# wenet-e2e/wenet

Hardware: AMD Instinct MI355X
Metric: audio-seconds/sec (RTF^-1), 12L Conformer fbank80, ctc_prefix_beam_search (higher is better)
Workload: dtype f32 (feed-forward and subsampling-conv2 GEMMs: fp32 operands as three exact bf16 planes, six plane products on the bf16 matrix cores, f32 accumulate -- error <= the v_mfma_f32 kernel's, tests/test_gpu_x6.py; everything else v_mfma_f32)

## Files before the change

include/wenet_amd.h:

```cpp
#ifndef WENET_AMD_H_
#define WENET_AMD_H_

#include <stdint.h>

#ifdef __cplusplus
extern "C" {
#endif

typedef struct wn_model wn_model;

typedef struct {
  int32_t feat_dim;
  int32_t d_model;
  int32_t n_heads;
  int32_t ffn_dim;
  int32_t n_layers;
  int32_t cnn_kernel;
  int32_t causal;
  int32_t use_dynamic_chunk;
  int32_t static_chunk_size;
  int32_t vocab;
  int32_t has_cmvn;
  int32_t dec_heads;
  int32_t dec_ffn_dim;
  int32_t dec_layers;
  int32_t dec_r_layers;
  int32_t bidirectional;
  int32_t sos, eos;
  int32_t max_pos;
  float norm_eps;
  int32_t encoder_type;
  int32_t input_layer;
  int32_t activation;
  int32_t key_bias;
  int32_t cnn_norm;
  int32_t dec_activation;
  int32_t dec_key_bias;
  int32_t dec_src_key_bias;
  int32_t dec_learned_pos;
  int32_t dec_max_pos;
} wn_config;

typedef struct {
  const char* name;
  const float* data;
  int64_t numel;
} wn_tensor;

const char* wn_last_error(void);
const char* wn_version(void);

int wn_model_create(const wn_config* cfg, const wn_tensor* weights,
                    int32_t n_weights, int32_t device, wn_model** out);
void wn_model_destroy(wn_model* m);

int wn_model_clone(const wn_model* src, wn_model** out);

#define WN_PREC_F32 0
#define WN_PREC_BF16 1
#define WN_PREC_FP8 2
int wn_model_set_precision(wn_model* m, int32_t precision);
int32_t wn_model_get_precision(const wn_model* m);

int32_t wn_batch_size(const wn_model* m);

int wn_model_set_encode_gate(wn_model* m, void* event);

int wn_workspace_create(int32_t device, wn_model** out);

int64_t wn_resample_length(int64_t n_in, int32_t orig_freq, int32_t new_freq);
int wn_resample(wn_model* m, const float* pcm_dev, int64_t n_in, int32_t orig_freq,
                int32_t new_freq, float* out_dev, int64_t n_out, void* stream);

int wn_fbank(wn_model* m, const float* pcm_dev, const int64_t* sample_off_host,
             int32_t B, float* feats_dev, int32_t max_frames,
             int32_t* n_frames_host, void* stream);

int wn_log_mel(wn_model* m, const float* pcm_dev, const int64_t* sample_off_host,
               int32_t B, int32_t n_mels, float* feats_dev, int32_t max_frames,
               int32_t* n_frames_host, void* stream);

int wn_encode(wn_model* m, const float* feats_dev, const int32_t* feat_lens_host,
              int32_t B, int32_t T, int32_t decoding_chunk_size,
              int32_t num_left_chunks, float* enc_out_dev,
              int32_t* enc_lens_host, void* stream);

int wn_encode_chunk(wn_model* m, const float* feats_dev, int32_t time, int32_t offset,
                    int32_t required_cache_size, const float* att_cache_dev,
                    int32_t cache_t1, const float* cnn_cache_dev, float* out_dev,
                    float* new_att_cache_dev, float* new_cnn_cache_dev,
                    int32_t* chunk_out, int32_t* new_cache_t1_out, void* stream);

int wn_encode_chunk_batch(wn_model* m, int32_t n_sess, const float* feats_dev, int32_t time,
                          const int32_t* offsets_host, int32_t required_cache_size,
                          const float* const* att_cache_dev, const int32_t* cache_t1_host,
                          const float* const* cnn_cache_dev, float* out_dev,
                          float* const* new_att_cache_dev, float* const* new_cnn_cache_dev,
                          int32_t* chunk_out, int32_t* new_cache_t1_out, void* stream);

int wn_set_encoder_out(wn_model* m, const float* enc_out_dev,
                       const int32_t* enc_lens_host, int32_t B, int32_t Tp,
                       void* stream);

int wn_ctc_logprobs(wn_model* m, int32_t topk, int32_t blank_id,
                    float blank_penalty, float* logp_dev, int32_t Tp,
                    void* stream);

int wn_set_ctc_probs(wn_model* m, const float* logp_dev,
                     const int32_t* lens_host, int32_t B, int32_t Tp,
                     int32_t V, int32_t topk, void* stream);

int wn_ctc_greedy_search(wn_model* m, int32_t blank_id, int32_t* tokens_host,
                         int32_t* tok_lens_host, int32_t max_len, void* stream);

int wn_ctc_force_align(wn_model* m, int32_t blank_id, float blank_penalty,
                       const int32_t* labels_host, const int32_t* label_lens_host,
                       int32_t max_label, const float* logp_dev, const int32_t* lens_host,
                       int32_t B, int32_t Tp, int32_t V, int32_t* path_host, float* score_host,
                       int32_t* status_host, float* frame_logp_host, float* emit_host,
                       void* stream);

int wn_set_context_graph(wn_model* m, int32_t n_nodes, const int32_t* fail,
                         const double* node_score, const double* output_score,
                         const double* token_score, int32_t n_edges,
                         const int32_t* edge_from, const int32_t* edge_token,
                         const int32_t* edge_to, void* stream);

int wn_ctc_prefix_beam_search(wn_model* m, int32_t beam, int32_t blank_id,
                              int32_t* n_hyps_host, int32_t* hyp_lens_host,
                              int32_t* hyp_tlens_host, int32_t* hyp_tokens_host,
                              int32_t* hyp_times_host, double* hyp_scores_host,
                              int32_t max_len, void* stream);

typedef struct wn_stream_set wn_stream_set;

typedef struct wn_stream_result {
  int32_t* n_hyps;
  int32_t* hyp_lens;
  int32_t* hyp_tlens;
  int32_t* hyp_tokens;
  int32_t* hyp_times;
  double* hyp_scores;
  double* hyp_viterbi;
  int32_t* frames_decoded;
  int32_t* trailing_blank;
  int32_t max_len;
} wn_stream_result;

int wn_stream_create(wn_model* m, int32_t n_slots, int32_t beam, int32_t max_frames,
                     int32_t blank_id, wn_stream_set** out, void* stream);
int wn_stream_destroy(wn_stream_set* set);

int wn_stream_set_endpoint(wn_stream_set* set, float blank_threshold, float blank_scale);

int wn_stream_reset(wn_stream_set* set, int32_t n, const int32_t* slot_ids, void* stream);

int wn_stream_advance(wn_stream_set* set, int32_t n, const int32_t* slot_ids,
                      const float* logp_dev, const int32_t* n_t_host, int32_t Tp, int32_t V,
                      int32_t nbest, const wn_stream_result* out, void* stream);

int wn_stream_advance_encoded(wn_stream_set* set, int32_t n, const int32_t* slot_ids,
                              const float* enc_out_dev, const int32_t* n_t_host, int32_t chunk,
                              int32_t nbest, const wn_stream_result* out, void* stream);

int wn_attention_rescoring(wn_model* m, int32_t beam, const int32_t* n_hyps_host,
                           const int32_t* hyp_lens_host,
                           const int32_t* hyp_tokens_host, int32_t max_len,
                           float reverse_weight, float* l2r_logp_host,
                           float* r2l_logp_host, void* stream);

int wn_rescore_prefetch(wn_model* m, int32_t use_right_decoder, void* stream);

int wn_rescore(wn_model* m, int32_t beam, const int32_t* n_hyps_host,
               const int32_t* hyp_lens_host, const int32_t* hyp_tokens_host,
               const double* ctc_scores_host, int32_t max_len, double ctc_weight,
               double reverse_weight, int32_t* best_idx_host, float* best_score_host,
               double* confidence_host, double* tok_conf_host, float* all_scores_host,
               void* stream);

int wn_decoder_forward(wn_model* m, int32_t utt, int32_t which, int32_t n_seq,
                       const int32_t* tokens_host, const int32_t* lens_host,
                       int32_t max_len, float* logp_dev, void* stream);

int wn_filter_blank_embedding(wn_model* m, float* padded_out_dev, int32_t* n_keep_host,
                              int32_t* t_out, void* stream);

int wn_attention_beam_search(wn_model* m, int32_t beam, int32_t maxlen, float length_penalty,
                             int32_t* tokens_host, int32_t* lens_host, void* stream);

// ... 395 lines not shown
```

wenet_amd/_lib.py:

```python
import ctypes
import os
from ctypes import (POINTER, Structure, c_char_p, c_double, c_float, c_int32,
                    c_int64, c_void_p)

_HERE = os.path.dirname(os.path.abspath(__file__))
LIB_PATH = os.path.join(_HERE, 'libwenet_amd.so')


class WnConfig(Structure):
    _fields_ = [(n, c_int32) for n in (
        'feat_dim', 'd_model', 'n_heads', 'ffn_dim', 'n_layers', 'cnn_kernel',
        'causal', 'use_dynamic_chunk', 'static_chunk_size', 'vocab',
        'has_cmvn', 'dec_heads', 'dec_ffn_dim', 'dec_layers', 'dec_r_layers',
        'bidirectional', 'sos', 'eos', 'max_pos')] + [('norm_eps', c_float)] + [
            (n, c_int32) for n in ('encoder_type', 'input_layer', 'activation',
                                   'key_bias', 'cnn_norm',
                                   'dec_activation', 'dec_key_bias', 'dec_src_key_bias',
                                   'dec_learned_pos', 'dec_max_pos')]


class WnTransducerConfig(Structure):
    _fields_ = [(n, c_int32) for n in ('pred_embed', 'pred_hidden', 'pred_layers', 'pred_out',
                                       'join_dim', 'blank')]


class WnStatelessPredictorConfig(Structure):
    _fields_ = [(n, c_int32) for n in ('kind', 'context', 'heads', 'activation', 'conv_bias')] + [
        ('norm_eps', c_float)]


class WnFireRedConfig(Structure):
    _fields_ = [(n, c_int32) for n in ('sub_channels', 'conv_inner_factor', 'max_frames')] + [
        ('attn_norm_eps', c_float)]


class WnBranchformerConfig(Structure):
    _fields_ = [(n, c_int32) for n in ('kind', 'cgmlp_units', 'cgmlp_kernel', 'merge_kernel',
                                       'linear_after_conv', 'head_dim')]


class WnParaformerConfig(Structure):
    _fields_ = [(n, c_int32) for n in ('lfr_m', 'lfr_n', 'kernel_size', 'dec_blocks',
                                       'max_frames')] + [
        (n, c_float) for n in ('threshold', 'tail_threshold', 'smooth_factor',
                               'noise_threshold')]


class WnTensor(Structure):
    _fields_ = [('name', c_char_p), ('data', POINTER(c_float)),
                ('numel', c_int64)]


class WnStreamResult(Structure):
    _fields_ = [('n_hyps', POINTER(c_int32)), ('hyp_lens', POINTER(c_int32)),
                ('hyp_tlens', POINTER(c_int32)), ('hyp_tokens', POINTER(c_int32)),
                ('hyp_times', POINTER(c_int32)), ('hyp_scores', POINTER(c_double)),
                ('hyp_viterbi', POINTER(c_double)), ('frames_decoded', POINTER(c_int32)),
                ('trailing_blank', POINTER(c_int32)), ('max_len', c_int32)]


class WnRnntStreamResult(Structure):
    _fields_ = [('tok_lens', POINTER(c_int32)), ('tokens', POINTER(c_int32)),
                ('times', POINTER(c_int32)), ('frames_decoded', POINTER(c_int32)),
                ('trailing_blank', POINTER(c_int32)), ('max_len', c_int32),
                ('steps', POINTER(c_int32))]


class WnRnntBeamStreamResult(Structure):
    _fields_ = [('n_hyps', POINTER(c_int32)), ('hyp_lens', POINTER(c_int32)),
                ('hyp_tokens', POINTER(c_int32)), ('hyp_scores', POINTER(c_double)),
                ('frames_decoded', POINTER(c_int32)), ('trailing_blank', POINTER(c_int32)),
                ('max_len', c_int32)]


class WnAttentionOp(Structure):
    _fields_ = [('Q', c_void_p), ('K', c_void_p), ('V', c_void_p),
                ('ldq', c_int32), ('ldk', c_int32), ('ldv', c_int32),
                ('q_rows', c_int32), ('kv_rows', c_int32),
                ('P', c_void_p), ('ldp', c_int32), ('p_rows', c_int32),
                ('p_off', POINTER(c_int32)), ('bias_u', c_void_p), ('bias_v', c_void_p),
                ('O', c_void_p), ('ldo', c_int32),
                ('q_off', POINTER(c_int32)), ('q_len', POINTER(c_int32)),
                ('kv_off', POINTER(c_int32)), ('kv_len', POINTER(c_int32)),
                ('n_seq', c_int32), ('n_heads', c_int32), ('mask_mode', c_int32),
                ('chunk_size', c_int32), ('left_chunks', c_int32), ('scale', c_float),
                ('flags', c_int32), ('precision', c_int32), ('x6_galign', c_int32)]


EXPORTS = [
    'wn_last_error', 'wn_version', 'wn_model_create', 'wn_model_destroy', 'wn_model_clone',
    'wn_model_set_precision', 'wn_model_get_precision', 'wn_batch_size', 'wn_model_set_encode_gate', 'wn_op_gemm_bf16',
    'wn_op_gemm_bf16_stored',
    'wn_attention_beam_search', 'wn_attention_beam_search_prompt', 'wn_attention_truncated',
    'wn_op_gemm_skinny', 'wn_encode_chunk_batch', 'wn_op_gemm_lowp', 'wn_op_mx_quantize', 'wn_op_ffn_fused', 'wn_op_gemm_x6', 'wn_op_ffn_x6', 'wn_op_gemm_x6r', 'wn_op_gemm_x6r512', 'wn_profile_kernel_name', 'wn_profile_ffn_split', 'wn_profile_ffn_clocks', 'wn_profile_gemm_clocks', 'wn_filter_blank_embedding',
    'wn_workspace_create', 'wn_resample_length', 'wn_resample', 'wn_fbank', 'wn_log_mel', 'wn_encode', 'wn_encode_chunk', 'wn_set_encoder_out',
    'wn_ctc_logprobs', 'wn_set_ctc_probs', 'wn_ctc_greedy_search', 'wn_ctc_force_align',
    'wn_set_context_graph', 'wn_ctc_prefix_beam_search', 'wn_attention_rescoring', 'wn_rescore', 'wn_rescore_prefetch', 'wn_decoder_forward', 'wn_decoder_next_topk', 'wn_op_gemm',
    'wn_op_layernorm', 'wn_op_log_add', 'wn_op_attention', 'wn_op_dwconv', 'wn_op_conv1',
    'wn_op_conv2d4',
    'wn_op_ctc_rows', 'wn_debug_set', 'wn_profile_enable',
    'wn_profile_collect', 'wn_tune_set', 'wn_model_tune_set', 'wn_tune_get',
    'wn_stream_create', 'wn_stream_destroy', 'wn_stream_set_endpoint', 'wn_stream_reset',
    'wn_stream_advance', 'wn_stream_advance_encoded',
    'wn_model_create_transducer', 'wn_transducer_greedy_search', 'wn_op_lstm_step',
    'wn_op_joint_argmax', 'wn_transducer_beam_search', 'wn_op_joint_fuse_topk',
    'wn_op_rnnt_beam_step', 'wn_transducer_beam_stats',
    'wn_rnnt_stream_create', 'wn_rnnt_stream_destroy', 'wn_rnnt_stream_reset',
    'wn_rnnt_stream_advance_encoded', 'wn_rnnt_stream_state',
    'wn_rnnt_beam_stream_create', 'wn_rnnt_beam_stream_destroy', 'wn_rnnt_beam_stream_reset',
    'wn_rnnt_beam_stream_advance_encoded', 'wn_rnnt_beam_stream_state',
    'wn_op_rnnt_beam_step_carry',
    'wn_transducer_score', 'wn_transducer_score_stats', 'wn_transducer_score_times',
    'wn_op_rnnt_trie',
    'wn_op_joint_logp_gather', 'wn_op_rnnt_lattice',
    'wn_op_attn_self_step', 'wn_op_attn_step_embed', 'wn_op_attn_prompt_cache', 'wn_op_beam_init',
    'wn_op_beam_update', 'wn_op_beam_finish',
    'wn_op_layernorm_ex', 'wn_op_layernorm2', 'wn_op_layernorm_mx', 'wn_op_ffn_reduce_ln',
    'wn_op_gemm_rowln',
    'wn_model_create_transducer_stateless', 'wn_op_stateless_step',
    'wn_op_attention_relshift', 'wn_op_firered_frontend', 'wn_model_create_firered',
    'wn_model_create_branchformer', 'wn_op_csgu_gate', 'wn_op_merge_dwconv', 'wn_csgu_time_tile',
    'wn_op_attention_d128', 'wn_op_lfr_front', 'wn_op_layernorm_wide', 'wn_op_cif_alpha',
    'wn_op_cif_fire', 'wn_model_create_paraformer', 'wn_paraformer_decode',
]

_lib = None


def lib():
    global _lib
    if _lib is not None:
        return _lib
    if not os.path.exists(LIB_PATH):
        raise RuntimeError(
            f'{LIB_PATH} is missing: build it with `python -m wenet_amd.build` '
            '(hipcc --offload-arch=gfx950). wenet_amd has no CPU fallback.')
    import torch
    L = ctypes.CDLL(LIB_PATH, mode=ctypes.RTLD_GLOBAL)
    i32, i64, f32, vp = c_int32, c_int64, c_float, c_void_p
    pi32, pf64 = POINTER(c_int32), POINTER(c_double)
    L.wn_last_error.restype = c_char_p
    L.wn_profile_kernel_name.restype = c_char_p
    L.wn_profile_kernel_name.argtypes = [vp]
    L.wn_profile_ffn_split.restype = c_int32
    L.wn_profile_ffn_split.argtypes = [vp]
    L.wn_profile_ffn_clocks.argtypes = [POINTER(ctypes.c_uint64)]
    L.wn_profile_gemm_clocks.argtypes = [POINTER(ctypes.c_uint64)]
    L.wn_version.restype = c_char_p
    L.wn_model_create.argtypes = [POINTER(WnConfig), POINTER(WnTensor), i32,
                                  i32, POINTER(vp)]
    L.wn_model_destroy.argtypes = [vp]
    L.wn_model_clone.argtypes = [vp, POINTER(vp)]
    L.wn_model_destroy.restype = None
    L.wn_workspace_create.argtypes = [i32, POINTER(vp)]
    L.wn_fbank.argtypes = [vp, vp, POINTER(i64), i32, vp, i32, pi32, vp]
    L.wn_log_mel.argtypes = [vp, vp, POINTER(i64), i32, i32, vp, i32, pi32, vp]
    L.wn_encode.argtypes = [vp, vp, pi32, i32, i32, i32, i32, vp, pi32, vp]
    L.wn_set_encoder_out.argtypes = [vp, vp, pi32, i32, i32, vp]
    L.wn_ctc_logprobs.argtypes = [vp, i32, i32, f32, vp, i32, vp]
    L.wn_encode_chunk.argtypes = [vp, vp, i32, i32, i32, vp, i32, vp, vp, vp, vp, pi32,
                                  pi32, vp]
    L.wn_encode_chunk_batch.argtypes = [vp, i32, vp, i32, pi32, i32, POINTER(vp), pi32,
                                        POINTER(vp), vp, POINTER(vp), POINTER(vp), pi32, pi32,
                                        vp]
    L.wn_resample_length.argtypes = [ctypes.c_int64, i32, i32]
    L.wn_resample_length.restype = ctypes.c_int64
    L.wn_resample.argtypes = [vp, vp, ctypes.c_int64, i32, i32, vp, ctypes.c_int64, vp]
    L.wn_set_ctc_probs.argtypes = [vp, vp, pi32, i32, i32, i32, i32, vp]
    L.wn_ctc_greedy_search.argtypes = [vp, i32, pi32, pi32, i32, vp]
    L.wn_ctc_force_align.argtypes = [vp, i32, f32, pi32, pi32, i32, vp, pi32, i32, i32, i32,
                                     pi32, POINTER(f32), pi32, POINTER(f32), POINTER(f32), vp]
    L.wn_set_context_graph.argtypes = [vp, i32, pi32, pf64, pf64, pf64, i32, pi32, pi32,
                                       pi32, vp]
    L.wn_ctc_prefix_beam_search.argtypes = [vp, i32, i32, pi32, pi32, pi32,
                                            pi32, pi32, pf64, i32, vp]
    L.wn_stream_create.argtypes = [vp, i32, i32, i32, i32, POINTER(vp), vp]
    L.wn_stream_destroy.argtypes = [vp]
    L.wn_stream_set_endpoint.argtypes = [vp, f32, f32]
    L.wn_stream_reset.argtypes = [vp, i32, pi32, vp]
    L.wn_stream_advance.argtypes = [vp, i32, pi32, vp, pi32, i32, i32, i32,
                                    POINTER(WnStreamResult), vp]
    L.wn_stream_advance_encoded.argtypes = [vp, i32, pi32, vp, pi32, i32, i32,
                                            POINTER(WnStreamResult), vp]
    L.wn_attention_rescoring.argtypes = [vp, i32, pi32, pi32, pi32, i32, f32,
                                         POINTER(f32), POINTER(f32), vp]
    L.wn_rescore.argtypes = [vp, i32, pi32, pi32, pi32, pf64, i32, c_double, c_double, pi32,
                             POINTER(f32), pf64, pf64, POINTER(f32), vp]
    L.wn_rescore_prefetch.argtypes = [vp, i32, vp]
    L.wn_decoder_forward.argtypes = [vp, i32, i32, i32, pi32, pi32, i32, vp, vp]
    L.wn_decoder_next_topk.argtypes = [vp, i32, pi32, pi32, pi32, i32, i32,
                                       POINTER(f32), pi32, vp]
    L.wn_attention_beam_search.argtypes = [vp, i32, i32, f32, pi32, pi32, vp]
    L.wn_attention_beam_search_prompt.argtypes = [vp, i32, i32, f32, pi32, i32, pi32, pi32, vp]
    L.wn_attention_truncated.argtypes = [vp]
    L.wn_op_gemm.argtypes = [vp, vp, vp, vp, vp, i32, i32, i32, f32, i32, vp]
    L.wn_op_gemm_skinny.argtypes = [vp, vp, vp, vp, vp, i32, i32, i32, i32, i32, i32, vp]
    L.wn_op_gemm_bf16.argtypes = L.wn_op_gemm.argtypes
    L.wn_op_gemm_bf16_stored.argtypes = [vp, vp, vp, vp, vp, i32, i32, i32, f32, i32, i32, vp]
    L.wn_op_gemm_lowp.argtypes = [vp, vp, vp, vp, vp, vp, vp, vp, i32, i32, i32, f32, i32, i32,
                                  i32, vp]
    L.wn_op_mx_quantize.argtypes = [vp, i32, i32, vp, vp, vp]
    L.wn_op_ffn_fused.argtypes = [vp, vp, vp, vp, vp, vp, vp, vp, vp, i32, i32, i32, i32, f32,
                                  f32, vp]
    L.wn_op_gemm_x6.argtypes = [vp, vp, vp, vp, vp, i32, i32, i32, f32, i32, i32, i32, vp]
    L.wn_op_ffn_x6.argtypes = [vp, vp, vp, vp, vp, vp, vp, vp, vp, i32, i32, i32, i32, f32,
                               f32, i32, vp]
    L.wn_filter_blank_embedding.argtypes = [vp, vp, pi32, pi32, vp]
    L.wn_op_gemm_x6r.argtypes = [vp, vp, vp, vp, vp, vp, vp, vp, i32, i32, i32, f32, f32, i32, vp]
    L.wn_op_gemm_x6r512.argtypes = [vp, vp, vp, vp, vp, vp, vp, vp, vp, vp, i32, i32, i32, f32, f32,
                                    i32, vp]
    L.wn_model_set_precision.argtypes = [vp, i32]
    L.wn_model_get_precision.argtypes = [vp]
    L.wn_batch_size.argtypes = [vp]
    L.wn_batch_size.restype = i32
    L.wn_model_set_encode_gate.argtypes = [vp, vp]
    L.wn_op_layernorm.argtypes = [vp, vp, vp, vp, i32, i32, f32, vp]
    L.wn_op_log_add.argtypes = [vp, vp, vp, i32, vp]
    L.wn_op_attention.argtypes = [POINTER(WnAttentionOp), pi32, vp]
    L.wn_op_dwconv.argtypes = [vp, i32, vp, vp, vp, vp, vp, i32, vp, i32, pi32, pi32, i32, i32,
                               i32, i32, i32, i32, f32, vp]
    L.wn_op_conv1.argtypes = [vp, vp, vp, vp, vp, vp, pi32, pi32, i32, i32, i32, i32, i32, i32,
                              vp]
    L.wn_op_conv2d4.argtypes = [vp, vp, pi32, i32, i32, vp, vp, vp, pi32, pi32, vp]
    L.wn_op_ctc_rows.argtypes = [vp, i32, i32, i32, i32, i32, f32, vp, vp, vp, i32, vp]
    L.wn_debug_set.argtypes = [vp, c_char_p, i32]
    L.wn_tune_set.argtypes = [c_char_p, i32]
    L.wn_model_tune_set.argtypes = [vp, c_char_p, i32]
    L.wn_tune_get.argtypes = [vp, c_char_p, pi32]
    L.wn_profile_enable.argtypes = [vp, i32]
    L.wn_profile_collect.argtypes = [vp, pi32, pf64, pf64]
    L.wn_model_create_transducer.argtypes = [POINTER(WnConfig), POINTER(WnTransducerConfig),
                                             POINTER(WnTensor), i32, i32, POINTER(vp)]
    L.wn_model_create_transducer_stateless.argtypes = [
        POINTER(WnConfig), POINTER(WnTransducerConfig), POINTER(WnStatelessPredictorConfig),
        POINTER(WnTensor), i32, i32, POINTER(vp)]
    L.wn_op_stateless_step.argtypes = [POINTER(WnStatelessPredictorConfig), pi32, POINTER(vp),
                                       pi32, vp, i32, i32, i32, i32, vp]
    L.wn_transducer_greedy_search.argtypes = [vp, i32, pi32, pi32, i32, pi32, vp]
    L.wn_rnnt_stream_create.argtypes = [vp, i32, i32, i32, i32, POINTER(vp), vp]
    L.wn_rnnt_stream_destroy.argtypes = [vp]
    L.wn_rnnt_stream_reset.argtypes = [vp, i32, pi32, vp]
    L.wn_rnnt_stream_advance_encoded.argtypes = [vp, i32, pi32, vp, pi32, i32,
# ... 107 lines not shown
```

wenet_amd/csrc/cabi_align.hip:

```cpp
#include "model_state.h"

namespace wn {
namespace {

int align_check(int blank_id, const int32_t* labels, const int32_t* label_lens, int max_label,
                const int32_t* lens, int B, int Tp, int V, const int32_t* status_host) {
  WN_CHECK(labels && label_lens && status_host, "wn_ctc_force_align: null argument");
  WN_CHECK(B >= 1 && Tp >= 1 && V >= 1 && max_label >= 0, "wn_ctc_force_align: bad argument");
  WN_CHECK(blank_id >= 0 && blank_id < V, "wn_ctc_force_align: blank_id outside the vocabulary");
  for (int b = 0; b < B; ++b) {
    WN_CHECK(label_lens[b] >= 0 && label_lens[b] <= max_label,
             "wn_ctc_force_align: label_len must be in [0, max_label]");
    if (lens) WN_CHECK(lens[b] >= 0 && lens[b] <= Tp, "wn_ctc_force_align: length > Tp");
    for (int i = 0; i < label_lens[b]; ++i) {
      const int id = labels[(size_t)b * max_label + i];
      if (id < 0 || id >= V) {
        set_error("wn_ctc_force_align: label id " + std::to_string(id) + " of utterance " +
                  std::to_string(b) + " is outside the vocabulary [0, " + std::to_string(V) + ")");
        return -1;
      }
      WN_CHECK(id != blank_id, "wn_ctc_force_align: blank_id among the labels");
    }
  }
  return 0;
// ... 2 lines not shown
}
}

extern "C" {

int wn_ctc_force_align(wn_model* m, int32_t blank_id, float blank_penalty,
                       const int32_t* labels_host, const int32_t* label_lens_host,
                       int32_t max_label, const float* logp_dev, const int32_t* lens_host,
                       int32_t B, int32_t Tp, int32_t V, int32_t* path_host, float* score_host,
                       int32_t* status_host, float* frame_logp_host, float* emit_host,
                       void* stream) {
  const bool given = logp_dev != nullptr;
  if (given) {
    WN_CHECK(lens_host, "wn_ctc_force_align: null lengths with caller-provided log-probs");
    WN_TRY(align_check(blank_id, labels_host, label_lens_host, max_label, lens_host, B, Tp, V,
                       status_host));
    WN_CHECK(m, "wn_ctc_force_align: null handle");
  } else {
    WN_CHECK(m && m->B > 0 && m->enc.p,
             "wn_ctc_force_align: no current batch (call wn_encode / wn_set_encoder_out)");
    WN_CHECK(!lens_host, "wn_ctc_force_align: lens_host without logp_dev");
    WN_CHECK(B == m->B && Tp == m->Tp, "wn_ctc_force_align: B / Tp are not the current batch's");
    V = m->cfg.vocab;
    WN_TRY(align_check(blank_id, labels_host, label_lens_host, max_label, nullptr, B, Tp, V,
                       status_host));
  }
  WN_ENTER(m);
  PrecisionScope prec_scope(m);
  hipStream_t s = (hipStream_t)stream;
  WN_HIP(hipSetDevice(m->device));

  const int M = given ? B * Tp : m->rows;
  std::vector<int> off(B), len(B);
  for (int b = 0; b < B; ++b) {
    off[b] = given ? b * Tp : m->off[b];
    len[b] = given ? lens_host[b] : m->len[b];
  }
  const int LP = max_label + 1;
  int max_fast = -1, max_slow = -1;
  std::vector<int> d((size_t)3 * B + (size_t)B * LP);
  std::vector<int64_t> bp_off(B);
  int64_t bp_bytes = 0;
  for (int b = 0; b < B; ++b) {
    const int L = label_lens_host[b];
    d[b] = off[b]; d[B + b] = len[b]; d[2 * B + b] = L;
    int* lab = d.data() + 3 * (size_t)B + (size_t)b * LP;
    lab[0] = blank_id;
    for (int i = 0; i < LP - 1; ++i) lab[1 + i] = i < L ? labels_host[(size_t)b * max_label + i] : blank_id;
    if (2 * L + 1 <= ALIGN_FAST_S) max_fast = std::max(max_fast, L);
    else max_slow = std::max(max_slow, L);
    bp_off[b] = bp_bytes;
    bp_bytes += ctc_align_bp_bytes(len[b], L, ALIGN_FAST_S);
  }
  const size_t d_bytes = (d.size() * sizeof(int) + 7) / 8 * 8;
  WN_TRY(m->stage.begin(d_bytes + bp_off.size() * sizeof(int64_t) + 256));
  WN_TRY(m->al_desc.ensure(d_bytes + bp_off.size() * sizeof(int64_t)));
  WN_TRY(m->stage.put_at(m->al_desc.p, d.data(), d.size() * sizeof(int), s));
  WN_TRY(m->stage.put_at(m->al_desc.as<char>() + d_bytes, bp_off.data(),
                         bp_off.size() * sizeof(int64_t), s));
  WN_TRY(m->stage.end(s));
  const int* dd = m->al_desc.as<int>();

  const size_t o_sc = 0, o_st = o_sc + (size_t)B * sizeof(float),
               o_path = o_st + (size_t)B * sizeof(int),
               o_fl = o_path + (size_t)B * Tp * sizeof(int),
               o_e = (o_fl + (size_t)B * Tp * 2 * sizeof(float) + 255) / 256 * 256,
               o_end = o_e + (size_t)std::max(M, 1) * LP * sizeof(float);
  WN_TRY(m->al_out.ensure(o_end));
  WN_TRY(m->al_bp.ensure((size_t)bp_bytes + 64));
  char* ob = m->al_out.as<char>();
  float* E = reinterpret_cast<float*>(ob + o_e);

  if (M > 0) {
    AlignGatherArgs g;
    g.M = M; g.V = V; g.blank = blank_id;
    g.off = dd; g.len = dd + B; g.lab_len = dd + 2 * B; g.lab = dd + 3 * B; g.lab_pitch = LP;
    g.E = E; g.ldE = LP;
    if (given) {
      g.x = logp_dev; g.ld = V; g.normalize = 0; g.blank_penalty = 0.f;
      g.row_utt = nullptr; g.Tp = Tp;
    } else {
      const ModelData& W = *m->data;
      WN_CHECK(W.ctc.w, "wn_ctc_force_align: this handle has no weights");
      const int V4 = (V + 31) / 32 * 32;
      WN_TRY(m->logits.ensure((size_t)M * V4 * sizeof(float)));
      WN_TRY(vocab_linear(m, W.ctc, m->enc.as<float>(), m->cfg.d_model, m->logits.as<float>(), V4,
                          M, s));
      g.x = m->logits.as<float>(); g.ld = V4; g.normalize = 1;
      g.blank_penalty = blank_penalty > 0.f ? blank_penalty : 0.f;
      g.row_utt = m->d_row_utt.as<int>(); g.Tp = Tp;
    }
    WN_TRY(ctc_align_gather(g, s));
  }
  AlignArgs a;
  a.E = E; a.ldE = LP; a.off = dd; a.len = dd + B; a.B = B; a.Tp = Tp;
  a.lab = dd + 3 * B; a.lab_pitch = LP; a.lab_len = dd + 2 * B;
  a.bp = m->al_bp.as<unsigned char>();
  a.bp_off = reinterpret_cast<const int64_t*>(m->al_desc.as<char>() + d_bytes);
  a.fast_S = ALIGN_FAST_S;
  a.path = reinterpret_cast<int*>(ob + o_path);
  a.frame_logp = frame_logp_host ? reinterpret_cast<float*>(ob + o_fl) : nullptr;
  a.score = reinterpret_cast<float*>(ob + o_sc);
  a.status = reinterpret_cast<int*>(ob + o_st);
  WN_TRY(ctc_align_viterbi(a, max_fast, max_slow, s));
  const size_t n_copy = emit_host ? o_end : (frame_logp_host ? o_e : o_fl);
  WN_TRY(m->al_host.ensure(n_copy));
  WN_HIP(hipMemcpyAsync(m->al_host.p, ob, n_copy, hipMemcpyDeviceToHost, s));
  WN_HIP(stream_wait(s));
  const char* hb = m->al_host.p;
  const int* st = reinterpret_cast<const int*>(hb + o_st);
  const float* sc = reinterpret_cast<const float*>(hb + o_sc);
  for (int b = 0; b < B; ++b) {
    status_host[b] = st[b];
    if (st[b] != 0) continue;
    if (score_host) score_host[b] = sc[b];
    const size_t n = (size_t)len[b];
    if (path_host)
      memcpy(path_host + (size_t)b * Tp, hb + o_path + (size_t)b * Tp * sizeof(int),
             n * sizeof(int));
    if (frame_logp_host)
      memcpy(frame_logp_host + (size_t)b * Tp * 2, hb + o_fl + (size_t)b * Tp * 2 * sizeof(float),
             n * 2 * sizeof(float));
    if (emit_host)
      memcpy(emit_host + (size_t)b * Tp * LP, hb + o_e + (size_t)off[b] * LP * sizeof(float),
             n * LP * sizeof(float));
  }
  return 0;
}

}
```

wenet_amd/csrc/cabi_ctc.hip:

```cpp
#include "model_state.h"

struct wn_stream_set {
  wn_model* m = nullptr;
  int n_slots = 0, beam = 0, max_frames = 0, blank = 0;
  float blank_thr = 0.8f;
  int64_t pool_ints = 0;
  DevBuf state, pool;
  DevBuf emit;
  std::vector<int> abs_t;
  DevBuf desc;
  Stager stage;
  DevBuf topk_val, topk_idx, logits;
  DevBuf out;
  PinnedBuf host;
};

namespace wn {
namespace {

__global__ void scatter_padded_any_kernel(const float* src, int lds,
                                          const int* off, const int* len,
                                          int Tp, int D, float* dst) {
  const int b = blockIdx.y, t = blockIdx.x;
  float* d = dst + ((int64_t)b * Tp + t) * D;
// ... 117 lines not shown
  WN_TRY(S->stage.begin(d.size() * sizeof(int) + 64));
  WN_TRY(S->stage.put(S->desc, d.data(), d.size() * sizeof(int), s));
  WN_TRY(S->stage.end(s));
  const StreamOutLayout o(n, rows, max_len);
  WN_TRY(S->out.ensure(o.end));
  WN_TRY(S->host.ensure(o.end));
  char* ob = S->out.as<char>();
  StreamPrefixBeamArgs a;
  a.topk_val = S->topk_val.as<float>(); a.topk_idx = S->topk_idx.as<int>(); a.k = beam;
  a.off = S->desc.as<int>() + n; a.len = S->desc.as<int>() + 2 * n; a.B = n;
  a.beam = beam; a.blank = S->blank; a.max_len = S->max_frames;
  a.pool = S->pool.as<int>(); a.pool_stride = S->pool_ints;
  a.n_hyps = reinterpret_cast<int*>(ob + o.nh); a.hyp_lens = reinterpret_cast<int*>(ob + o.len);
  a.hyp_tlens = reinterpret_cast<int*>(ob + o.tlen);
  a.hyp_tokens = reinterpret_cast<int*>(ob + o.tok);
  a.hyp_times = reinterpret_cast<int*>(ob + o.tim);
  a.hyp_scores = reinterpret_cast<double*>(ob + o.sc);
  a.st.state = S->state.p; a.st.slot = S->desc.as<int>();
  a.st.nbest = nbest ? 1 : 0; a.st.out_stride = max_len;
  a.st.logp = logp; a.st.ld = ld; a.st.blank_thr = S->blank_thr;
  a.st.hyp_vit = reinterpret_cast<double*>(ob + o.vit);
  a.st.emit = S->emit.as<int>();
  a.st.frames = reinterpret_cast<int*>(ob + o.fd); a.st.trail = reinterpret_cast<int*>(ob + o.tb);
  PbCycles dbg;
  WN_TRY(dbg.arm(S->m, &a.dbg_cycles));
  WN_TRY(ctc_prefix_beam_stream(a, s));
  WN_TRY(dbg.print("stream search", "state store + emit", false, s));
  WN_HIP(hipMemcpyAsync(S->host.p, ob, o.end, hipMemcpyDeviceToHost, s));
  for (int i = 0; i < n; ++i) S->abs_t[slot_ids[i]] += n_t[i];
  WN_HIP(stream_wait(s));
  const char* hb = S->host.p;
  const int* nh = reinterpret_cast<const int*>(hb + o.nh);
  const int* hl = reinterpret_cast<const int*>(hb + o.len);
  const int* htl = reinterpret_cast<const int*>(hb + o.tlen);
  const double* sc = reinterpret_cast<const double*>(hb + o.sc);
  const double* vit = reinterpret_cast<const double*>(hb + o.vit);
  memcpy(out->n_hyps, nh, (size_t)n * sizeof(int));
  memcpy(out->frames_decoded, hb + o.fd, (size_t)n * sizeof(int));
  memcpy(out->trailing_blank, hb + o.tb, (size_t)n * sizeof(int));
  for (int i = 0; i < n; ++i) {
    for (int j = 0; j < beam; ++j) {
      const size_t dst = (size_t)i * beam + j, src = (size_t)i * rows + j;
      const bool have = j < rows;
      const int nl = have ? std::min(std::max(hl[src], 0), max_len) : 0;
      const int ntl = have ? std::min(std::max(htl[src], 0), max_len) : 0;
      out->hyp_lens[dst] = nl; out->hyp_tlens[dst] = ntl;
      out->hyp_scores[dst] = have ? sc[src] : -HUGE_VAL;
      if (out->hyp_viterbi) out->hyp_viterbi[dst] = have ? vit[src] : -HUGE_VAL;
      if (have) {
        memcpy(out->hyp_tokens + dst * max_len, hb + o.tok + src * max_len * sizeof(int),
               (size_t)nl * sizeof(int));
        memcpy(out->hyp_times + dst * max_len, hb + o.tim + src * max_len * sizeof(int),
               (size_t)ntl * sizeof(int));
      }
    }
  }
  return 0;
}

}
}

extern "C" {

int wn_ctc_logprobs(wn_model* m, int32_t topk, int32_t blank_id,
                    float blank_penalty, float* logp_dev, int32_t Tp,
                    void* stream) {
  WN_CHECK(m && m->B > 0, "wn_ctc_logprobs: no current batch (call wn_encode)");
  WN_ENTER(m);
  m->pb_valid = false;
  PrecisionScope prec_scope(m);
  const ModelData& W = *m->data;
  WN_CHECK(W.ctc.w, "wn_ctc_logprobs: this handle has no weights");
  hipStream_t s = (hipStream_t)stream;
  WN_HIP(hipSetDevice(m->device));
  const wn_config& c = m->cfg;
  const int M = m->rows, V = c.vocab;
  const int k = std::max(1, topk);
  WN_CHECK(k <= V, "top-k larger than the vocabulary");
  WN_CHECK(!logp_dev || Tp == m->Tp, "wn_ctc_logprobs: Tp mismatch");
  m->ctc_rows = M; m->ctc_k = k;
  int ldv = V;
  if (M > 0) {
    const int V4 = (V + 31) / 32 * 32;
    ldv = V4;
    WN_TRY(m->logits.ensure((size_t)M * V4 * sizeof(float)));
    WN_TRY(m->topk_val.ensure((size_t)M * k * sizeof(float)));
    WN_TRY(m->topk_idx.ensure((size_t)M * k * sizeof(int)));
    WN_TRY(vocab_linear(m, W.ctc, m->enc.as<float>(), c.d_model, m->logits.as<float>(), V4, M,
                        s));
    CtcRowArgs r;
    r.logits = m->logits.as<float>(); r.ld = V4; r.M = M; r.V = V; r.k = k;
    r.blank = blank_id; r.blank_penalty = blank_penalty > 0.f ? blank_penalty : 0.f;
    r.topk_val = m->topk_val.as<float>(); r.topk_idx = m->topk_idx.as<int>();
    r.logp = logp_dev ? m->logits.as<float>() : nullptr; r.ld_out = V4;
    WN_TRY(ctc_logsoftmax_topk(r, s));
  }
  if (logp_dev) {
    if (M > 0) {
      hipLaunchKernelGGL(scatter_padded_any_kernel, dim3(m->Tp, m->B), dim3(256),
                         0, s, m->logits.as<float>(), ldv, m->d_off.as<int>(),
                         m->d_len.as<int>(), m->Tp, V, logp_dev);
      WN_HIP(hipGetLastError());
    } else {
      WN_HIP(hipMemsetAsync(logp_dev, 0, (size_t)m->B * m->Tp * V * sizeof(float), s));
    }
  }
  m->ctc_valid = true;
  return 0;
}

int wn_set_ctc_probs(wn_model* m, const float* logp_dev, const int32_t* lens_host,
                     int32_t B, int32_t Tp, int32_t V, int32_t topk,
                     void* stream) {
  WN_CHECK(m && logp_dev && lens_host && B > 0 && Tp > 0 && V > 0,
           "wn_set_ctc_probs: bad argument");
  WN_ENTER(m);
  m->pb_valid = false;
  hipStream_t s = (hipStream_t)stream;
  WN_HIP(hipSetDevice(m->device));
  const int k = std::max(1, topk);
  WN_CHECK(k <= V, "top-k larger than the vocabulary");
  std::vector<int> off(B), len(B);
  for (int b = 0; b < B; ++b) {
    WN_CHECK(lens_host[b] >= 0 && lens_host[b] <= Tp, "length > Tp");
    off[b] = b * Tp; len[b] = lens_host[b];
  }
  WN_TRY(set_layout(m, B, Tp, off, len, B * Tp, s));
  WN_TRY(m->stage.end(s));
  const int M = B * Tp;
  WN_TRY(m->topk_val.ensure((size_t)M * k * sizeof(float)));
  WN_TRY(m->topk_idx.ensure((size_t)M * k * sizeof(int)));
  hipLaunchKernelGGL(topk_raw_kernel, dim3(M), dim3(256), 0, s, logp_dev, V, V,
                     k, m->topk_val.as<float>(), m->topk_idx.as<int>());
  WN_HIP(hipGetLastError());
  m->ctc_rows = M; m->ctc_k = k; m->ctc_valid = true;
  return 0;
}

int wn_ctc_greedy_search(wn_model* m, int32_t blank_id, int32_t* tokens_host,
                         int32_t* tok_lens_host, int32_t max_len, void* stream) {
  WN_CHECK(m && m->ctc_valid, "greedy: no CTC posteriors (call wn_ctc_logprobs)");
  WN_ENTER(m);
  WN_CHECK(tokens_host && tok_lens_host, "greedy: null output");
  hipStream_t s = (hipStream_t)stream;
  WN_HIP(hipSetDevice(m->device));
  const int B = m->B;
  int longest = 0;
  for (int b = 0; b < B; ++b) longest = std::max(longest, m->len[b]);
  WN_CHECK(max_len >= longest, "greedy: max_len smaller than the longest utterance");
  const int ml = std::max(max_len, 1);
  WN_TRY(m->g_tok.ensure((size_t)B * ml * sizeof(int)));
  WN_TRY(m->g_len.ensure((size_t)B * sizeof(int)));
  WN_TRY(ctc_greedy_collapse(m->topk_idx.as<int>(), m->ctc_k, m->d_off.as<int>(),
                             m->d_len.as<int>(), B, blank_id, m->g_tok.as<int>(),
                             ml, m->g_len.as<int>(), s));
  WN_HIP(hipMemcpyAsync(tokens_host, m->g_tok.p, (size_t)B * ml * sizeof(int),
                        hipMemcpyDeviceToHost, s));
  WN_HIP(hipMemcpyAsync(tok_lens_host, m->g_len.p, (size_t)B * sizeof(int),
                        hipMemcpyDeviceToHost, s));
  WN_HIP(stream_wait(s));
  return 0;
}

int wn_filter_blank_embedding(wn_model* m, float* padded_out_dev, int32_t* n_keep_host,
                              int32_t* t_out, void* stream) {
  WN_CHECK(m && m->B > 0 && m->enc.p && m->ctc_valid && n_keep_host && t_out,
           "filter_blank_embedding: needs the encoder output and the CTC posteriors of the "
           "current batch (wn_encode / wn_set_encoder_out, then wn_ctc_logprobs)");
  WN_ENTER(m);
  hipStream_t s = (hipStream_t)stream;
  WN_HIP(hipSetDevice(m->device));
  const int B = m->B, d = m->cfg.d_model, M = m->rows;
  WN_CHECK(m->ctc_rows == M, "filter_blank_embedding: CTC posteriors of another layout");
  WN_TRY(m->nb_map.ensure((size_t)std::max(M, 1) * sizeof(int)));
  WN_TRY(m->nb_keep.ensure((size_t)B * sizeof(int)));
  WN_TRY(nonblank_map(m->topk_idx.as<int>(), m->ctc_k, m->d_off.as<int>(), m->d_len.as<int>(), B,
                      m->nb_map.as<int>(), m->nb_keep.as<int>(), s));
  std::vector<int> keep(B);
  WN_HIP(hipMemcpyAsync(keep.data(), m->nb_keep.p, (size_t)B * sizeof(int),
                        hipMemcpyDeviceToHost, s));
  WN_HIP(stream_wait(s));
  int T = 0;
  for (int b = 0; b < B; ++b) { n_keep_host[b] = keep[b]; T = std::max(T, keep[b]); }
  *t_out = T;
  if (T == 0) {
    static bool warned = false;
    if (!warned) {
      fprintf(stderr, "[wenet_amd] filter_blank_embedding: no non-blank frame in the whole "
                      "batch; the encoder output is left unfiltered\n");
      warned = true;
// ... 184 lines not shown
  WN_TRY(S->desc.ensure(3 * (size_t)n_slots * sizeof(int)));
  const StreamOutLayout o(n_slots, 1, max_frames);
  WN_TRY(S->out.ensure(o.end));
  WN_TRY(S->host.ensure(o.end));
  std::vector<int> all(n_slots);
  for (int i = 0; i < n_slots; ++i) all[i] = i;
  WN_TRY(S->stage.begin(all.size() * sizeof(int) + 64));
  WN_TRY(S->stage.put(S->desc, all.data(), all.size() * sizeof(int), s));
  WN_TRY(S->stage.end(s));
  WN_TRY(ctc_stream_reset(S->state.p, S->pool.as<int>(), S->pool_ints, max_frames, beam,
                          S->desc.as<int>(), n_slots, s));
  WN_HIP(hipStreamSynchronize(s));
  *out = S.release();
  return 0;
}

int wn_stream_destroy(wn_stream_set* set) {
  delete set;
  return 0;
}

int wn_stream_set_endpoint(wn_stream_set* set, float blank_threshold, float blank_scale) {
  WN_CHECK(set, "wn_stream_set_endpoint: null argument");
  WN_CHECK(blank_threshold > 0.f && blank_scale > 0.f, "wn_stream_set_endpoint: bad argument");
  set->blank_thr = blank_threshold * blank_scale;
  return 0;
}

int wn_stream_reset(wn_stream_set* set, int32_t n, const int32_t* slot_ids, void* stream) {
  WN_CHECK(set && slot_ids, "wn_stream_reset: null argument");
  WN_CHECK(n >= 1 && n <= set->n_slots, "wn_stream_reset: n must be in [1, n_slots]");
  for (int i = 0; i < n; ++i)
    WN_CHECK(slot_ids[i] >= 0 && slot_ids[i] < set->n_slots, "wn_stream_reset: slot id out of range");
  WN_ENTER(set->m);
  hipStream_t s = (hipStream_t)stream;
  WN_HIP(hipSetDevice(set->m->device));
  WN_TRY(set->stage.begin((size_t)n * sizeof(int) + 64));
  WN_TRY(set->stage.put(set->desc, slot_ids, (size_t)n * sizeof(int), s));
  WN_TRY(set->stage.end(s));
  WN_TRY(ctc_stream_reset(set->state.p, set->pool.as<int>(), set->pool_ints, set->max_frames,
                          set->beam, set->desc.as<int>(), n, s));
  for (int i = 0; i < n; ++i) set->abs_t[slot_ids[i]] = 0;
  return 0;
}

int wn_stream_advance(wn_stream_set* set, int32_t n, const int32_t* slot_ids,
                      const float* logp_dev, const int32_t* n_t_host, int32_t Tp, int32_t V,
                      int32_t nbest, const wn_stream_result* out, void* stream) {
  WN_CHECK(set && slot_ids && logp_dev && n_t_host && out, "wn_stream_advance: null argument");
  WN_CHECK(Tp >= 1 && V >= 1, "wn_stream_advance: bad argument");
  WN_CHECK(set->beam <= V, "wn_stream_advance: top-k larger than the vocabulary");
  WN_CHECK(set->blank < V, "wn_stream_advance: blank_id outside the vocabulary");
  WN_TRY(stream_check(set, n, slot_ids, n_t_host, Tp, out));
  WN_ENTER(set->m);
  hipStream_t s = (hipStream_t)stream;
  WN_HIP(hipSetDevice(set->m->device));
  const int M = n * Tp, k = set->beam;
  WN_TRY(set->topk_val.ensure((size_t)M * k * sizeof(float)));
  WN_TRY(set->topk_idx.ensure((size_t)M * k * sizeof(int)));
  hipLaunchKernelGGL(topk_raw_kernel, dim3(M), dim3(256), 0, s, logp_dev, V, V, k,
                     set->topk_val.as<float>(), set->topk_idx.as<int>());
  WN_HIP(hipGetLastError());
  return stream_search(set, n, slot_ids, n_t_host, Tp, logp_dev, V, nbest, out, s);
}

int wn_stream_advance_encoded(wn_stream_set* set, int32_t n, const int32_t* slot_ids,
                              const float* enc_out_dev, const int32_t* n_t_host, int32_t chunk,
                              int32_t nbest, const wn_stream_result* out, void* stream) {
  WN_CHECK(set && slot_ids && enc_out_dev && n_t_host && out,
           "wn_stream_advance_encoded: null argument");
  WN_CHECK(chunk >= 1, "wn_stream_advance_encoded: bad argument");
  wn_model* m = set->m;
  const ModelData& W = *m->data;
  WN_CHECK(W.ctc.w, "wn_stream_advance_encoded: this handle has no weights");
  WN_CHECK(set->beam <= m->cfg.vocab && set->blank < m->cfg.vocab,
           "wn_stream_advance_encoded: beam / blank_id outside the vocabulary");
  WN_TRY(stream_check(set, n, slot_ids, n_t_host, chunk, out));
  WN_ENTER(m);
  PrecisionScope prec_scope(m);
  hipStream_t s = (hipStream_t)stream;
  WN_HIP(hipSetDevice(m->device));
  const wn_config& c = m->cfg;
  const int M = n * chunk, V = c.vocab, k = set->beam;
  const int V4 = (V + 31) / 32 * 32;
  WN_TRY(set->logits.ensure((size_t)M * V4 * sizeof(float)));
  WN_TRY(set->topk_val.ensure((size_t)M * k * sizeof(float)));
  WN_TRY(set->topk_idx.ensure((size_t)M * k * sizeof(int)));
  WN_TRY(vocab_linear(m, W.ctc, enc_out_dev, c.d_model, set->logits.as<float>(), V4, M, s));
  CtcRowArgs r;
  r.logits = set->logits.as<float>(); r.ld = V4; r.M = M; r.V = V; r.k = k;
  r.blank = set->blank; r.blank_penalty = 0.f;
  r.topk_val = set->topk_val.as<float>(); r.topk_idx = set->topk_idx.as<int>();
  r.logp = set->logits.as<float>(); r.ld_out = V4;
  WN_TRY(ctc_logsoftmax_topk(r, s));
  return stream_search(set, n, slot_ids, n_t_host, chunk, set->logits.as<float>(), V4, nbest, out,
                       s);
}

}
```

wenet_amd/csrc/cabi_firered.hip:

```cpp
#include "model_state.h"

static int encoder_layers_firered(wn_model* m, hipStream_t s) {
  const ModelData& W = *m->data;
  const wn_config& c = m->cfg;
  const int d = c.d_model, d2 = 2 * d, H = c.n_heads, M = m->rows;
  float* x = m->x.as<float>();
  float* t1 = m->t1.as<float>();
  float* t2 = m->t2.as<float>();
  float* hb = m->hbuf.as<float>();
  float* qkv = m->qkv.as<float>();
  const float eps = c.norm_eps;
  int max_len = 0;
  for (int b = 0; b < m->B; ++b) max_len = std::max(max_len, m->len[b]);
  const int n_run = m->dbg_layers >= 0 ? std::min(m->dbg_layers, c.n_layers) : c.n_layers;
  for (int li = 0; li < n_run; ++li) {
    const EncLayer& L = W.layers[li];
    WN_TRY(ln(L.norm_ff_mac, x, t1, M, d, eps, s));
    WN_TRY(linear(L.ffm1, t1, d, hb, c.ffn_dim, M, s, ACT_SILU));
    WN_TRY(linear(L.ffm2, hb, c.ffn_dim, x, d, M, s, ACT_NONE, x, d, 0.5f));
    WN_TRY(ln(L.norm_mha, x, t1, M, d, m->fr.c.attn_norm_eps, s));
    WN_TRY(linear(L.qkv, t1, d, qkv, 3 * d, M, s));
    RelShiftAttnArgs a;
    a.Q = qkv; a.K = qkv + d; a.V = qkv + 2 * d;
    a.ldq = a.ldk = a.ldv = 3 * d;
    a.P = L.pos_tab; a.ldp = d;
    a.p_center = m->fr.c.max_frames - 1; a.p_rows = 2 * m->fr.c.max_frames - 1;
    a.bias_u = L.bias_u; a.bias_v = L.bias_v;
    a.O = t2; a.ldo = d;
    a.off = m->d_off.as<int>(); a.len = m->d_len.as<int>();
    a.n_seq = m->B; a.n_heads = H; a.max_len = max_len;
    a.scale = 1.0f / sqrtf(64.0f);
    WN_TRY(attention_relshift(a, s));
    WN_TRY(linear(L.out, t2, d, x, d, M, s, ACT_NONE, x, d));
    WN_TRY(ln(L.norm_conv, x, t1, M, d, eps, s));
    float* glu = hb;
    float* cv = hb + (size_t)M * d2;
    WN_TRY(linear(L.pw1, t1, d, glu, d2, M, s, ACT_NONE, nullptr, 0, 1.0f, true));
    DwConvArgs dw;
    dw.x = glu; dw.ldx = d2; dw.wt = L.dw_wt; dw.bias = L.dw_b; dw.cpad = L.cpad;
    dw.ln_w = L.conv_norm.w; dw.ln_b = L.conv_norm.b; dw.norm_mode = 0;
    dw.y = cv; dw.ldy = d2;
    dw.row_utt = m->d_row_utt.as<int>(); dw.off = m->d_off.as<int>(); dw.len = m->d_len.as<int>();
    dw.M = M; dw.D = d2; dw.K = c.cnn_kernel; dw.causal = 0;
    dw.t_max = m->Tp; dw.eps = 1e-5f;
    WN_TRY(dwconv_ln_silu(dw, s));
    WN_TRY(linear(L.pw2, cv, d2, x, d, M, s, ACT_NONE, x, d));
    WN_TRY(ln(L.norm_ff, x, t1, M, d, eps, s));
    WN_TRY(linear(L.ff1, t1, d, hb, c.ffn_dim, M, s, ACT_SILU));
    WN_TRY(linear(L.ff2, hb, c.ffn_dim, x, d, M, s, ACT_NONE, x, d, 0.5f));
    WN_TRY(ln(L.norm_final, x, x, M, d, eps, s));
  }
  WN_TRY(m->enc.ensure((size_t)std::max(M, 1) * d * sizeof(float)));
  WN_HIP(hipMemcpyAsync(m->enc.p, m->x.p, (size_t)M * d * sizeof(float), hipMemcpyDeviceToDevice,
                        s));
  return 0;
}

int encode_firered(wn_model* m, const float* feats_dev, const int32_t* feat_lens_host, int B, int T,
                   float* enc_out_dev, int32_t* enc_lens_host, hipStream_t s) {
  const ModelData& W = *m->data;
  const wn_config& c = m->cfg;
  const int d = c.d_model, F1 = m->F1(), F2 = m->F2(), C = m->fr.c.sub_channels;
  auto out_len = [](int n) { return n > 0 ? ((n + 6 - 3) / 2 + 1 - 3) / 2 + 1 : 0; };
  const int Tp = out_len(T);
  WN_CHECK(B < 65536, "wn_encode: more than 65535 utterances");
  WN_CHECK(Tp <= m->fr.c.max_frames,
           "wn_encode: an utterance of " + std::to_string(T) + " frames gives " +
               std::to_string(Tp) + " encoder frames, more than the " +
               std::to_string(m->fr.c.max_frames) + " the position rows of this handle cover");
  m->ln0_done = false;
  m->front_route = 0;
  std::vector<int> off2(B), len2(B), off1(B), len1(B), flen(B);
  int M = 0, M1 = 0, max_t2 = 0;
  for (int b = 0; b < B; ++b) {
    const int L = feat_lens_host[b];
    WN_CHECK(L >= 0 && L <= T, "wn_encode: feature length out of range");
    const int l2 = out_len(L), l1 = l2 > 0 ? 2 * l2 + 1 : 0;
    flen[b] = L;
    off2[b] = M; len2[b] = l2; M += l2;
    off1[b] = M1; len1[b] = l1; M1 += l1;
    max_t2 = std::max(max_t2, l2);
    if (enc_lens_host) enc_lens_host[b] = l2;
  }
  WN_TRY(set_layout(m, B, Tp, off2, len2, M, s));
  if (M > 0) {
    WN_TRY(upload_desc(m, m->d_off1, off1, s));
    WN_TRY(upload_desc(m, m->d_len1, len1, s));
    WN_TRY(upload_desc(m, m->ck_desc, flen, s));
  }
  WN_TRY(m->stage.end(s));
  if (M > 0) {
    const int hid = std::max(c.ffn_dim, 4 * d);
    WN_TRY(m->c1.ensure((size_t)M1 * F1 * C * sizeof(float)));
    WN_TRY(m->c2.ensure((size_t)M * F2 * C * sizeof(float)));
    WN_TRY(m->x.ensure((size_t)M * d * sizeof(float)));
    WN_TRY(m->t1.ensure((size_t)M * d * sizeof(float)));
    WN_TRY(m->t2.ensure((size_t)M * d * sizeof(float)));
    WN_TRY(m->hbuf.ensure((size_t)M * hid * sizeof(float)));
    WN_TRY(m->qkv.ensure((size_t)M * 3 * d * sizeof(float)));
    FireRedFrontArgs a;
    a.feats = feats_dev; a.mean = W.cmvn_mean; a.istd = W.cmvn_istd;
    a.w1 = W.conv1_w; a.b1 = W.conv1_b; a.w2 = W.conv2.w; a.b2 = W.conv2.b;
    a.h1 = m->c1.as<float>(); a.out = m->c2.as<float>(); a.ldo = C * F2;
    a.len = m->ck_desc.as<int>();
    a.t1_off = m->d_off1.as<int>(); a.t1_len = m->d_len1.as<int>();
    a.t2_off = m->d_off.as<int>(); a.t2_len = m->d_len.as<int>();
    a.B = B; a.T = T; a.F = c.feat_dim; a.F1 = F1; a.F2 = F2; a.C = C; a.max_t2 = max_t2;
    WN_TRY(firered_frontend(a, s));
    WN_TRY(linear(W.sub_out, m->c2.as<float>(), C * F2, m->x.as<float>(), d, M, s));
    WN_TRY(encoder_layers_firered(m, s));
  }
  if (enc_out_dev) {
    if (M > 0) {
      WN_TRY(scatter_padded(m->enc.as<float>(), d, m->d_off.as<int>(), m->d_len.as<int>(), B, Tp,
                            d, enc_out_dev, s));
    } else if (Tp > 0) {
      WN_HIP(hipMemsetAsync(enc_out_dev, 0, (size_t)B * Tp * d * sizeof(float), s));
    }
  }
  return 0;
}

extern "C" {

int wn_model_create_firered(const wn_config* cfg, const wn_firered_config* fcfg,
                            const wn_tensor* weights, int32_t n_weights, int32_t device,
                            wn_model** out) {
  WN_CHECK(fcfg, "wn_model_create_firered: null argument");
  return create_model_impl(cfg, nullptr, nullptr, fcfg, nullptr, weights, n_weights, device, out);
}

}
```

wenet_amd/csrc/cabi_model.hip:

```cpp
#include "model_state.h"
#include "weight_stage.h"

namespace wn {
namespace {

int stage_fused(const Src& src, HostStage& hs, const std::string& name,
                const std::vector<std::string>& parts, int out_each, int in,
                int no_bias_part = -1) {
  std::vector<float> w((size_t)parts.size() * out_each * in),
      b((size_t)parts.size() * out_each, 0.f);
  for (size_t i = 0; i < parts.size(); ++i) {
    WN_GET(pw, parts[i] + ".weight", (int64_t)out_each * in);
    memcpy(w.data() + i * out_each * in, pw, sizeof(float) * out_each * in);
    if ((int)i == no_bias_part) continue;
    WN_GET(pb, parts[i] + ".bias", out_each);
    memcpy(b.data() + i * out_each, pb, sizeof(float) * out_each);
  }
  hs.add(name + ".weight", w.data(), w.size());
  hs.add(name + ".bias", b.data(), b.size());
  return 0;
}

int stage_decoder(const Src& src, HostStage& hs, const std::string& pfx,
                  int nlayers, const wn_config& c) {
// ... 818 lines not shown
        if (!l->w || l->in % 128 != 0) continue;
        char* q = p;
        p += ((size_t)l->out * l->in + 255) / 256 * 256;
        unsigned* sc = reinterpret_cast<unsigned*>(p);
        p += (size_t)(l->in / 128) * l->out * 4;
        WN_TRY(mx_quantize(l->w, l->in, l->out, l->in, q, sc, l->out, nullptr));
        at[l->w] = ModelData::MxW{q, sc};
      }
      WN_HIP(hipStreamSynchronize(nullptr));
    }
    W.weights_mx.swap(buf);
    W.mx_at.swap(at);
    W.mx_built = true;
  }
  m->prec = precision == PREC_F32 ? PREC_F32 : PREC_BF16;
  m->fp8_ffn = precision == PREC_FP8;
  return 0;
}

int32_t wn_model_get_precision(const wn_model* m) {
  return m ? (m->fp8_ffn ? (int32_t)PREC_FP8 : m->prec) : -1;
}

int32_t wn_batch_size(const wn_model* m) { return m ? m->B : -1; }

int wn_model_set_encode_gate(wn_model* m, void* event) {
  WN_CHECK(m, "wn_model_set_encode_gate: null handle");
  m->enc_gate = (hipEvent_t)event;
  return 0;
}

int wn_profile_enable(wn_model* m, int32_t on) {
  WN_CHECK(m, "wn_profile_enable: null model");
  m->prof_on = on != 0;
  m->prof_stride = on > 1 ? (unsigned)on : 6u;
  m->prof_used = 0;
  m->prof_flops = 0.0;
  return 0;
}

const char* wn_profile_kernel_name(const wn_model* m) {
  return m ? m->prof_kernel : "";
}

int32_t wn_profile_ffn_split(const wn_model* m) { return m ? m->prof_split : 0; }

int wn_profile_gemm_clocks(uint64_t* out64) {
  WN_CHECK(out64, "wn_profile_gemm_clocks: null output");
  if (wn::tune().x6_probe == 8)
    return wn::gemm_x6r_clocks(reinterpret_cast<unsigned long long*>(out64));
  if (wn::tune().lp_probe & 4)
    return wn::gemm_lp_clocks(reinterpret_cast<unsigned long long*>(out64));
  return wn::gemm_x6_clocks(reinterpret_cast<unsigned long long*>(out64));
}

int wn_profile_ffn_clocks(uint64_t* out64) {
  WN_CHECK(out64, "wn_profile_ffn_clocks: null output");
  return wn::ffn_x6f_clocks(reinterpret_cast<unsigned long long*>(out64));
}

int wn_profile_collect(wn_model* m, int32_t* n_launches, double* total_ms,
                       double* total_flops) {
  WN_CHECK(m && n_launches && total_ms && total_flops, "wn_profile_collect: null");
  double ms = 0.0;
  for (size_t i = 0; i + 1 < m->prof_used; i += 2) {
    WN_HIP(hipEventSynchronize(m->prof_ev[i + 1]));
    float t = 0.f;
    WN_HIP(hipEventElapsedTime(&t, m->prof_ev[i], m->prof_ev[i + 1]));
    ms += t;
  }
  *n_launches = (int32_t)(m->prof_used / 2);
  *total_ms = ms;
  *total_flops = m->prof_flops;
  m->prof_used = 0;
  m->prof_flops = 0.0;
  return 0;
}

int wn_debug_set(wn_model* m, const char* key, int32_t value) {
  WN_CHECK(m && key, "wn_debug_set: null argument");
  const std::string k(key);
  if (k == "n_layers") m->dbg_layers = value;
  else if (k == "skip_after_norm") m->dbg_skip_after_norm = value;
  else { set_error("wn_debug_set: unknown key " + k); return -1; }
  return 0;
}

int wn_tune_set(const char* key, int32_t value) {
  WN_CHECK(key, "wn_tune_set: null key");
  const std::string k(key);
  int* f = tune_field(g_tune_default, k);
  if (!f) { set_error("wn_tune_set: unknown key " + k); return -1; }
  WN_CHECK(value != TUNE_INHERIT, "wn_tune_set: INT32_MIN is the per-handle 'inherit' marker");
  if (tune_check(k, value, "wn_tune_set") != 0) return -1;
  *f = value;
  return 0;
}

int wn_model_tune_set(wn_model* m, const char* key, int32_t value) {
  WN_CHECK(m && key, "wn_model_tune_set: null argument");
  WN_ENTER(m);
  const std::string k(key);
  int* f = tune_field(m->tune_ovr, k);
  if (!f) { set_error("wn_model_tune_set: unknown key " + k); return -1; }
  if (tune_check(k, value, "wn_model_tune_set") != 0) return -1;
  *f = value;
  return 0;
}

int wn_tune_get(const wn_model* m, const char* key, int32_t* value) {
  WN_CHECK(key && value, "wn_tune_get: null argument");
  const std::string k(key);
  Tune eff = g_tune_default;
  if (m) tune_resolve(m->tune_ovr, &eff);
  const int* f = tune_field(eff, k);
  if (!f) { set_error("wn_tune_get: unknown key " + k); return -1; }
  *value = *f;
  return 0;
}

int wn_workspace_create(int32_t device, wn_model** out) {
  WN_CHECK(out, "wn_workspace_create: null argument");
  WN_HIP(hipSetDevice(device));
  wn_model* m = new wn_model();
  memset(&m->cfg, 0, sizeof(m->cfg));
  m->device = device;
  *out = m;
  return 0;
}

}
```

wenet_amd/csrc/conformer.hip:

```cpp
#include <algorithm>
#include "model_state.h"

namespace {
struct ProfBracket {
  wn_model* m;
  hipStream_t s;
  bool on = false;
  int record(int which) { WN_HIP(hipEventRecord(m->prof_ev[m->prof_used + which], s)); return 0; }
  int begin() {
    on = m->prof_on && (m->prof_seq++ % m->prof_stride) == 0;
    if (!on) return 0;
    if (m->prof_used + 2 > m->prof_ev.size())
      for (int i = 0; i < 64; ++i) {
        hipEvent_t e;
        WN_HIP(hipEventCreate(&e));
        m->prof_ev.push_back(e);
      }
    return record(0);
  }
  int end(double flops, const char* kernel) {
    if (!on) return 0;
    WN_TRY(record(1));
    m->prof_used += 2;
    m->prof_flops += flops;
// ... 10 lines not shown
  WN_TRY(linear(l, A, l.in, C, l.out, M, s, act, nullptr, 0, 1.0f, false, h16, h16));
  return pb.end(2.0 * M * (double)l.out * l.in,
                t_linear_took_x6
                    ? "x6_split + gemm_x6_kernel (FFN w_1 + act through linear(), six bf16 plane products)"
                    : "gemm (FFN w_1)");
}

int ffn_module(wn_model* m, const Norm& nrm, const Linear& w1, const Linear& w2, int act,
               float alpha, bool ln_done, bool h16, hipStream_t s) {
  const wn_config& c = m->cfg;
  const int d = c.d_model, M = m->rows;
  float* x = m->x.as<float>();
  float* t1 = m->t1.as<float>();
  float* hb = m->hbuf.as<float>();
  bool mx = false;
  const ModelData::MxW *q1 = nullptr, *q2 = nullptr;
  if (t_mx && h16 && !ln_done) {
    auto i1 = t_mx->find(w1.w), i2 = t_mx->find(w2.w);
    const int64_t t256 = (int64_t)cdiv(M, 256) * cdiv(std::min(w1.out, w2.out), 256);
    GemmArgs p1, p2;
    p1.M = p2.M = M; p1.N = w1.out; p1.K = d; p1.lda = d; p1.ldc = w1.out;
    p1.fp8 = p2.fp8 = true; p1.c_mx = true;
    p2.N = d; p2.K = w1.out; p2.lda = w1.out; p2.ldc = d; p2.resid = x; p2.ldr = d;
    if (i1 != t_mx->end() && i2 != t_mx->end() && d % 256 == 0 && w1.out % 128 == 0 &&
        t256 >= tune().fp8_min_tiles && gemm_bf16p_supported(p1) && gemm_bf16p_supported(p2)) {
      mx = true; q1 = &i1->second; q2 = &i2->second;
    }
  }
  if (!mx) {
    if (!ln_done) WN_TRY(ln(nrm, x, t1, M, d, c.norm_eps, s, h16));
    WN_TRY(ffn_w1(m, w1, t1, hb, M, s, act, h16));
    return linear(w2, hb, w1.out, x, d, M, s, ACT_NONE, x, d, alpha, false, h16);
  }
  const int pitch = cdiv(M, 256) * 256;
  WN_TRY(m->mx_sa.ensure((size_t)(d / 128) * pitch * 4));
  WN_TRY(m->mx_sh.ensure((size_t)(w1.out / 128) * pitch * 4));
  WN_TRY(layernorm_mx(x, d, nrm.w, nrm.b, t1, m->mx_sa.as<unsigned>(), pitch, M, d,
                      c.norm_eps, s));
  GemmArgs g;
  g.A = t1; g.bias = w1.b; g.C = hb; g.M = M; g.N = w1.out; g.K = d;
  g.lda = d; g.ldc = w1.out; g.act = act; g.fp8 = true; g.c_mx = true;
  g.a_scale = m->mx_sa.as<unsigned>(); g.a_scale_pitch = pitch;
  g.w_scale = q1->scale; g.w_scale_pitch = w1.out;
  g.c_scale = m->mx_sh.as<unsigned>(); g.c_scale_pitch = pitch;
  ProfBracket pb{m, s};
  WN_TRY(pb.begin());
  WN_TRY(gemm_mxfp8(g, q1->q, s));
  WN_TRY(pb.end(2.0 * M * (double)w1.out * d, nullptr));
  GemmArgs h;
  h.A = hb; h.bias = w2.b; h.C = x; h.resid = x; h.M = M; h.N = d; h.K = w1.out;
  h.lda = w1.out; h.ldc = d; h.ldr = d; h.alpha = alpha; h.fp8 = true;
  h.a_scale = m->mx_sh.as<unsigned>(); h.a_scale_pitch = pitch;
  h.w_scale = q2->scale; h.w_scale_pitch = d;
  return gemm_mxfp8(h, q2->q, s);
}

int ffn_x6_split(int M, int F) {
  int S = 1;
  while (S < 16 && cdiv(M, 128) * (S * 2) <= 256 && (F / 16) % (S * 2) == 0) S *= 2;
  return S;
}

static int ffn_x6_route(wn_model* m, const Linear& w1, const Linear& w2, int act) {
  const ModelData& W = *m->data;
  const int d = m->cfg.d_model, M = m->rows, F = w1.out;
  if (t_gemm_prec != PREC_F32 || tune().gemm_x6 == 0 || w1.out != w2.in ||
      !(d == 256 || d == 512) || F % 16 != 0)
    return 0;
  const bool small = M < 512 && tune().gemm_x6 != 2;
  const bool fused_ok = tune().ffn_x6f != 0 && tune().x6_af32 == 0 &&
                        ffn_x6f_supported(M, d, F, act) && !(small && tune().ffn_x6f == 3);
  if (W.x6_at.count(w1.w) == 0 || W.x6_at.count(w2.w) == 0) return 0;
  const bool fused = fused_ok && W.x6p_at.count(w2.w) != 0;
  if (small) return fused ? 1 : 0;
  return fused ? 1 : 2;
}

static void* t1_image_for(wn_model* m, const Linear& w1, const Linear& w2, int act) {
  if (tune().ffn_ximg == 0) return nullptr;
  const int r = ffn_x6_route(m, w1, w2, act);
  if (r == 0 || (r == 2 && tune().x6_af32 != 0)) return nullptr;
  if (m->t1_img.ensure(x6_bytes(m->rows, m->cfg.d_model)) != 0) return nullptr;
  return m->t1_img.p;
}

static int ffn_x6_try(wn_model* m, const Linear& w1, const Linear& w2, int act, hipStream_t s) {
  const ModelData& W = *m->data;
  const int d = m->cfg.d_model, M = m->rows, F = w1.out;
  const bool ximg = m->t1_img_ok;
  m->t1_img_ok = false;
  const int route = ffn_x6_route(m, w1, w2, act);
  WN_CHECK(route != 0 || !ximg,
           "ffn_x6_try: LN(x) was left as a plane image but no six-product form takes it");
  if (route == 0) return 0;
  auto i1 = W.x6_at.find(w1.w), i2 = W.x6_at.find(w2.w);
  ProfBracket pb{m, s};
  if (route == 1) {
    FfnX6Args a;
    a.S = ffn_x6f_split(M, F);
    if (m->ffn_part.ensure((size_t)a.S * M * d * sizeof(float)) != 0) return -1;
    a.X = m->t1.as<float>(); a.ldx = d; a.W13 = i1->second; a.W2p = W.x6p_at.find(w2.w)->second;
    a.b1 = w1.b;
    if (ximg) { a.X3 = m->t1_img.p; a.X = nullptr; }
    a.P = m->ffn_part.as<float>(); a.M = M; a.D = d; a.F = F; a.act = act;
    WN_TRY(pb.begin());
    if (ffn_x6f(a, s) != 0) return -1;
    WN_TRY(pb.end(4.0 * M * (double)F * d,
                  "ffn_x6f_kernel (FFN w_1 + act + w_2, six bf16 plane products)"));
    m->prof_split = a.S;
    return a.S;
  }
  const int S = ffn_x6_split(M, F);
  if (m->ffn_part.ensure((size_t)S * M * d * sizeof(float)) != 0) return -1;
  const bool af32 = tune().x6_af32 != 0 && (int64_t)M * F * 4 < ((int64_t)1 << 31);
  X6Args g1;
  g1.B3 = i1->second; g1.M = M; g1.N = F; g1.K = d; g1.bias = w1.b; g1.act = act;
  if (af32) {
    WN_CHECK(!ximg, "ffn_x6_try: LN(x) was left as a plane image, x6_af32 wants fp32 rows");
    if (m->hbuf.ensure((size_t)M * F * sizeof(float)) != 0) return -1;
    g1.A = m->t1.as<float>(); g1.lda = d; g1.a_bytes = (int64_t)M * d * 4;
    g1.epi = 0; g1.C = m->hbuf.as<float>(); g1.ldc = F;
  } else {
    if (m->x6_h.ensure(x6_bytes(M, F)) != 0 || (!ximg && m->x6_a.ensure(x6_bytes(M, d)) != 0)) return -1;
    if (!ximg && x6_split(m->t1.as<float>(), M, d, d, m->x6_a.as<char>(), s) != 0) return -1;
    g1.A3 = ximg ? m->t1_img.as<char>() : m->x6_a.as<char>(); g1.epi = 2; g1.C3 = m->x6_h.as<char>();
  }
  WN_TRY(pb.begin());
  if (gemm_x6(g1, s) != 0) return -1;
  WN_TRY(pb.end(2.0 * M * (double)F * d, "gemm_x6_kernel (FFN w_1 + act, six bf16 plane products)"));
  X6Args g2;
  g2.B3 = i2->second; g2.M = M; g2.N = d; g2.K = F;
  g2.epi = 1; g2.ksplit = S; g2.C = m->ffn_part.as<float>();
  if (af32) { g2.A = m->hbuf.as<float>(); g2.lda = F; g2.a_bytes = (int64_t)M * F * 4; }
  else g2.A3 = m->x6_h.as<char>();
  if (gemm_x6(g2, s) != 0) return -1;
  m->prof_split = S;
  return S;
}

int ffn_x6_pair(wn_model* m, const Linear& w1, const Linear& w2, int act, const float* A, int M,
                hipStream_t s) {
  const ModelData& W = *m->data;
  const int d = w1.in, F = w1.out;
  if (t_gemm_prec != PREC_F32 || tune().gemm_x6 == 0 || tune().x6_linear == 0 ||
      w1.out != w2.in || w2.out != d || !(d == 256 || d == 512) || F % 16 != 0 || M < 512 ||
      2.0 * M * (double)F * d < 1e8 * g_x6_linear_min)
    return 0;
  auto i1 = W.x6_at.find(w1.w), i2 = W.x6_at.find(w2.w);
  if (i1 == W.x6_at.end() || i2 == W.x6_at.end()) return 0;
  const int S = ffn_x6_split(M, F);
  if (m->ffn_part.ensure((size_t)S * M * d * sizeof(float)) != 0 ||
      m->x6_a.ensure(x6_bytes(M, d)) != 0 || m->x6_h.ensure(x6_bytes(M, F)) != 0)
    return -1;
  if (x6_split(A, M, d, d, m->x6_a.as<char>(), s) != 0) return -1;
  X6Args g1;
  g1.A3 = m->x6_a.as<char>(); g1.B3 = i1->second; g1.M = M; g1.N = F; g1.K = d; g1.bias = w1.b;
  g1.act = act; g1.epi = 2; g1.C3 = m->x6_h.as<char>();
  if (gemm_x6(g1, s) != 0) return -1;
  X6Args g2;
  g2.A3 = m->x6_h.as<char>(); g2.B3 = i2->second; g2.M = M; g2.N = d; g2.K = F;
  g2.epi = 1; g2.ksplit = S; g2.C = m->ffn_part.as<float>();
  if (gemm_x6(g2, s) != 0) return -1;
  return S;
}

static int ffn_fused_try(wn_model* m, const Linear& w1, const Linear& w2, int act, hipStream_t s) {
// ... 146 lines not shown
  a.mask_mode = c.mask_mode; a.chunk_size = c.cs; a.left_chunks = c.lc;
  a.scale = 1.0f / sqrtf(64.0f);
  if (ax6_img) {
    a.x6_img = m->attn_img.p; a.x6_img_bytes = m->attn_img.cap; a.x6_rows = M;
    if (tune().attn_x6_galign != 0) {
      a.x6_galign = 1;
      a.row_utt = m->d_row_utt.as<int>();
    }
  } else if (a.fold && tune().attn_x6 != 0 && c.f32 && M >= 512) {
    if (m->attn_img.ensure(attention_x6_image_bytes(M, m->B, H)) == 0) {
      a.x6_img = m->attn_img.p; a.x6_img_bytes = m->attn_img.cap; a.x6_rows = M;
    }
  }
  if (c.f32 && tune().attn_x6_order != 0 && m->attn_n_blk > 0) {
    a.blk_tab = m->d_row_utt.as<int>() + m->attn_blk_off;
    a.n_blk = m->attn_n_blk;
  }
  if (!qkv_q) return attention(a, s);
  a.x6_img_ready = true;
  WN_CHECK(a.fold && attention_x6_supported(a),
           "encoder: QKV wrote the key-tile images but the six-product attention declines");
  return attention_x6(a, s);
}

int conv_module(const LayerCtx& c, const EncLayer& L, bool* ln_ff_done) {
  wn_model* m = c.m;
  const wn_config& cfg = m->cfg;
  const int d = c.d, M = c.M;
  hipStream_t s = c.s;
  float *x = c.x, *t1 = c.t1, *t2 = c.t2;
  auto image = [&](const Linear& l, int N, int epi) {
    return c.rowx ? x6r_image(c, l, N, epi) : nullptr;
  };
  const void* out_ch = tune().x6r_chain != 0 ? image(L.out, d, 3) : nullptr;
  const void* pw1_ch = !out_ch ? nullptr : d == 512 ? x6_image(L.pw1) : image(L.pw1, 2 * d, 2);
  if (out_ch && pw1_ch) {
    X6RArgs g = x6r_rowln_args(c, L.out, out_ch, t2, L.norm_conv, 3);
    g.y = nullptr;
    g.W3b = pw1_ch; g.bias2 = L.pw1.b; g.C = t2; g.ldc = d;
    if (gemm_x6r(g, s) != 0) return -2;
  } else {
    if (const void* w6 = image(L.out, d, 1)) {
      if (gemm_x6r(x6r_rowln_args(c, L.out, w6, t2, L.norm_conv, 1), s) != 0) return -2;
    } else if (c.rowln) {
      WN_TRY(rowln_gemm(c, L.out, t2, L.norm_conv));
    } else {
      WN_TRY(linear(L.out, t2, d, x, d, M, s, ACT_NONE, x, d, 1.0f, false, c.h16));
      WN_TRY(ln(L.norm_conv, x, t1, M, d, c.eps, s, c.h16));
    }
    if (const void* w6 = image(L.pw1, 2 * d, 2)) {
      X6RArgs g;
      g.A = t1; g.lda = d; g.K = d; g.W3 = w6; g.bias = L.pw1.b; g.M = M; g.N = 2 * d;
      g.epi = 2; g.C = t2; g.ldc = d;
      WN_TRY(gemm_x6r(g, s));
    } else {
      WN_TRY(linear(L.pw1, t1, d, t2, d, M, s, ACT_NONE, nullptr, 0, 1.0f, true, c.h16));
    }
  }
  DwConvArgs dw;
  dw.x = t2; dw.ldx = d; dw.wt = L.dw_wt; dw.bias = L.dw_b; dw.cpad = L.cpad;
  dw.ln_w = L.conv_norm.w; dw.ln_b = L.conv_norm.b; dw.norm_mode = cfg.cnn_norm;
  dw.y = t1; dw.ldy = d;
  dw.row_utt = m->d_row_utt.as<int>(); dw.off = m->d_off.as<int>();
  dw.len = m->d_len.as<int>();
  dw.M = M; dw.D = d; dw.K = cfg.cnn_kernel; dw.causal = cfg.causal;
  dw.t_max = m->Tp; dw.eps = 1e-5f;
  const void* pw2_w6 = image(L.pw2, d, 1);
  const bool dwc = pw2_w6 && tune().x6r_dwc != 0 && d == 256;
  if (!dwc) WN_TRY(dwconv_ln_silu(dw, s));
  *ln_ff_done = pw2_w6 || c.rowln;
  if (pw2_w6) {
    void* ff_img = t1_image_for(m, L.ff1, L.ff2, ACT_SILU);
    X6RArgs g = x6r_rowln_args(c, L.pw2, pw2_w6, t1, L.norm_ff, 1);
    if (dwc) { g.dw = dw; g.dw_on = 1; }
    if (ff_img) { g.y3 = ff_img; g.y = nullptr; }
    if (gemm_x6r(g, s) != 0) return -2;
    m->t1_img_ok = ff_img != nullptr;
    return 0;
  }
  if (c.rowln) return rowln_gemm(c, L.pw2, t1, L.norm_ff);
  return linear(L.pw2, t1, d, x, d, M, s, ACT_NONE, x, d);
}

int final_ffn(const LayerCtx& c, const EncLayer& L, const EncLayer* Ln, bool ln_ff_done) {
  wn_model* m = c.m;
  const int d = c.d, M = c.M;
  hipStream_t s = c.s;
  int fS = 0;
  if (c.f32) {
    if (!ln_ff_done) WN_TRY(ln(L.norm_ff, c.x, c.t1, M, d, c.eps, s));
    fS = ffn_fused_try(m, L.ff1, L.ff2, ACT_SILU, s);
    if (fS < 0) return -2;
  }
  if (fS > 0) {
    const float* P = m->ffn_part.as<float>();
    if (!Ln)
      return ffn_reduce_ln(c.x, P, fS, L.ff2.b, 0.5f, L.norm_final.w, L.norm_final.b, nullptr,
                           nullptr, nullptr, M, d, c.eps, 2, s);
    void* mac_img = t1_image_for(m, Ln->ffm1, Ln->ffm2, ACT_SILU);
    if (!mac_img)
      return ffn_reduce_ln(c.x, P, fS, L.ff2.b, 0.5f, L.norm_final.w, L.norm_final.b,
                           Ln->norm_ff_mac.w, Ln->norm_ff_mac.b, c.t1, M, d, c.eps, 1, s);
    WN_TRY(ffn_reduce_ln_img(c.x, P, fS, L.ff2.b, 0.5f, L.norm_final.w, L.norm_final.b,
                             Ln->norm_ff_mac.w, Ln->norm_ff_mac.b, mac_img, M, d, c.eps, s));
    m->t1_img_ok = true;
    return 0;
  }
  WN_TRY(ffn_module(m, L.norm_ff, L.ff1, L.ff2, ACT_SILU, 0.5f, c.f32, c.h16, s));
  if (Ln && !(t_mx && c.h16))
    return layernorm2(c.x, L.norm_final.w, L.norm_final.b, Ln->norm_ff_mac.w, Ln->norm_ff_mac.b,
                      c.x, c.t1, M, d, c.eps, s, c.h16);
  return ln(L.norm_final, c.x, c.x, M, d, c.eps, s);
}

}

int encoder_layers(wn_model* m, int chunk, int left, hipStream_t s) {
  const ModelData& W = *m->data;
  const wn_config& cfg = m->cfg;
  const LayerCtx c(m, chunk, left, s);
  const int n_run = m->dbg_layers >= 0 ? std::min(m->dbg_layers, cfg.n_layers) : cfg.n_layers;
  m->t1_img_ok = false;
  for (int li = 0; li < n_run; ++li) {
    const EncLayer& L = W.layers[li];
    const void* qkv_w6 = x6r_image(c, L.qkv, 3 * c.d, 0);
    int pro_S = 0;
    bool ln_ff_done = false;
    WN_TRY(macaron_ffn(c, L, li, qkv_w6 != nullptr, &pro_S));
    WN_TRY(self_attention(c, L, qkv_w6, pro_S));
    WN_TRY(conv_module(c, L, &ln_ff_done));
    WN_TRY(final_ffn(c, L, li + 1 < n_run ? &W.layers[li + 1] : nullptr, ln_ff_done));
  }
  return after_norm_out(m, s);
}

int encoder_layers_chunk(wn_model* m, int n_sess, int R, const int* offsets,
                         std::vector<ChunkSess>& sess, float* out, hipStream_t s) {
  const ModelData& W = *m->data;
  const wn_config& c = m->cfg;
  const int d = c.d_model, H = c.n_heads, M = n_sess * R;
  const int lorder = c.causal ? c.cnn_kernel - 1 : 0;
  const int LR = lorder + R;
  float* x = m->x.as<float>();
  float* t1 = m->t1.as<float>();
  float* t2 = m->t2.as<float>();
  float* hb = m->hbuf.as<float>();
  float* qkv = m->qkv.as<float>();
  const float eps = c.norm_eps;
  std::vector<int> qoff(n_sess), qlen(n_sess, R), kvoff(n_sess), kvlen(n_sess), poff(n_sess),
      coff(n_sess), clen(n_sess, LR), rowutt((size_t)n_sess * LR);
  std::vector<int64_t> pw2_rows((size_t)M);
  int total_kv = 0, max_tk = 0;
  for (int b = 0; b < n_sess; ++b) {
    const int tk = sess[b].t1 + R;
    qoff[b] = b * R;
    kvoff[b] = total_kv; kvlen[b] = tk;
    sess[b].kv_off = total_kv;
    total_kv += tk; max_tk = std::max(max_tk, tk);
    poff[b] = offsets[b] - sess[b].t1;
    coff[b] = b * LR;
    for (int r = 0; r < LR; ++r) rowutt[(size_t)b * LR + r] = b;
    for (int r = 0; r < R; ++r) pw2_rows[(size_t)b * R + r] = ((int64_t)b * LR + lorder + r) * d;
  }
  WN_TRY(m->ck_kv.ensure((size_t)total_kv * 2 * d * sizeof(float)));
  WN_TRY(m->ck_xext.ensure((size_t)n_sess * LR * d * sizeof(float)));
  WN_TRY(m->ck_glu.ensure((size_t)n_sess * LR * d * sizeof(float)));
  WN_TRY(m->stage.begin((size_t)(n_sess * (LR + 8) + 64) * sizeof(int) +
                        (size_t)M * sizeof(int64_t) + n_sess * sizeof(ChunkSess) + 4096));
  WN_TRY(upload_desc(m, m->ck_desc, qoff, s));
  WN_TRY(upload_desc(m, m->r_qlen, qlen, s));
  WN_TRY(upload_desc(m, m->r_kvoff, kvoff, s));
  WN_TRY(upload_desc(m, m->r_kvlen, kvlen, s));
  WN_TRY(upload_desc(m, m->r_pos, poff, s));
  WN_TRY(upload_desc(m, m->r_qoff, coff, s));
  WN_TRY(upload_desc(m, m->r_tgt, clen, s));
  WN_TRY(upload_desc(m, m->ck_rowutt, rowutt, s));
  WN_TRY(m->stage.put(m->d_a_row_off, pw2_rows.data(), pw2_rows.size() * sizeof(int64_t), s));
  WN_TRY(m->stage.put(m->ck_sess, sess.data(), sess.size() * sizeof(ChunkSess), s));
  WN_TRY(m->stage.end(s));
  const ChunkSess* dsess = m->ck_sess.as<ChunkSess>();
  float* kv = m->ck_kv.as<float>();
  float* xext = m->ck_xext.as<float>();
  float* glu = m->ck_glu.as<float>();
  for (int li = 0; li < c.n_layers; ++li) {
    const EncLayer& L = W.layers[li];
    WN_TRY(ln(L.norm_ff_mac, x, t1, M, d, eps, s));
    WN_TRY(linear(L.ffm1, t1, d, hb, c.ffn_dim, M, s, ACT_SILU));
    WN_TRY(linear(L.ffm2, hb, c.ffn_dim, x, d, M, s, ACT_NONE, x, d, 0.5f));
    WN_TRY(ln(L.norm_mha, x, t1, M, d, eps, s));
    WN_TRY(linear(L.qkv, t1, d, qkv, 3 * d, M, s));
    WN_TRY(chunk_kv_assemble(dsess, n_sess, li, max_tk, qkv, R, H, kv, s));
    AttnArgs a;
    a.Q = qkv; a.ldq = 3 * d;
    a.K = kv; a.V = kv + d; a.ldk = a.ldv = 2 * d;
    a.P = L.pos_tab; a.ldp = d; a.p_off = m->r_pos.as<int>();
    a.bias_u = L.bias_u; a.bias_v = L.bias_v;
    a.O = t2; a.ldo = d;
    a.q_off = m->ck_desc.as<int>(); a.q_len = m->r_qlen.as<int>();
    a.kv_off = m->r_kvoff.as<int>(); a.kv_len = m->r_kvlen.as<int>();
    a.n_seq = n_sess; a.n_heads = H; a.max_q_len = R;
    a.mask_mode = 0;
    a.scale = 1.0f / sqrtf(64.0f);
    WN_TRY(attention(a, s));
    WN_TRY(linear(L.out, t2, d, x, d, M, s, ACT_NONE, x, d));
    WN_TRY(ln(L.norm_conv, x, t1, M, d, eps, s));
    if (lorder > 0) {
      WN_TRY(chunk_conv_input(dsess, n_sess, li, t1, R, d, lorder, xext, s));
      WN_TRY(linear(L.pw1, xext, d, glu, d, n_sess * LR, s, ACT_NONE, nullptr, 0, 1.0f, true));
    } else {
      WN_TRY(linear(L.pw1, t1, d, glu, d, M, s, ACT_NONE, nullptr, 0, 1.0f, true));
    }
    DwConvArgs dw;
    dw.x = glu; dw.ldx = d; dw.wt = L.dw_wt; dw.bias = L.dw_b; dw.cpad = L.cpad;
    dw.ln_w = L.conv_norm.w; dw.ln_b = L.conv_norm.b; dw.norm_mode = c.cnn_norm;
// ... 22 lines not shown
```

wenet_amd/csrc/ffn_fused.hip:

```cpp
#include "common.h"
#include "gemm_epilogue.h"
#include "kernels.h"
#include "x6.h"

namespace wn {

namespace {

typedef int i32x4 __attribute__((ext_vector_type(4)));

constexpr int FBM = 128;
constexpr int FHC = 64;
constexpr int STG = 32768;
constexpr int HC_BYTES = FBM * FHC * 4;

template <int ND, int ACT, int RING>
__global__ __launch_bounds__(512) void ffn_fused_kernel(FfnArgs p) {
  extern __shared__ __attribute__((aligned(16))) char smem_f[];
  typedef __attribute__((address_space(3))) void* lds_ptr;
  constexpr int D = 256 * ND;
  constexpr int NA = D / 32;
  constexpr int NB = (FHC / 32) * ND;
  constexpr int SPC = NA + NB;
  char* hc = smem_f + RING * STG;
// ... 147 lines not shown
        if (ACT == ACT_RELU) x = fmaxf(x, 0.f);
        if (ACT == ACT_GELU) x = 0.5f * x * (1.0f + erff(x * 0.70710678118654752f));
        const int row = wmA * 32 + (r & 3) + 8 * (r >> 2) + 4 * hi;
        *reinterpret_cast<float*>(hc + row * 256 + ((((col >> 2) ^ (row & 15))) << 4) +
                                  (col & 3) * 4) = x;
      }
    }
    asm volatile("s_waitcnt lgkmcnt(0)" ::: "memory");
    __builtin_amdgcn_s_barrier();
    FragB xb0 = loadB(g, 0, 0), xb1 = loadB(g, 0, 1);
#pragma unroll
    for (int j = 0; j < NB; ++j, ++g) {
      const int kt = j / ND, nd = j % ND;
      auto mmaB = [&](const FragB& f) {
#pragma unroll
        for (int s = 0; s < 4; ++s)
#pragma unroll
          for (int mt = 0; mt < 2; ++mt)
#pragma unroll
            for (int nt = 0; nt < 2; ++nt)
              yacc[nd][mt][nt] = __builtin_amdgcn_mfma_f32_32x32x2f32(
                  f.a[mt][s], f.b[nt][s], yacc[nd][mt][nt], 0, 0, 0);
      };
      const FragB yb0 = loadB(g, kt, 2), yb1 = loadB(g, kt, 3);
      mmaB(xb0); mmaB(xb1);
      mid_barrier(g);
      if (j + 1 < NB) {
        xb0 = loadB(g + 1, (j + 1) / ND, 0);
        xb1 = loadB(g + 1, (j + 1) / ND, 1);
      } else if (c + 1 < nchunk) {
        xa0 = loadA(g + 1, 0);
        xa1 = loadA(g + 1, 1);
      }
      mmaB(yb0); mmaB(yb1);
    }
  }
  asm volatile("s_waitcnt vmcnt(0)" ::: "memory");

  float* P = p.P + (int64_t)slice * p.M * D;
#pragma unroll
  for (int nd = 0; nd < ND; ++nd)
#pragma unroll
    for (int mt = 0; mt < 2; ++mt)
#pragma unroll
      for (int nt = 0; nt < 2; ++nt) {
        const int col = nd * 256 + wnB * 64 + nt * 32 + li;
        const int row0 = m0 + wmB * 64 + mt * 32 + 4 * hi;
#pragma unroll
        for (int r = 0; r < 16; ++r) {
          const int row = row0 + (r & 3) + 8 * (r >> 2);
          if (row < p.M) P[(int64_t)row * D + col] = yacc[nd][mt][nt][r];
        }
      }
}


template <int E, int MODE>
__global__ __launch_bounds__(256) void ffn_reduce_ln_kernel(
    float* __restrict__ x, const float* __restrict__ P, int S, const float* __restrict__ b2,
    float alpha, const float* __restrict__ w, const float* __restrict__ b,
    const float* __restrict__ w2, const float* __restrict__ bb2, float* __restrict__ y,
    int M, float eps) {
  static_assert(E % 4 == 0, "4 columns per lane and chunk");
  constexpr int D = E * 64;
  const int lane = threadIdx.x & 63;
  const int row = blockIdx.x * 4 + (threadIdx.x >> 6);
  if (row >= M) return;
  float v[E];
#pragma unroll
  for (int j = 0; j < E / 4; ++j) {
    const int c = j * 256 + lane * 4;
    f32x4 acc = *reinterpret_cast<const f32x4*>(b2 + c);
    int s = 0;
    for (; s + 8 <= S; s += 8) {
      f32x4 t[8];
#pragma unroll
      for (int u = 0; u < 8; ++u)
        t[u] = *reinterpret_cast<const f32x4*>(P + ((int64_t)(s + u) * M + row) * D + c);
#pragma unroll
      for (int u = 0; u < 8; ++u) acc += t[u];
    }
    for (; s < S; ++s)
      acc += *reinterpret_cast<const f32x4*>(P + ((int64_t)s * M + row) * D + c);
    const f32x4 xo = *reinterpret_cast<const f32x4*>(x + (int64_t)row * D + c);
#pragma unroll
    for (int e = 0; e < 4; ++e) v[4 * j + e] = xo[e] + alpha * acc[e];
  }
  auto store = [&](float* dst) {
#pragma unroll
    for (int j = 0; j < E / 4; ++j)
      *reinterpret_cast<f32x4*>(dst + (int64_t)row * D + j * 256 + lane * 4) =
          f32x4{v[4 * j], v[4 * j + 1], v[4 * j + 2], v[4 * j + 3]};
  };
  auto norm = [&](const float* gw, const float* gb) {
    float s = 0.f;
#pragma unroll
    for (int e = 0; e < E; ++e) s += v[e];
    const float mean = wave_sum(s) * (1.0f / D);
    float q = 0.f;
#pragma unroll
    for (int e = 0; e < E; ++e) {
      const float d = v[e] - mean;
      q = __builtin_fmaf(d, d, q);
    }
    const float rstd = 1.0f / sqrtf(wave_sum(q) * (1.0f / D) + eps);
#pragma unroll
    for (int j = 0; j < E / 4; ++j) {
      const f32x4 ww = *reinterpret_cast<const f32x4*>(gw + j * 256 + lane * 4);
      const f32x4 bv = *reinterpret_cast<const f32x4*>(gb + j * 256 + lane * 4);
#pragma unroll
      for (int e = 0; e < 4; ++e) v[4 * j + e] = (v[4 * j + e] - mean) * rstd * ww[e] + bv[e];
    }
  };
  if (MODE == 0) {
    store(x);
    norm(w, b);
    store(y);
  } else if (MODE == 1) {
    norm(w, b);
    store(x);
    norm(w2, bb2);
    store(y);
  } else {
    norm(w, b);
    store(x);
  }
}

template <int E>
__global__ __launch_bounds__(256) void ffn_reduce_ln_img_kernel(
    float* __restrict__ x, const float* __restrict__ P, int S, const float* __restrict__ b2,
    float alpha, const float* __restrict__ w, const float* __restrict__ b,
    const float* __restrict__ w2, const float* __restrict__ bb2, char* __restrict__ y3,
    int M, float eps) {
  static_assert(E % 4 == 0, "4 columns per lane and chunk");
  constexpr int D = E * 64;
  constexpr int NP = D / 8;
  constexpr int SEG = 144;
  __shared__ __attribute__((aligned(16))) char planes[3 * NP * SEG];
  const int lane = threadIdx.x & 63, wave = threadIdx.x >> 6;
  const int m0 = blockIdx.x * 8;
  for (int rr = 0; rr < 2; ++rr) {
    const int rl = wave * 2 + rr;
    const int row = m0 + rl;
    if (row >= M) continue;
    float v[E];
#pragma unroll
    for (int j = 0; j < E / 4; ++j) {
      const int c = j * 256 + lane * 4;
      f32x4 acc = *reinterpret_cast<const f32x4*>(b2 + c);
      int s = 0;
      for (; s + 8 <= S; s += 8) {
        f32x4 t[8];
#pragma unroll
        for (int u = 0; u < 8; ++u)
          t[u] = *reinterpret_cast<const f32x4*>(P + ((int64_t)(s + u) * M + row) * D + c);
#pragma unroll
        for (int u = 0; u < 8; ++u) acc += t[u];
      }
      for (; s < S; ++s)
        acc += *reinterpret_cast<const f32x4*>(P + ((int64_t)s * M + row) * D + c);
      const f32x4 xo = *reinterpret_cast<const f32x4*>(x + (int64_t)row * D + c);
#pragma unroll
      for (int e = 0; e < 4; ++e) v[4 * j + e] = xo[e] + alpha * acc[e];
    }
    auto norm = [&](const float* gw, const float* gb) {
      float sm = 0.f;
#pragma unroll
      for (int e = 0; e < E; ++e) sm += v[e];
      const float mean = wave_sum(sm) * (1.0f / D);
      float q = 0.f;
#pragma unroll
      for (int e = 0; e < E; ++e) {
        const float d = v[e] - mean;
        q = __builtin_fmaf(d, d, q);
      }
      const float rstd = 1.0f / sqrtf(wave_sum(q) * (1.0f / D) + eps);
#pragma unroll
      for (int j = 0; j < E / 4; ++j) {
        const f32x4 ww = *reinterpret_cast<const f32x4*>(gw + j * 256 + lane * 4);
        const f32x4 bv = *reinterpret_cast<const f32x4*>(gb + j * 256 + lane * 4);
#pragma unroll
        for (int e = 0; e < 4; ++e) v[4 * j + e] = (v[4 * j + e] - mean) * rstd * ww[e] + bv[e];
      }
    };
    norm(w, b);
#pragma unroll
    for (int j = 0; j < E / 4; ++j)
      *reinterpret_cast<f32x4*>(x + (int64_t)row * D + j * 256 + lane * 4) =
          f32x4{v[4 * j], v[4 * j + 1], v[4 * j + 2], v[4 * j + 3]};
    norm(w2, bb2);
#pragma unroll
    for (int j = 0; j < E / 4; ++j) {
      bf16x4 h0, h1, h2;
#pragma unroll
      for (int e = 0; e < 4; ++e) {
        const Split3 sp = split3(v[4 * j + e]);
        h0[e] = sp.h0; h1[e] = sp.h1; h2[e] = sp.h2;
      }
      const int piece = (j * 16 + (lane >> 2)) * 2 + ((lane >> 1) & 1);
      char* o = planes + piece * SEG + rl * 16 + (lane & 1) * 8;
      *reinterpret_cast<bf16x4*>(o) = h0;
      *reinterpret_cast<bf16x4*>(o + NP * SEG) = h1;
      *reinterpret_cast<bf16x4*>(o + 2 * NP * SEG) = h2;
    }
  }
  __syncthreads();
  const int tiles = (M + 31) >> 5, tile = m0 >> 5, r32 = m0 & 31;
#pragma unroll
  for (int it = 0; it < 3 * NP * 8 / 256; ++it) {
    const int q = it * 256 + threadIdx.x;
    const int rl = q & 7, ph = q >> 3;
    const int pl = ph / NP, kh = ph - pl * NP;
    if (m0 + rl < M) {
      const f32x4 val = *reinterpret_cast<const f32x4*>(planes + ph * SEG + rl * 16);
      *reinterpret_cast<f32x4*>(y3 + ((int64_t)(kh >> 1) * tiles + tile) * X3_TILE + pl * X3_REC +
                                (kh & 1) * 512 + (r32 + rl) * 16) = val;
    }
  }
}

}


int ffn_fused_split(int M, int D, int F) {
  const int tiles_m = cdiv(M, FBM), cap = 256;
  int S = 1;
  while (S < 16 && tiles_m * (S * 2) <= cap && F % (S * 2 * FHC) == 0) S *= 2;
  while (F / S / FHC > 16) {
    if (F % (S * 2 * FHC) != 0) return 0;
    S *= 2;
  }
  return S;
}

bool ffn_fused_supported(int M, int D, int F, int act) {
  if (!(D == 256 || D == 512) || F % FHC != 0 || M <= 0) return false;
  if (act != ACT_SILU && act != ACT_RELU && act != ACT_GELU) return false;
  if ((int64_t)M * D * 4 >= (int64_t(1) << 31) || (int64_t)F * D * 4 >= (int64_t(1) << 31))
    return false;
  const int S = ffn_fused_split(M, D, F);
  if (S <= 0) return false;
  return tune().ffn_fused == 2 || cdiv(M, FBM) * S >= 128;
}

template <int ND, int ACT>
int launch_ffn(const FfnArgs& a, hipStream_t s) {
  const size_t lds = (size_t)4 * STG + HC_BYTES;
  const dim3 grid(cdiv(a.M, FBM) * a.S), blk(512);
  auto kern = ffn_fused_kernel<ND, ACT, 4>;
  WN_MAX_DYN_LDS(kern, lds);
  hipLaunchKernelGGL(kern, grid, blk, lds, s, a);
  WN_HIP(hipGetLastError());
  return 0;
}

int ffn_fused(const FfnArgs& a, hipStream_t s) {
  WN_CHECK(a.X && a.W1 && a.b1 && a.W2 && a.P && a.S > 0 && a.F % (a.S * FHC) == 0 &&
               a.F / a.S / FHC <= 16, "ffn_fused: bad arguments");
  WN_CHECK(a.D == 256 || a.D == 512, "ffn_fused: d_model 256 or 512");
#define WN_FFN(ND)                                                         \
  switch (a.act) {                                                         \
    case ACT_SILU: return launch_ffn<ND, ACT_SILU>(a, s);                  \
    case ACT_RELU: return launch_ffn<ND, ACT_RELU>(a, s);                  \
    case ACT_GELU: return launch_ffn<ND, ACT_GELU>(a, s);                  \
    default: break;                                                        \
  }
  if (a.D == 256) { WN_FFN(1) } else { WN_FFN(2) }
#undef WN_FFN
  set_error("ffn_fused: unsupported activation");
  return -1;
}

int ffn_reduce_ln(float* x, const float* P, int S, const float* b2, float alpha,
                  const float* w, const float* b, const float* w2, const float* bb2, float* y,
                  int M, int D, float eps, int mode, hipStream_t s) {
  WN_CHECK(M > 0 && (D == 256 || D == 512) && mode >= 0 && mode <= 2, "ffn_reduce_ln: shape");
  dim3 g(cdiv(M, 4)), t(256);
#define WN_RL(E, MODE)                                                                 \
  hipLaunchKernelGGL((ffn_reduce_ln_kernel<E, MODE>), g, t, 0, s, x, P, S, b2, alpha, w, b, \
                     w2, bb2, y, M, eps)
  if (D == 256) {
    if (mode == 0) WN_RL(4, 0); else if (mode == 1) WN_RL(4, 1); else WN_RL(4, 2);
  } else {
    if (mode == 0) WN_RL(8, 0); else if (mode == 1) WN_RL(8, 1); else WN_RL(8, 2);
  }
#undef WN_RL
  WN_HIP(hipGetLastError());
  return 0;
}

int ffn_reduce_ln_img(float* x, const float* P, int S, const float* b2, float alpha,
                      const float* w, const float* b, const float* w2, const float* bb2,
                      void* y3, int M, int D, float eps, hipStream_t s) {
  WN_CHECK(M > 0 && (D == 256 || D == 512) && y3 && w2 && bb2, "ffn_reduce_ln_img: shape");
  if (D == 256)
    hipLaunchKernelGGL(ffn_reduce_ln_img_kernel<4>, dim3(cdiv(M, 8)), dim3(256), 0, s, x, P, S,
                       b2, alpha, w, b, w2, bb2, reinterpret_cast<char*>(y3), M, eps);
  else
    hipLaunchKernelGGL(ffn_reduce_ln_img_kernel<8>, dim3(cdiv(M, 8)), dim3(256), 0, s, x, P, S,
                       b2, alpha, w, b, w2, bb2, reinterpret_cast<char*>(y3), M, eps);
  WN_HIP(hipGetLastError());
  return 0;
}

}
```

wenet_amd/csrc/kernels.h:

```cpp
#pragma once
#include "common.h"

namespace wn {

int layernorm(const float* x, int ldx, const float* w, const float* b, float* y,
              int ldy, int M, int D, float eps, hipStream_t s, bool y_bf16 = false);

int layernorm_mx(const float* x, int ldx, const float* w, const float* b, void* q,
                 unsigned* scale, int pitch, int M, int D, float eps, hipStream_t s);

int layernorm2(const float* x, const float* w1, const float* b1, const float* w2,
               const float* b2, float* y1, float* y2, int M, int D, float eps,
               hipStream_t s, bool y2_bf16 = false);

struct Conv1Args {
  const float* feats;
  const float* mean;
  const float* istd;
  const float* w;
  const float* bias;
  float* out;
  char* out3 = nullptr;
  int tiles = 0;
  const int* t1_off;
// ... 58 lines not shown
  int nw = 2;
  bool relpos = false;
  bool in16 = false;
  bool kbias = false;
  int code() const {
    return kind | ks << 4 | nw << 8 | (int)relpos << 12 | (int)in16 << 13 | (int)kbias << 14;
  }
};
AttnForm attention_form(const AttnArgs& a);
AttnForm attention_bf16_form(const AttnArgs& a);
size_t attention_x6_image_bytes(int rows, int n_seq, int n_heads);
bool attention_x6_supported(const AttnArgs& a);
int attention_x6(const AttnArgs& a, hipStream_t s);
int relpos_fold(float* K, int ldk, const float* P, int ldp, const float* bias_u,
                const float* bias_v, const int* row_utt, const int* off, const int* p_off,
                float* kbias, int n_heads, int M, int D, hipStream_t s);
int attention_bf16(const AttnArgs& a, hipStream_t s);

struct RelShiftAttnArgs {
  const float* Q; const float* K; const float* V;
  int ldq, ldk, ldv;
  const float* P; int ldp;
  int p_center, p_rows;
  const float* bias_u; const float* bias_v;
  float* O; int ldo;
  const int* off; const int* len;
  int n_seq, n_heads, max_len;
  float scale = 0.125f;
};
int attention_relshift(const RelShiftAttnArgs& a, hipStream_t s);

struct FireRedFrontArgs {
  const float* feats;
  const float* mean;
  const float* istd;
  const float* w1;
  const float* b1;
  const float* w2;
  const float* b2;
  float* h1;
  float* out; int ldo;
  const int* len;
  const int* t1_off; const int* t1_len;
  const int* t2_off; const int* t2_len;
  int B, T, F, F1, F2, C, max_t2;
};
int firered_frontend(const FireRedFrontArgs& a, hipStream_t s);

constexpr int CSGU_TILE = 32;
constexpr int CSGU_MAX_K = 63;
constexpr int CSGU_MAX_C = 1024;
struct DwTileArgs {
  const float* x; int ldx;
  const float* wt;
  const float* bias;
  float* y; int ldy;
  const int* off; const int* len;
  int B, C, K, causal, max_len;
  const float* ln_w = nullptr; const float* ln_b = nullptr;
  float2* stats = nullptr; int M = 0; float eps = 1e-5f;
  const float* r = nullptr; int ldr = 0;
};
int csgu_gate(const DwTileArgs& a, hipStream_t s);
int merge_dwconv(const DwTileArgs& a, hipStream_t s);
int csgu_mul(const float* r, int ldr, const float* g, int ldg, float* y, int ldy, int M, int C,
             hipStream_t s);

struct FfnArgs {
  const float* X;
  const float* W1;
  const float* b1;
  const float* W2;
  float* P;
  int M, D, F, S, act;
};
int ffn_fused_split(int M, int D, int F);
bool ffn_fused_supported(int M, int D, int F, int act);
int ffn_fused(const FfnArgs& a, hipStream_t s);
int ffn_reduce_ln(float* x, const float* P, int S, const float* b2, float alpha,
                  const float* w, const float* b, const float* w2, const float* bb2, float* y,
                  int M, int D, float eps, int mode, hipStream_t s);
int ffn_reduce_ln_img(float* x, const float* P, int S, const float* b2, float alpha,
                      const float* w, const float* b, const float* w2, const float* bb2,
                      void* y3, int M, int D, float eps, hipStream_t s);

struct X6Args {
  const void* A3 = nullptr;
  const float* A = nullptr; int lda = 0; int64_t a_bytes = 0;
  const void* B3 = nullptr;
  int M = 0, N = 0, K = 0;
  int row0 = 0;
  int ksplit = 1;
  int bm = 0;
  int nw = 0;
  int epi = 0;
  const float* bias = nullptr;
  const float* resid = nullptr; int ldr = 0;
  float alpha = 1.0f; int act = 0;
  float* C = nullptr; int ldc = 0;
  void* C3 = nullptr;
  const int* a_pix = nullptr;
  int a_tiles = 0, conv_kbc = 0;
  int conv_taps = 0;
  int tap_delta[9] = {0, 0, 0, 0, 0, 0, 0, 0, 0};
  int probe = 0;
  float* part = nullptr; size_t part_bytes = 0;
};
int gemm_x6_clocks(unsigned long long* out);
size_t x6_bytes(int R, int K);
int x6_split(const float* src, int R, int K, int ld, void* dst, hipStream_t s);
int gemm_x6_bm(int M, int N, int ksplit);
int gemm_x6(const X6Args& a, hipStream_t s);
enum X6ConvTile {
  X6CONV_128 = 0,
  X6CONV_256 = 1,
  X6CONV_256_REM128 = 2,
  X6CONV_256_KTAIL = 3
};
struct X6ConvForm {
  int tile = X6CONV_128;
  int full = 0;
  int slices = 0;
};
X6ConvForm gemm_x6_conv_form(const X6Args& a);
struct FfnX6Args {
  const float* X = nullptr;
  int ldx = 0;
  const void* X3 = nullptr;
  const void* W13 = nullptr;
  const void* W2p = nullptr;
  const float* b1 = nullptr;
  float* P = nullptr;
  int M = 0, D = 0, F = 0, S = 0, act = 0;
};
int ffn_x6f_clocks(unsigned long long* out);
int x6_split_perm(const float* src, int R, int K, int ld, void* dst, hipStream_t s);
int ffn_x6f_split(int M, int F);
bool ffn_x6f_supported(int M, int D, int F, int act);
int ffn_x6f(const FfnX6Args& a, hipStream_t s);


struct RowLnArgs {
  const float* A; int lda;
  const float* W;
  const float* bias;
  const float* resid; int ldr;
  float alpha;
  float* x_out; int ldx;
  const float* ln_w; const float* ln_b; float eps;
  float* y; int ldy;
  int M, N, K;
};
struct X6RArgs {
  const float* A = nullptr; int lda = 0;
  int K = 256;
  const void* W3 = nullptr;
  const float* bias = nullptr;
  int M = 0, N = 0;
  int epi = 0;
  float* C = nullptr; int ldc = 0;
  const float* resid = nullptr; int ldr = 0; float alpha = 1.0f;
  float* x_out = nullptr; int ldx = 0;
  const float* ln_w = nullptr; const float* ln_b = nullptr; float eps = 1e-5f;
  float* y = nullptr; int ldy = 0;
  void* y3 = nullptr;
  const void* W3b = nullptr; const float* bias2 = nullptr;
  const float* pro_P = nullptr; int pro_S = 0; const float* pro_b2 = nullptr;
// ... 398 lines not shown
```

wenet_amd/csrc/model.hip:

```cpp
#include <algorithm>
#include "model_state.h"

namespace wn {

static thread_local std::string g_error;
void set_error(const std::string& msg) { g_error = msg; }
const char* last_error_cstr() { return g_error.c_str(); }

}

thread_local const std::map<const float*, ModelData::MxW>* t_mx = nullptr;
thread_local const std::map<const float*, const void*>* t_x6 = nullptr;
thread_local DevBuf* t_x6_a = nullptr;

namespace wn {
Tune g_tune_default;
thread_local const Tune* t_tune = nullptr;

int* tune_field(Tune& t, const std::string& key) {
#define X(name, dflt) if (key == #name) return &t.name;
  WN_TUNE_KEYS(X)
#undef X
  return nullptr;
}
// ... 9 lines not shown
    set_error(std::string(who) + ": x6_probe 1 / 2 (no MFMAs / no DMA) need a WN_ABLATION build");
    return -1;
  }
  if (key == "ffn_x6f_var" && value != 0 && value != 25088) {
    set_error(std::string(who) + ": ffn_x6f_var variants other than the clock-stamp form "
              "(25088) need a WN_ABLATION build");
    return -1;
  }
  if (key == "attn_x6_var" && value != 0) {
    set_error(std::string(who) + ": attn_x6_var needs a WN_ABLATION build");
    return -1;
  }
  if (key == "ffn_x6f_ring" && value != 3) {
    set_error(std::string(who) + ": ffn_x6f_ring needs a WN_ABLATION build");
    return -1;
  }
#endif
  return 0;
}

void tune_resolve(const Tune& ovr, Tune* eff) {
#define X(name, dflt) eff->name = ovr.name != TUNE_INHERIT ? ovr.name : g_tune_default.name;
  WN_TUNE_KEYS(X)
#undef X
}

Tune tune_all_inherit() {
  Tune t;
#define X(name, dflt) t.name = TUNE_INHERIT;
  WN_TUNE_KEYS(X)
#undef X
  return t;
}
}


bool bf16_store_active() {
  return t_gemm_prec == PREC_BF16 && tune().bf16_store != 0 && tune().attn_bf16 != 0 &&
         t_wslab_bf16 != nullptr;
}

int upload_desc(wn_model* m, DevBuf& buf, const std::vector<int>& v,
                hipStream_t s) {
  return m->stage.put(buf, v.data(), v.size() * sizeof(int), s);
}

thread_local bool t_linear_took_x6 = false;

int linear(const Linear& l, const float* A, int lda, float* C, int ldc, int M,
           hipStream_t s, int act, const float* resid, int ldr, float alpha, bool glu, bool a_bf16,
           bool c_bf16) {
  if (t_gemm_prec == PREC_F32 && tune().gemm_x6 != 0 && tune().x6_linear != 0 && t_x6 && t_x6_a && !glu &&
      !a_bf16 && !c_bf16 && l.in % 16 == 0 && l.out % 4 == 0 && lda % 4 == 0 && ldc % 4 == 0 &&
      (resid == nullptr || ldr % 4 == 0) && M >= 512 &&
      2.0 * M * (double)l.out * l.in >= 1e8 * g_x6_linear_min) {
    auto it = t_x6->find(l.w);
    if (it != t_x6->end()) {
      t_linear_took_x6 = true;
      WN_TRY(t_x6_a->ensure(x6_bytes(M, l.in)));
      WN_TRY(x6_split(A, M, l.in, lda, t_x6_a->as<char>(), s));
      X6Args x;
      x.A3 = t_x6_a->as<char>(); x.B3 = it->second; x.M = M; x.N = l.out; x.K = l.in;
      x.epi = 0; x.bias = l.b; x.resid = resid; x.ldr = ldr; x.alpha = alpha; x.act = act;
      x.C = C; x.ldc = ldc;
      return gemm_x6(x, s);
    }
  }
  t_linear_took_x6 = false;
  GemmArgs g;
  g.A = A; g.W = l.w; g.bias = l.b; g.C = C; g.resid = resid;
  g.M = M; g.N = l.out; g.K = l.in; g.lda = lda; g.ldc = ldc; g.ldr = ldr;
  g.alpha = alpha; g.act = act; g.glu = glu;
  g.a_bf16 = a_bf16; g.c_bf16 = c_bf16;
  return gemm_f32(g, s);
}

int ln(const Norm& n, const float* x, float* y, int M, int D, float eps,
       hipStream_t s, bool y_bf16) {
  return layernorm(x, D, n.w, n.b, y, D, M, D, eps, s, y_bf16);
}

int after_norm_out(wn_model* m, hipStream_t s) {
  const int d = m->cfg.d_model, M = m->rows;
  WN_TRY(m->enc.ensure((size_t)std::max(M, 1) * d * sizeof(float)));
  if (m->dbg_skip_after_norm) {
    WN_HIP(hipMemcpyAsync(m->enc.p, m->x.p, (size_t)M * d * sizeof(float),
                          hipMemcpyDeviceToDevice, s));
    return 0;
  }
  return ln(m->data->after_norm, m->x.as<float>(), m->enc.as<float>(), M, d, m->cfg.norm_eps, s);
}

int build_x6_images(const wn_config& cfg, ModelData& W, bool skip_encoder) {
  std::vector<const Linear*> ws;
  static const std::vector<EncLayer> no_layers;
  const std::vector<EncLayer>& enc_layers = skip_encoder ? no_layers : W.layers;
  for (const auto& L : enc_layers) { ws.push_back(&L.ffm1); ws.push_back(&L.ffm2);
                                    ws.push_back(&L.ff1); ws.push_back(&L.ff2);
                                    ws.push_back(&L.qkv); ws.push_back(&L.out);
                                    ws.push_back(&L.pw2); ws.push_back(&L.pw1); }
  for (const Decoder* D : {&W.left, &W.right})
    for (const auto& L : D->layers) {
      ws.push_back(&L.self_qkv); ws.push_back(&L.self_out); ws.push_back(&L.src_q);
      ws.push_back(&L.src_kv); ws.push_back(&L.src_out); ws.push_back(&L.ff1);
      ws.push_back(&L.ff2);
    }
  for (const auto& L : W.tf_layers) { ws.push_back(&L.qkv); ws.push_back(&L.out);
                                       ws.push_back(&L.ff1); ws.push_back(&L.ff2); }
  if (W.conv2.w && !skip_encoder) ws.push_back(&W.conv2);
  if (W.sub_out.w && !skip_encoder) ws.push_back(&W.sub_out);
  std::vector<const Linear*> vocab;
  if (W.ctc.w) vocab.push_back(&W.ctc);
  for (const Decoder* D : {&W.left, &W.right})
    if (D->out.w) vocab.push_back(&D->out);
  for (const Linear* l : vocab) ws.push_back(l);
  size_t bytes = 0;
  for (const Linear* l : ws)
    if (l->w && l->in % 16 == 0) bytes += x6_bytes(l->out, l->in);
  if (bytes > 0) {
    WN_TRY(W.weights_x6.ensure(bytes));
    char* p = W.weights_x6.as<char>();
    for (const Linear* l : ws) {
      if (!l->w || l->in % 16 != 0 || W.x6_at.count(l->w)) continue;
      WN_TRY(x6_split(l->w, l->out, l->in, l->in, p, nullptr));
      W.x6_at[l->w] = p;
      p += x6_bytes(l->out, l->in);
    }
  }
  if (cfg.d_model == 256) {
    std::vector<const Linear*> w2s;
    for (const auto& L : enc_layers) { w2s.push_back(&L.ffm2); w2s.push_back(&L.ff2); }
    size_t pbytes = 0;
    for (const Linear* l : w2s)
      if (l->w && l->in % 64 == 0 && l->out == 256) pbytes += x6_bytes(l->out, l->in);
    if (pbytes > 0) {
      WN_TRY(W.weights_x6p.ensure(pbytes));
      char* q = W.weights_x6p.as<char>();
      for (const Linear* l : w2s) {
        if (!l->w || l->in % 64 != 0 || l->out != 256 || W.x6p_at.count(l->w)) continue;
        WN_TRY(x6_split_perm(l->w, l->out, l->in, l->in, q, nullptr));
        W.x6p_at[l->w] = q;
        q += x6_bytes(l->out, l->in);
      }
    }
  }
  if (cfg.d_model == 256 && cfg.n_heads == 4) {
    size_t n_q = 0;
    for (const auto& L : enc_layers)
      if (L.qkv.w && L.qkv.b && L.qkv.out == 768 && L.qkv.in == 256 && L.pos_tab) ++n_q;
    if (n_q > 0) {
      const size_t img = x6_bytes(768, 256), per = img + 768 * sizeof(float);
      DevBuf stage;
      WN_TRY(stage.ensure((size_t)768 * 256 * sizeof(float)));
      WN_TRY(W.weights_x6q.ensure(n_q * per));
      char* q = W.weights_x6q.as<char>();
      for (const auto& L : enc_layers) {
        if (!(L.qkv.w && L.qkv.b && L.qkv.out == 768 && L.qkv.in == 256 && L.pos_tab) ||
            W.x6q_at.count(L.qkv.w))
          continue;
        float* qb = reinterpret_cast<float*>(q + img);
        for (int h = 0; h < 4; ++h)
          for (int part = 0; part < 3; ++part) {
            const size_t nr = (size_t)h * 192 + part * 64, orow = (size_t)part * 256 + h * 64;
            WN_HIP(hipMemcpyAsync(stage.as<float>() + nr * 256, L.qkv.w + orow * 256,
                                  64 * 256 * sizeof(float), hipMemcpyDeviceToDevice, nullptr));
            WN_HIP(hipMemcpyAsync(qb + nr, L.qkv.b + orow, 64 * sizeof(float),
                                  hipMemcpyDeviceToDevice, nullptr));
          }
        WN_TRY(x6_split(stage.as<float>(), 768, 256, 256, q, nullptr));
        W.x6q_at[L.qkv.w] = {q, qb};
        q += per;
      }
      WN_HIP(hipStreamSynchronize(nullptr));
    }
  }
  size_t b4_floats = 0;
  for (const Linear* l : vocab)
    if (l->b && l->out % 4 != 0) b4_floats += (size_t)(l->out + 3) / 4 * 4;
  if (b4_floats > 0) {
    WN_TRY(W.bias4_buf.ensure(b4_floats * sizeof(float)));
    WN_HIP(hipMemsetAsync(W.bias4_buf.p, 0, b4_floats * sizeof(float), nullptr));
    float* q = W.bias4_buf.as<float>();
    for (const Linear* l : vocab) {
      if (!l->b || l->out % 4 == 0 || W.bias4.count(l->w)) continue;
      WN_HIP(hipMemcpyAsync(q, l->b, (size_t)l->out * sizeof(float), hipMemcpyDeviceToDevice,
                            nullptr));
      W.bias4[l->w] = q;
      q += (l->out + 3) / 4 * 4;
    }
  }
  return 0;
}

int vocab_linear(wn_model* m, const Linear& l, const float* A, int lda, float* C, int ldc,
                 int M, hipStream_t s) {
  const ModelData& W = *m->data;
  const int V = l.out, V4 = (V + 3) / 4 * 4;
  WN_CHECK(ldc >= V4 && ldc % 4 == 0, "vocab_linear: pitch");
  const void* w6 = nullptr;
  const float* bias = l.b;
  if (t_gemm_prec == PREC_F32 && tune().gemm_x6 != 0 && tune().x6_linear != 0 &&
      l.in % 16 == 0 && lda % 4 == 0 && M >= 512) {
    auto it = W.x6_at.find(l.w);
    if (it != W.x6_at.end()) w6 = it->second;
    if (w6 && V != V4 && l.b) {
      bias = nullptr;
      auto ib = W.bias4.find(l.w);
      if (ib != W.bias4.end()) bias = ib->second;
      if (!bias) w6 = nullptr;
    }
  }
  if (!w6) return linear(l, A, lda, C, ldc, M, s);
  WN_TRY(m->x6_lin.ensure(x6_bytes(M, l.in)));
  WN_TRY(x6_split(A, M, l.in, lda, m->x6_lin.as<char>(), s));
  X6Args x;
  x.A3 = m->x6_lin.as<char>(); x.B3 = w6; x.M = M; x.N = V4; x.K = l.in;
  x.epi = 0; x.bias = bias; x.C = C; x.ldc = ldc;
  return gemm_x6(x, s);
}

namespace wn {
namespace {

__global__ void build_conv2_pix_kernel(const int* row_utt2, const int* off2, const int* off1,
                                       int M, int F1, int F2, int fstep, int* a_pix) {
  const int i = blockIdx.x * blockDim.x + threadIdx.x;
  if (i >= M * F2) return;
  const int g = i / F2, f2 = i % F2;
  const int u = row_utt2[g];
  a_pix[i] = (off1[u] + 2 * (g - off2[u])) * F1 + fstep * f2;
}

__global__ void build_conv2_rows_kernel(const int* row_utt2, const int* off2,
                                        const int* off1, int M, int F1, int F2,
                                        int C, int64_t* a_row_off) {
  const int i = blockIdx.x * blockDim.x + threadIdx.x;
  if (i >= M * F2) return;
  const int g = i / F2, f2 = i % F2;
  const int u = row_utt2[g];
  const int t2 = g - off2[u];
  const int64_t t1 = off1[u] + 2 * t2;
  a_row_off[i] = (t1 * F1 + 2 * f2) * (int64_t)C;
}

__global__ void scatter_padded_kernel(const float* src, int lds, const int* off,
                                      const int* len, int Tp, int D4,
                                      float* dst) {
  const int b = blockIdx.y, t = blockIdx.x;
  f32x4* d = reinterpret_cast<f32x4*>(dst + ((int64_t)b * Tp + t) * D4 * 4);
  if (t < len[b]) {
    const f32x4* s =
        reinterpret_cast<const f32x4*>(src + (int64_t)(off[b] + t) * lds);
    for (int i = threadIdx.x; i < D4; i += blockDim.x) d[i] = s[i];
  } else {
    const f32x4 z = {0.f, 0.f, 0.f, 0.f};
    for (int i = threadIdx.x; i < D4; i += blockDim.x) d[i] = z;
  }
}

__global__ void pad_feats_kernel(const float* feats, int T, int F, const int* seg_off,
                                 const int* len, const float* mean,
                                 const float* istd, float* xpad) {
  const int b = blockIdx.y, j = blockIdx.x;
  const int L = len[b];
  if (j >= L + 3) return;
  float* dst = xpad + (int64_t)(seg_off[b] + j) * F;
  const int t = j - 1;
  if (t >= 0 && t < L) {
    const float* src = feats + ((int64_t)b * T + t) * F;
    for (int i = threadIdx.x; i < F; i += blockDim.x) {
      float v = src[i];
      if (mean) v = (v - mean[i]) * istd[i];
      dst[i] = v;
    }
  } else {
    for (int i = threadIdx.x; i < F; i += blockDim.x) dst[i] = 0.f;
  }
}

__global__ void zero_rows_kernel(float* base, int D4, const int* rows, int n) {
  const int r = blockIdx.x;
  if (r >= n) return;
  f32x4* d = reinterpret_cast<f32x4*>(base + (int64_t)rows[r] * D4 * 4);
  const f32x4 z = {0.f, 0.f, 0.f, 0.f};
  for (int i = threadIdx.x; i < D4; i += blockDim.x) d[i] = z;
}

}
}

int scatter_padded(const float* src, int lds, const int* off, const int* len, int B, int Tp, int D,
                   float* dst, hipStream_t s) {
  hipLaunchKernelGGL(scatter_padded_kernel, dim3(Tp, B), dim3(64), 0, s, src, lds, off, len, Tp,
                     D / 4, dst);
  WN_HIP(hipGetLastError());
  return 0;
}

int set_layout(wn_model* m, int B, int Tp, const std::vector<int>& off,
               const std::vector<int>& len, int rows, hipStream_t s) {
  m->B = B; m->Tp = Tp; m->off = off; m->len = len; m->rows = rows;
  m->mem_cache_valid = false;
  if (m->kv_ready) {
    (void)hipStreamWaitEvent(s, m->side.e1, 0);
    m->kv_ready = false;
  }
  std::vector<int> row_utt(std::max(rows, 1), -1);
  for (int b = 0; b < B; ++b)
    for (int t = 0; t < len[b]; ++t) row_utt[off[b] + t] = b;
  m->attn_blk_off = (int)((row_utt.size() + 15) / 16 * 16);
  m->attn_n_blk = 0;
  {
    const int H = m->cfg.n_heads;
    std::vector<int> order(B);
    for (int b = 0; b < B; ++b) order[b] = b;
    std::stable_sort(order.begin(), order.end(), [&](int x, int y) { return len[x] > len[y]; });
    std::vector<int> tab;
    if (B < 65536 && H < 256)
      for (int light = 0; light < 2; ++light)
        for (int b : order) {
          const int nqb = (len[b] + 63) / 64;
          for (int qb = 0; qb < nqb && qb < 256; ++qb) {
            const bool is_light = len[b] - qb * 64 <= 32;
            if ((int)is_light != light) continue;
            for (int h = 0; h < H; ++h) tab.push_back((b << 16) | (h << 8) | qb);
          }
        }
    row_utt.resize(m->attn_blk_off + tab.size(), -1);
    std::copy(tab.begin(), tab.end(), row_utt.begin() + m->attn_blk_off);
    m->attn_n_blk = (int)tab.size();
  }
  WN_TRY(m->stage.begin((size_t)(row_utt.size() + 4 * B + 64) * sizeof(int) + 1024));
  WN_TRY(upload_desc(m, m->d_off, off, s));
  WN_TRY(upload_desc(m, m->d_len, len, s));
  WN_TRY(upload_desc(m, m->d_row_utt, row_utt, s));
  m->ctc_valid = false;
  return 0;
}

int sub_out_linear(wn_model* m, int M, int F2, hipStream_t s) {
  const ModelData& W = *m->data;
  const wn_config& c = m->cfg;
  const int d = c.d_model, K = F2 * d;
  if (t_gemm_prec != PREC_F32 || tune().gemm_x6 == 0 || W.layers.empty() ||
      (d != 256 && d != 512) || K % 16 != 0 || M < 512 || (int64_t)M * K * 4 >= ((int64_t)1 << 31) ||
      bf16_store_active())
    return 0;
  auto it = W.x6_at.find(W.sub_out.w);
  if (it == W.x6_at.end()) return 0;
  const int bm = 256;
  const int tiles = cdiv(M, bm) * cdiv(d, 256), nkb = K / 16;
  int S = 0;
  for (int t = std::min(16, 256 / std::max(tiles, 1)); t >= 2; --t)
    if (nkb % t == 0) { S = t; break; }
  if (S < 2) return 0;
  WN_TRY(m->ffn_part.ensure((size_t)S * M * d * sizeof(float)));
  X6Args g;
  g.A = m->c2.as<float>(); g.lda = K; g.a_bytes = (int64_t)M * K * 4;
  g.B3 = it->second; g.M = M; g.N = d; g.K = K; g.epi = 1; g.ksplit = S; g.bm = bm;
  g.C = m->ffn_part.as<float>();
  WN_TRY(gemm_x6(g, s));
  WN_HIP(hipMemsetAsync(m->x.p, 0, (size_t)M * d * sizeof(float), s));
  const EncLayer& L0 = W.layers[0];
  WN_TRY(ffn_reduce_ln(m->x.as<float>(), m->ffn_part.as<float>(), S, W.sub_out.b, sqrtf((float)d),
                       L0.norm_ff_mac.w, L0.norm_ff_mac.b, nullptr, nullptr, m->t1.as<float>(), M,
                       d, c.norm_eps, 0, s));
  m->ln0_done = true;
  return 1;
}

int encode_gate_wait(wn_model* m, hipStream_t s) {
  if (m->enc_gate) {
    hipEvent_t e = m->enc_gate;
    m->enc_gate = nullptr;
    WN_HIP(hipStreamWaitEvent(s, e, 0));
  }
  return 0;
}

int conv2_kind(const wn_model* m, int M, int M1, const void** w6) {
  const ModelData& W = *m->data;
  const int d = m->cfg.d_model, F1 = m->F1(), F2 = m->F2();
  *w6 = nullptr;
  if (t_gemm_prec == PREC_F32 && tune().gemm_x6 != 0 && d % 32 == 0 &&
      F1 <= 64 &&
      (M * F2 >= 4096 || tune().gemm_x6 == 2)) {
    auto it = W.x6_at.find(W.conv2.w);
    if (it != W.x6_at.end()) *w6 = it->second;
  }
  if (*w6 && (tune().x6_af32 != 0 || tune().x6_conv_af32 != 0) &&
      (int64_t)M1 * F1 * d * 4 < ((int64_t)1 << 31))
    return CONV2_X6_AF32;
  return *w6 ? CONV2_X6_PLANES : CONV2_GEMM_F32;
}

int subsample_conv2d4(wn_model* m, const float* feats_dev,
                      const int32_t* feat_lens_host, int B, int T,
                      int32_t* enc_lens_host, int pos0, hipStream_t s) {
  const ModelData& W = *m->data;
  const wn_config& c = m->cfg;
  const int d = c.d_model, F1 = m->F1(), F2 = m->F2();
  const int Tp = ((T - 1) / 2 - 1) / 2;
  m->ln0_done = false;
  m->front_route = 0;
  WN_CHECK(pos0 + Tp <= c.max_pos, "utterance longer than the positional table");
  std::vector<int> off2(B), len2(B), off1(B), len1(B);
  int M = 0, M1 = 0, max_t1 = 0;
  for (int b = 0; b < B; ++b) {
    const int L = feat_lens_host[b];
    WN_CHECK(L >= 0 && L <= T, "wn_encode: feature length out of range");
    const int l2 = L > 6 ? (L - 7) / 4 + 1 : 0;
    off2[b] = M; len2[b] = l2; M += l2;
    const int l1 = l2 > 0 ? 2 * l2 + 1 : 0;
    off1[b] = M1; len1[b] = l1; M1 += l1;
    max_t1 = std::max(max_t1, l1);
    if (enc_lens_host) enc_lens_host[b] = l2;
  }
  WN_TRY(set_layout(m, B, Tp, off2, len2, M, s));
  if (M == 0) WN_TRY(m->stage.end(s));
  if (M > 0) {
    WN_TRY(upload_desc(m, m->d_off1, off1, s));
    WN_TRY(upload_desc(m, m->d_len1, len1, s));
    WN_TRY(m->stage.end(s));
    if (tune().enc_gate_pos == 0) WN_TRY(encode_gate_wait(m, s));
    WN_TRY(m->c1.ensure((size_t)M1 * F1 * d * sizeof(float)));
    WN_TRY(m->c2.ensure((size_t)M * F2 * d * sizeof(float)));
    WN_TRY(m->x.ensure((size_t)M * d * sizeof(float)));
    WN_TRY(m->t1.ensure((size_t)M * d * sizeof(float)));
    WN_TRY(m->t2.ensure((size_t)M * d * sizeof(float)));
    WN_TRY(m->hbuf.ensure((size_t)M * c.ffn_dim * sizeof(float)));
    WN_TRY(m->qkv.ensure((size_t)M * 3 * d * sizeof(float)));
    WN_TRY(m->d_a_row_off.ensure((size_t)M * F2 * sizeof(int64_t)));
    const void* w6 = nullptr;
    const int kind = conv2_kind(m, M, M1, &w6);
    if (kind == CONV2_X6_AF32) {
      WN_TRY(m->c1.ensure((size_t)M1 * F1 * d * sizeof(float)));
      Conv1Args c1;
      c1.feats = feats_dev; c1.mean = W.cmvn_mean; c1.istd = W.cmvn_istd;
      c1.w = W.conv1_w; c1.bias = W.conv1_b; c1.out = m->c1.as<float>();
      c1.t1_off = m->d_off1.as<int>(); c1.t1_len = m->d_len1.as<int>();
      c1.B = B; c1.T = T; c1.F = c.feat_dim; c1.F1 = F1; c1.C = d; c1.max_t1 = max_t1;
      WN_TRY(cmvn_conv1_relu(c1, s));
      int* pix = reinterpret_cast<int*>(m->d_a_row_off.as<int64_t>());
      hipLaunchKernelGGL(build_conv2_pix_kernel, dim3(cdiv(M * F2, 256)), dim3(256), 0, s,
                         m->d_row_utt.as<int>(), m->d_off.as<int>(), m->d_off1.as<int>(), M,
                         F1, F2, 2, pix);
      WN_HIP(hipGetLastError());
      X6Args g;
      g.A = m->c1.as<float>(); g.a_bytes = (int64_t)M1 * F1 * d * 4;
      g.B3 = w6; g.M = M * F2; g.N = d; g.K = 9 * d;
      g.epi = 0; g.bias = W.conv2.b; g.act = ACT_RELU; g.C = m->c2.as<float>(); g.ldc = d;
      g.a_pix = pix; g.conv_kbc = d / 16;
      for (int ky = 0; ky < 3; ++ky)
        for (int kx = 0; kx < 3; ++kx) g.tap_delta[ky * 3 + kx] = ky * F1 + kx;
      const X6ConvForm form = gemm_x6_conv_form(g);
      WN_TRY(gemm_x6(g, s));
      WN_TRY(linear(W.sub_out, m->c2.as<float>(), F2 * d, m->x.as<float>(), d, M,
                    s, ACT_NONE, nullptr, 0, sqrtf((float)d)));
      m->front_route = front_route_code(kind, form, false, t_linear_took_x6);
      return 0;
    }
    if (kind == CONV2_X6_PLANES) {
      const int tiles = cdiv(M1 * F1, 32);
      WN_TRY(m->c1.ensure(x6_bytes(M1 * F1, d)));
      Conv1Args c1;
      c1.feats = feats_dev; c1.mean = W.cmvn_mean; c1.istd = W.cmvn_istd;
      c1.w = W.conv1_w; c1.bias = W.conv1_b; c1.out = nullptr;
      c1.out3 = m->c1.as<char>(); c1.tiles = tiles;
      c1.t1_off = m->d_off1.as<int>(); c1.t1_len = m->d_len1.as<int>();
      c1.B = B; c1.T = T; c1.F = c.feat_dim; c1.F1 = F1; c1.C = d; c1.max_t1 = max_t1;
      WN_TRY(cmvn_conv1_relu(c1, s));
      int* pix = reinterpret_cast<int*>(m->d_a_row_off.as<int64_t>());
      hipLaunchKernelGGL(build_conv2_pix_kernel, dim3(cdiv(M * F2, 256)), dim3(256), 0, s,
                         m->d_row_utt.as<int>(), m->d_off.as<int>(), m->d_off1.as<int>(), M,
                         F1, F2, 1, pix);
      WN_HIP(hipGetLastError());
      WN_TRY(encode_gate_wait(m, s));
      X6Args g;
      g.A3 = m->c1.as<char>(); g.B3 = w6; g.M = M * F2; g.N = d; g.K = 9 * d;
      g.epi = 0; g.bias = W.conv2.b; g.act = ACT_RELU; g.C = m->c2.as<float>(); g.ldc = d;
      g.a_pix = pix; g.a_tiles = tiles; g.conv_kbc = d / 16;
      g.conv_taps = 9;
      {
        const int ncu = 256;
        const int t256 = cdiv(M * F2, 256), rem = t256 - t256 / ncu * ncu;
        if (d <= 256 && t256 >= ncu && rem > 0 && rem <= ncu / 2) {
// ... 36 lines not shown
    g.act = ACT_RELU; g.a_row_off = m->d_a_row_off.as<int64_t>();
    g.conv_C = d; g.conv_sy = (int64_t)F1 * d; g.conv_sx = d;
    WN_TRY(gemm_f32(g, s));
    WN_TRY(linear(W.sub_out, m->c2.as<float>(), F2 * d, m->x.as<float>(), d, M,
                  s, ACT_NONE, nullptr, 0, sqrtf((float)d)));
    m->front_route = front_route_code(kind, X6ConvForm(), false, t_linear_took_x6);
  }
  return 0;
}

int transformer_layers(wn_model* m, hipStream_t s) {
  const ModelData& W = *m->data;
  const wn_config& c = m->cfg;
  const int d = c.d_model, M = m->rows;
  float* x = m->x.as<float>();
  float* t1 = m->t1.as<float>();
  float* t2 = m->t2.as<float>();
  float* hb = m->hbuf.as<float>();
  float* qkv = m->qkv.as<float>();
  const float eps = c.norm_eps;
  int max_len = 0;
  for (int b = 0; b < m->B; ++b) max_len = std::max(max_len, m->len[b]);
  const int act = c.activation == 1 ? ACT_GELU : ACT_SILU;
  const bool h16 = bf16_store_active();
  const int n_run = m->dbg_layers >= 0 ? std::min(m->dbg_layers, c.n_layers)
                                      : c.n_layers;
  for (int li = 0; li < n_run; ++li) {
    const TfLayer& L = W.tf_layers[li];
    WN_TRY(ln(L.n1, x, t1, M, d, eps, s, h16));
    const bool q16 = h16 && tune().qkv_bf16 != 0;
    WN_TRY(linear(L.qkv, t1, d, qkv, 3 * d, M, s, ACT_NONE, nullptr, 0, 1.0f, false,
                  h16, q16));
    AttnArgs a;
    if (q16) {
      const __bf16* qh = reinterpret_cast<const __bf16*>(qkv);
      a.Q = reinterpret_cast<const float*>(qh);
      a.K = reinterpret_cast<const float*>(qh + d);
      a.V = reinterpret_cast<const float*>(qh + 2 * d);
      a.qkv_bf16 = true;
    } else {
      a.Q = qkv; a.K = qkv + d; a.V = qkv + 2 * d;
    }
    a.ldq = a.ldk = a.ldv = 3 * d;
    a.O = t2; a.ldo = d; a.o_bf16 = h16;
    a.q_off = a.kv_off = m->d_off.as<int>();
    a.q_len = a.kv_len = m->d_len.as<int>();
    a.n_seq = m->B; a.n_heads = c.n_heads; a.max_q_len = max_len;
    a.mask_mode = 0;
    a.scale = 1.0f / sqrtf(64.0f);
    WN_TRY(attention(a, s));
    WN_TRY(linear(L.out, t2, d, x, d, M, s, ACT_NONE, x, d, 1.0f, false, h16));
    WN_TRY(ffn_module(m, L.n2, L.ff1, L.ff2, act, 1.0f, false, h16, s));
  }
  return after_norm_out(m, s);
}

int encode_transformer(wn_model* m, const float* feats_dev,
                       const int32_t* feat_lens_host, int B, int T,
                       float* enc_out_dev, int32_t* enc_lens_host, hipStream_t s) {
  const ModelData& W = *m->data;
  const wn_config& c = m->cfg;
  const int d = c.d_model, F = c.feat_dim;
  const int Tp = (T - 1) / 2 + 1;
  const int par = (T + 1) % 2;
  WN_CHECK(Tp <= c.max_pos, "utterance longer than the positional table");
  std::vector<int> seg(B), off2(B), len2(B), lens(B);
  int rows_pad = 0, M = 0;
  std::vector<int> zero_rows;
  for (int b = 0; b < B; ++b) {
    const int L = feat_lens_host[b];
    WN_CHECK(L >= 0 && L <= T, "wn_encode: feature length out of range");
    lens[b] = L;
    seg[b] = rows_pad;
    rows_pad += L + 3;
    const int l2 = L > par ? (L - par + 1) / 2 : 0;
    off2[b] = M; len2[b] = l2; M += l2;
    if (enc_lens_host) enc_lens_host[b] = l2;
    zero_rows.push_back(seg[b]);
    if (L == T) zero_rows.push_back(seg[b] + 1 + L);
  }
  m->B = B; m->Tp = Tp; m->off = off2; m->len = len2; m->rows = M;
  m->ctc_valid = false;
  m->mem_cache_valid = false;
  if (m->kv_ready) {
    (void)hipStreamWaitEvent(s, m->side.e1, 0);
    m->kv_ready = false;
  }
  if (M == 0) {
    WN_TRY(m->stage.begin((size_t)B * 16 + 1024));
    WN_TRY(upload_desc(m, m->d_off, off2, s));
    WN_TRY(upload_desc(m, m->d_len, len2, s));
    WN_TRY(m->stage.end(s));
  } else {
    std::vector<int64_t> a_off((size_t)M);
    std::vector<int> row_t((size_t)M);
    for (int b = 0; b < B; ++b)
      for (int t = 0; t < len2[b]; ++t) {
        a_off[off2[b] + t] = (int64_t)(seg[b] + 2 * t) * d;
        row_t[off2[b] + t] = t;
      }
    WN_TRY(m->stage.begin((size_t)M * 16 + (size_t)B * 64 * 5 + zero_rows.size() * 4 +
                          64 * 12 + 4096));
    WN_TRY(upload_desc(m, m->d_off, off2, s));
    WN_TRY(upload_desc(m, m->d_len, len2, s));
    {
      std::vector<int> row_utt(M, -1);
      for (int b = 0; b < B; ++b)
        for (int t = 0; t < len2[b]; ++t) row_utt[off2[b] + t] = b;
      WN_TRY(upload_desc(m, m->d_row_utt, row_utt, s));
      m->attn_n_blk = 0;
    }
    WN_TRY(upload_desc(m, m->d_off1, seg, s));
    WN_TRY(upload_desc(m, m->d_len1, lens, s));
    WN_TRY(upload_desc(m, m->d_row_t, row_t, s));
    WN_TRY(upload_desc(m, m->d_zero_rows, zero_rows, s));
    WN_TRY(m->stage.put(m->d_a_row_off, a_off.data(), a_off.size() * sizeof(int64_t), s));
    WN_TRY(m->stage.end(s));
    const int K1 = W.tconv1.in;
    WN_TRY(m->xpad.ensure(((size_t)rows_pad * F + K1 + 64) * sizeof(float)));
    WN_TRY(m->c1.ensure(((size_t)rows_pad + 2) * d * sizeof(float)));
    WN_TRY(m->x.ensure((size_t)M * d * sizeof(float)));
    WN_TRY(m->t1.ensure((size_t)M * d * sizeof(float)));
    WN_TRY(m->t2.ensure((size_t)M * d * sizeof(float)));
    WN_TRY(m->pos_rows.ensure((size_t)M * d * sizeof(float)));
    WN_TRY(m->hbuf.ensure((size_t)M * c.ffn_dim * sizeof(float)));
    WN_TRY(m->qkv.ensure((size_t)M * 3 * d * sizeof(float)));
    int max_len = 0;
    for (int b = 0; b < B; ++b) max_len = std::max(max_len, lens[b]);
    WN_HIP(hipMemsetAsync(m->xpad.as<float>() + (size_t)rows_pad * F, 0,
                          (size_t)(K1 + 64) * sizeof(float), s));
    hipLaunchKernelGGL(pad_feats_kernel, dim3(max_len + 3, B), dim3(64), 0, s,
                       feats_dev, T, F, m->d_off1.as<int>(), m->d_len1.as<int>(),
                       W.cmvn_mean, W.cmvn_istd, m->xpad.as<float>());
    WN_HIP(hipGetLastError());
    GemmArgs g1;
    g1.A = m->xpad.as<float>(); g1.W = W.tconv1.w; g1.bias = W.tconv1.b;
    g1.C = m->c1.as<float>() + d; g1.M = rows_pad - 2; g1.N = d; g1.K = K1;
    g1.lda = F; g1.ldc = d; g1.act = ACT_GELU;
    WN_CHECK(F % 4 == 0, "conv1d2 front end: feature dim must be a multiple of 4");
    WN_TRY(gemm_f32(g1, s));
    hipLaunchKernelGGL(zero_rows_kernel, dim3((unsigned)zero_rows.size()), dim3(64), 0,
                       s, m->c1.as<float>(), d / 4, m->d_zero_rows.as<int>(),
                       (int)zero_rows.size());
    WN_HIP(hipGetLastError());
    WN_TRY(copy_rows(W.pe, d, m->d_row_t.as<int>(), m->pos_rows.as<float>(), d,
                     nullptr, M, d, s));
    GemmArgs g2;
    g2.A = m->c1.as<float>(); g2.W = W.tconv2.w; g2.bias = W.tconv2.b;
    g2.C = m->x.as<float>(); g2.M = M; g2.N = d; g2.K = 3 * d; g2.ldc = d;
    g2.act = ACT_GELU; g2.resid = m->pos_rows.as<float>(); g2.ldr = d;
    g2.a_row_off = m->d_a_row_off.as<int64_t>();
    g2.conv_C = 3 * d; g2.conv_sy = 0; g2.conv_sx = 0;
    WN_TRY(gemm_f32(g2, s));
    WN_TRY(transformer_layers(m, s));
  }
  if (enc_out_dev) {
    if (M > 0) {
      WN_TRY(scatter_padded(m->enc.as<float>(), d, m->d_off.as<int>(), m->d_len.as<int>(), B, Tp,
                            d, enc_out_dev, s));
    } else if (Tp > 0) {
      WN_HIP(hipMemsetAsync(enc_out_dev, 0, (size_t)B * Tp * d * sizeof(float), s));
    }
  }
  return 0;
}

// ... 1 lines not shown
```

wenet_amd/csrc/model_state.h:

```cpp
#pragma once
#include <math.h>
#include <stdio.h>
#include <stdlib.h>
#include <string.h>

#include <atomic>
#include <chrono>
#include <map>
#include <memory>
#include <mutex>
#include <string>
#include <vector>

#include "../../include/wenet_amd.h"
#include "kernels.h"

namespace wn {

const char* last_error_cstr();


struct DevBuf {
  void* p = nullptr;
  size_t cap = 0;
// ... 179 lines not shown
  DevBuf weights_x6q;
  std::map<const float*, std::pair<const void*, const float*>> x6q_at;
  DevBuf bias4_buf;
  std::map<const float*, const float*> bias4;
  std::map<std::string, const float*> w;
  const float* conv1_w = nullptr; const float* conv1_b = nullptr;
  Linear conv2, sub_out;
  const float* cmvn_mean = nullptr; const float* cmvn_istd = nullptr;
  const float* pe = nullptr;
  Norm after_norm;
  Linear ctc;
  std::vector<EncLayer> layers;
  std::vector<TfLayer> tf_layers;
  Linear tconv1, tconv2;
  bool fbank_ok = true;
  Decoder left, right;
  DevBuf pos_tabs;
  struct LstmLayer { const float* w_ih; const float* w_hh; const float* b_ih; const float* b_hh; };
  const float* pred_embed = nullptr;
  std::vector<LstmLayer> pred_rnn;
  Linear pred_proj, j_enc, j_pred, j_out;
  const float* pred_pos = nullptr;
  const float* pred_conv_w = nullptr; const float* pred_conv_b = nullptr;
  Linear pred_ffn;
  Norm pred_norm;
  PfData pf;
  const float* fb_window = nullptr; const float* fb_twiddle = nullptr;
  const float* fb_mel_w = nullptr;
  DevBuf fb_tab_i;

  mutable std::mutex lazy;
  mutable DevBuf weights_bf16;
  struct MxW { const void* q; const unsigned* scale; };
  mutable DevBuf weights_mx;
  mutable std::map<const float*, MxW> mx_at;
  mutable bool mx_built = false;
  mutable DevBuf lm_dft;
  mutable std::map<int, DevBuf> lm_mel;
  mutable std::map<std::pair<int, int>, DevBuf> rs_taps;
};

struct wn_model {
  wn_config cfg;
  struct {
    bool on = false;
    wn_transducer_config c = {};
    wn_stateless_predictor_config sp = {};
  } tr;
  struct {
    bool on = false;
    wn_firered_config c = {};
  } fr;
  struct {
    bool on = false;
    wn_branchformer_config c = {};
  } bf;
  struct {
    bool on = false;
    wn_paraformer_config c = {};
  } pf;
  DevBuf pf_alpha, pf_img, pf_emb, pf_int, pf_x, pf_y, pf_t, pf_o, pf_q, pf_kv, pf_h, pf_out;
  PinnedBuf pf_host;
  int device = 0;
  std::shared_ptr<const ModelData> data = std::make_shared<ModelData>();
  bool fp8_ffn = false;
  DevBuf nb_map, nb_keep, nb_enc, nb_off_old;
  DevBuf x6_a, x6_h;
  DevBuf x6_lin;
  DevBuf mx_sa, mx_sh;

  int B = 0, Tp = 0, rows = 0;
  std::vector<int> off, len;
  DevBuf d_off, d_len, d_row_utt, d_off1, d_len1, d_a_row_off;
  DevBuf c1, c2, x, t1, t2, hbuf, qkv, enc;
  DevBuf bf_cat, bf_mrg, bf_gate, bf_stats;
  DevBuf ffn_part;
  DevBuf attn_kbias;
  DevBuf xpad, pos_rows, d_row_t, d_zero_rows;
  DevBuf ck_kv, ck_xext, ck_glu, ck_desc, ck_rowutt, ck_sess;
  DevBuf lm_off, lm_foff, lm_nfr, lm_rowutt, lm_frames, lm_spec, lm_pw, lm_melout, lm_umax;
  int ctc_rows = 0, ctc_k = 0;
  bool ctc_valid = false;
  bool ln0_done = false;
  int front_route = 0;
  DevBuf logits, topk_val, topk_idx;
  DevBuf pb_dbg;
  DevBuf g_tok, g_len, pb_pool;
  DevBuf pb_out;
  PinnedBuf pb_host;
  bool pb_valid = false;
  int pb_B = 0, pb_beam = 0, pb_max_len = 0;
  size_t pb_o_sc = 0, pb_o_nh = 0, pb_o_len = 0, pb_o_tok = 0;
  DevBuf al_desc, al_bp, al_out;
  PinnedBuf al_host;
  DevBuf r_tok, r_rtok, r_pos, r_tgt, r_rtgt, r_qoff, r_qlen, r_kvoff, r_kvlen;
  DevBuf r_x, r_t1, r_t2, r_qkv, r_h, r_mem, r_logits, r_out;
  DevBuf r_mem_all;
  DevBuf r_seqsrc, r_seqfirst;
  DevBuf r_gqoff, r_gqlen, r_gkvoff, r_gkvlen;
  DevBuf r_hyp;
  DevBuf r_res;
  PinnedBuf r_host;
  DevBuf ab_cache, ab_state;
  DevBuf ab_prompt;
  DevBuf sk_part;
  DevBuf tr_enc, tr_f32, tr_i32, tr_tok;
  DevBuf tr_ctc;
  int tr_beam_steps = 0;
  int64_t tr_beam_advance = 0;
  int64_t tr_score_rows = 0, tr_score_unshared = 0;
  int tr_score_nodes = 0;
  DevBuf tr_sc_f32, tr_sc_i32, tr_sc_logp;
  hipEvent_t tr_sc_ev[5] = {nullptr, nullptr, nullptr, nullptr, nullptr};
  float tr_score_ms[4] = {0.f, 0.f, 0.f, 0.f};
  PinnedBuf tr_host;
  hipEvent_t tr_ev[2] = {nullptr, nullptr};
  ~wn_model() {
    for (hipEvent_t e : tr_ev) if (e) (void)hipEventDestroy(e);
    for (hipEvent_t e : tr_sc_ev) if (e) (void)hipEventDestroy(e);
  }
  bool ab_truncated = false;
  bool mem_cache_valid = false;

  SideStream side;
  DevBuf r_kv_all, r_enc3;
  DevBuf attn_img;
  int attn_blk_off = 0, attn_n_blk = 0;
  DevBuf t1_img;
  bool t1_img_ok = false;
  bool kv_ready = false;
  hipEvent_t enc_gate = nullptr;
  int kv_rows = 0, kv_nl = 0, kv_nr = 0;
  Stager stage;
  std::vector<hipEvent_t> prof_ev;
  size_t prof_used = 0;
  bool prof_on = false;
  unsigned prof_seq = 0;
  unsigned prof_stride = 6;
  double prof_flops = 0.0;
  const char* prof_kernel = "gemm (FFN w_1)";
  int prof_split = 1;
  int prec = PREC_F32;
  std::atomic<bool> busy{false};
  Tune tune_ovr = tune_all_inherit();
  Tune tune_eff;
  int dbg_layers = -1;
  int dbg_skip_after_norm = 0;
  std::shared_ptr<DevBuf> ctx_buf;
  CtxGraph ctx;
  DevBuf fb_off, fb_nfr;

  int F1() const { return (cfg.feat_dim - 1) / 2; }
  int F2() const { return (F1() - 1) / 2; }
};


inline hipError_t stream_wait(hipStream_t s) {
  if (tune().sync_spin != 0) {
    const auto t0 = std::chrono::steady_clock::now();
    for (int i = 0;; ++i) {
      const hipError_t e = hipStreamQuery(s);
      if (e != hipErrorNotReady) return e;
      if ((i & 255) == 255 && std::chrono::steady_clock::now() - t0 > std::chrono::milliseconds(50)) break;
    }
  }
  return hipStreamSynchronize(s);
}

struct HandleGuard {
  wn_model* m;
  bool ok;
  const Tune* saved_tune;
  explicit HandleGuard(wn_model* m_) : m(m_), ok(false), saved_tune(t_tune) {
    bool expected = false;
    ok = m->busy.compare_exchange_strong(expected, true, std::memory_order_acquire);
    if (ok) {
      tune_resolve(m->tune_ovr, &m->tune_eff);
      t_tune = &m->tune_eff;
    }
  }
  ~HandleGuard() {
    if (ok) {
      t_tune = saved_tune;
      m->busy.store(false, std::memory_order_release);
    }
  }
};
#define WN_ENTER(m)                                                              \
  HandleGuard handle_guard(m);                                                   \
  if (!handle_guard.ok) {                                                        \
    ::wn::set_error("this wn_model handle is in use by another host thread; "    \
                    "one thread per handle (wn_model_clone gives a second one)"); \
    return -4;                                                                   \
  }

extern thread_local const std::map<const float*, ModelData::MxW>* t_mx;
extern thread_local const std::map<const float*, const void*>* t_x6;
extern thread_local DevBuf* t_x6_a;

struct PrecisionScope {
  int saved;
  const float* s_f32; const void* s_bf16; int64_t s_elems;
  const std::map<const float*, ModelData::MxW>* s_mx;
  const std::map<const float*, const void*>* s_x6; DevBuf* s_x6_a;
  explicit PrecisionScope(const wn_model* m)
      : saved(t_gemm_prec), s_f32(t_wslab_f32), s_bf16(t_wslab_bf16),
        s_elems(t_wslab_elems), s_mx(t_mx), s_x6(t_x6), s_x6_a(t_x6_a) {
    const ModelData& W = *m->data;
    t_mx = m->fp8_ffn ? &W.mx_at : nullptr;
    t_x6 = &W.x6_at;
    t_x6_a = const_cast<DevBuf*>(&m->x6_lin);
    t_gemm_prec = m->prec;
    const bool img = m->prec == PREC_BF16 && W.weights_bf16.p;
    t_wslab_f32 = img ? W.weights.as<float>() : nullptr;
    t_wslab_bf16 = img ? W.weights_bf16.p : nullptr;
    t_wslab_elems = img ? W.n_weight_elems : 0;
  }
  ~PrecisionScope() {
    t_gemm_prec = saved;
    t_wslab_f32 = s_f32; t_wslab_bf16 = s_bf16; t_wslab_elems = s_elems;
    t_mx = s_mx;
    t_x6 = s_x6; t_x6_a = s_x6_a;
  }
};


bool bf16_store_active();
int upload_desc(wn_model* m, DevBuf& buf, const std::vector<int>& v, hipStream_t s);
constexpr int g_x6_linear_min = 60;
extern thread_local bool t_linear_took_x6;
int linear(const Linear& l, const float* A, int lda, float* C, int ldc, int M, hipStream_t s,
           int act = ACT_NONE, const float* resid = nullptr, int ldr = 0, float alpha = 1.0f,
           bool glu = false, bool a_bf16 = false, bool c_bf16 = false);
int ln(const Norm& n, const float* x, float* y, int M, int D, float eps, hipStream_t s,
       bool y_bf16 = false);
int after_norm_out(wn_model* m, hipStream_t s);
int build_x6_images(const wn_config& cfg, ModelData& W, bool skip_encoder = false);
int vocab_linear(wn_model* m, const Linear& l, const float* A, int lda, float* C, int ldc, int M,
                 hipStream_t s);
int scatter_padded(const float* src, int lds, const int* off, const int* len, int B, int Tp, int D,
                   float* dst, hipStream_t s);
int set_layout(wn_model* m, int B, int Tp, const std::vector<int>& off,
               const std::vector<int>& len, int rows, hipStream_t s);
int subsample_conv2d4(wn_model* m, const float* feats_dev, const int32_t* feat_lens_host, int B,
                      int T, int32_t* enc_lens_host, int pos0, hipStream_t s);
int encode_gate_wait(wn_model* m, hipStream_t s);
enum Conv2Kind {
  CONV2_GEMM_F32 = 0,
  CONV2_X6_AF32 = 1,
  CONV2_X6_PLANES = 2
};
int conv2_kind(const wn_model* m, int M, int M1, const void** w6);
inline int front_route_code(int kind, const X6ConvForm& f, bool sub_out, bool linear_x6) {
  return kind | f.tile << 4 | f.slices << 8 | (int)sub_out << 12 | (int)linear_x6 << 13 | 1 << 16;
}
int ffn_module(wn_model* m, const Norm& nrm, const Linear& w1, const Linear& w2, int act,
               float alpha, bool ln_done, bool h16, hipStream_t s);
int ffn_x6_split(int M, int F);
int ffn_x6_pair(wn_model* m, const Linear& w1, const Linear& w2, int act, const float* A, int M,
                hipStream_t s);
int encoder_layers(wn_model* m, int chunk, int left, hipStream_t s);
int encoder_layers_chunk(wn_model* m, int n_sess, int R, const int* offsets,
                         std::vector<ChunkSess>& sess, float* out, hipStream_t s);
int encode_firered(wn_model* m, const float* feats_dev, const int32_t* feat_lens_host, int B, int T,
                   float* enc_out_dev, int32_t* enc_lens_host, hipStream_t s);
int encode_branchformer(wn_model* m, const float* feats_dev, const int32_t* feat_lens_host, int B,
                        int T, int chunk, int left, float* enc_out_dev, int32_t* enc_lens_host,
                        hipStream_t s);
int encode_paraformer(wn_model* m, const float* feats_dev, const int32_t* feat_lens_host, int B,
                      int T, float* enc_out_dev, int32_t* enc_lens_host, hipStream_t s);
int create_model_impl(const wn_config* cfg, const wn_transducer_config* tcfg,
                      const wn_stateless_predictor_config* scfg, const wn_firered_config* fcfg,
                      const wn_branchformer_config* bcfg, const wn_tensor* weights,
                      int32_t n_weights, int32_t device, wn_model** out);
int encode_transformer(wn_model* m, const float* feats_dev, const int32_t* feat_lens_host, int B,
                       int T, float* enc_out_dev, int32_t* enc_lens_host, hipStream_t s);
```

wenet_amd/csrc/tune.h:

```cpp
#pragma once
#include <stdint.h>

#include <string>

namespace wn {

#define WN_TUNE_KEYS(X)                                                                         \
                          \
  X(gemm_tile_bf16, 0)                                                                          \
                            \
  X(bf16_store, 1)                                                                              \
                      \
  X(lp_probe, 0)                                                                                \
                       \
  X(attn_split, 0)                                                                              \
                     \
  X(attn_bf16, 1)                                                                               \
                 \
  X(attn_bf16_nw, 0)                                                                            \
                                                                            \
  X(attn_bf16_defer, 80)                                                                        \
                                                              \
  X(attn_bf16_dma, 1)                                                                           \
                        \
  X(qkv_bf16, 1)                                                                                \
            \
  X(fp8_min_tiles, 192)                                                                         \
       \
  X(ffn_fused, 1)                                                                               \
                                                                   \
  X(gemm_x6, 1)                                                                                 \
                                         \
  X(x6_linear, 1)                                                                               \
                      \
  X(x6_af32, 0)                                                                                 \
            \
  X(x6_conv_af32, 0)                                                                            \
     \
  X(enc_gate_pos, 0)                                                                            \
                                                            \
  X(x6_conv_bm, 128)                                                                            \
                    \
  X(x6_probe, 0)                                                                                \
                     \
  X(ffn_x6f, 1)                                                                                 \
            \
  X(ffn_ximg, 1)                                                                                \
                             \
  X(ffn_x6f_ring, 3)                                                                            \
                  \
  X(ffn_x6f_var, 0)                                                                             \
                                                                        \
  X(x6r, 1)                                                                                     \
                  \
  X(x6r_chain, 1)                                                                               \
          \
  X(x6r_dwc, 1)                                                                                 \
        \
  X(x6r_pro, 1)                                                                                 \
            \
  X(x6r512_rows, 0)                                                                             \
                 \
  X(gemm_rowln, 1)                                                                              \
          \
  X(dwconv_tiled, 1)                                                                            \
                               \
  X(attn_x6, 1)                                                                                 \
                   \
  X(attn_xcd, 1)                                                                                \
        \
  X(attn_x6_galign, 2)                                                                          \
                             \
  X(attn_x6_order, 1)                                                                           \
    \
  X(attn_x6_var, 0)                                                                             \
        \
  X(attn_fold, 1)                                                                               \
                  \
  X(rescore_groups, 1)                                                                          \
                                                \
  X(rescore_prefetch, 1)                                                                        \
    \
  X(beam_weak_hash, 0)                                                                          \
                                                                              \
  X(beam_lds_pool, 1)                                                                           \
    \
  X(sync_spin, 1)                                                                               \
                         \
  X(ctc_wave, 1)                                                                                \
        \
  X(dec_skinny, 0)                                                                              \
                                            \
  X(rnnt_lookahead, 4)

struct Tune {
#define X(name, dflt) int name = dflt;
  WN_TUNE_KEYS(X)
#undef X
};

constexpr int32_t TUNE_INHERIT = INT32_MIN;

extern Tune g_tune_default;
extern thread_local const Tune* t_tune;
inline const Tune& tune() { return t_tune ? *t_tune : g_tune_default; }

int* tune_field(Tune& t, const std::string& key);
int tune_check(const std::string& key, int32_t value, const char* who);
void tune_resolve(const Tune& ovr, Tune* eff);
Tune tune_all_inherit();

}
```

Baseline: 71640.

## Emit bf16-plane images from fused reduce+LayerNorm at encoder head and tail

The last layer's final FFN reduce+LayerNorm kernel now also applies the after-norm and writes the three-plane bf16 image of the encoder output. The CTC vocab GEMM reads that image and skips its separate split pass and the standalone after-norm. The subsampling output reduce likewise writes layer 0's macaron-FFN input image directly, dropping a memset of x and letting layer 0 skip its split. The change also adds a host top-k copy API, a debug option that pre-fills the logits buffer, and a tunable CTC logits pitch; these add state flags that must be kept valid across calls.

```diff
diff --git a/include/wenet_amd.h b/include/wenet_amd.h
--- a/include/wenet_amd.h
+++ b/include/wenet_amd.h
@@ -105,6 +105,9 @@
 int wn_ctc_logprobs(wn_model* m, int32_t topk, int32_t blank_id,
                     float blank_penalty, float* logp_dev, int32_t Tp,
                     void* stream);
+
+int wn_ctc_topk_host(wn_model* m, float* val_host, int32_t* idx_host, int64_t capacity,
+                     int32_t* rows_out, int32_t* k_out, void* stream);
 
 int wn_set_ctc_probs(wn_model* m, const float* logp_dev,
                      const int32_t* lens_host, int32_t B, int32_t Tp,
diff --git a/wenet_amd/_lib.py b/wenet_amd/_lib.py
--- a/wenet_amd/_lib.py
+++ b/wenet_amd/_lib.py
@@ -94,7 +94,7 @@
     'wn_attention_beam_search', 'wn_attention_beam_search_prompt', 'wn_attention_truncated',
     'wn_op_gemm_skinny', 'wn_encode_chunk_batch', 'wn_op_gemm_lowp', 'wn_op_mx_quantize', 'wn_op_ffn_fused', 'wn_op_gemm_x6', 'wn_op_ffn_x6', 'wn_op_gemm_x6r', 'wn_op_gemm_x6r512', 'wn_profile_kernel_name', 'wn_profile_ffn_split', 'wn_profile_ffn_clocks', 'wn_profile_gemm_clocks', 'wn_filter_blank_embedding',
     'wn_workspace_create', 'wn_resample_length', 'wn_resample', 'wn_fbank', 'wn_log_mel', 'wn_encode', 'wn_encode_chunk', 'wn_set_encoder_out',
-    'wn_ctc_logprobs', 'wn_set_ctc_probs', 'wn_ctc_greedy_search', 'wn_ctc_force_align',
+    'wn_ctc_logprobs', 'wn_ctc_topk_host', 'wn_set_ctc_probs', 'wn_ctc_greedy_search', 'wn_ctc_force_align',
     'wn_set_context_graph', 'wn_ctc_prefix_beam_search', 'wn_attention_rescoring', 'wn_rescore', 'wn_rescore_prefetch', 'wn_decoder_forward', 'wn_decoder_next_topk', 'wn_op_gemm',
     'wn_op_layernorm', 'wn_op_log_add', 'wn_op_attention', 'wn_op_dwconv', 'wn_op_conv1',
     'wn_op_conv2d4',
@@ -158,6 +158,7 @@
     L.wn_encode.argtypes = [vp, vp, pi32, i32, i32, i32, i32, vp, pi32, vp]
     L.wn_set_encoder_out.argtypes = [vp, vp, pi32, i32, i32, vp]
     L.wn_ctc_logprobs.argtypes = [vp, i32, i32, f32, vp, i32, vp]
+    L.wn_ctc_topk_host.argtypes = [vp, vp, vp, i64, pi32, pi32, vp]
     L.wn_encode_chunk.argtypes = [vp, vp, i32, i32, i32, vp, i32, vp, vp, vp, vp, pi32,
                                   pi32, vp]
     L.wn_encode_chunk_batch.argtypes = [vp, i32, vp, i32, pi32, i32, POINTER(vp), pi32,
diff --git a/wenet_amd/csrc/cabi_align.hip b/wenet_amd/csrc/cabi_align.hip
--- a/wenet_amd/csrc/cabi_align.hip
+++ b/wenet_amd/csrc/cabi_align.hip
@@ -108,7 +108,7 @@
     } else {
       const ModelData& W = *m->data;
       WN_CHECK(W.ctc.w, "wn_ctc_force_align: this handle has no weights");
-      const int V4 = (V + 31) / 32 * 32;
+      const int V4 = ctc_logits_pitch(V);
       WN_TRY(m->logits.ensure((size_t)M * V4 * sizeof(float)));
       WN_TRY(vocab_linear(m, W.ctc, m->enc.as<float>(), m->cfg.d_model, m->logits.as<float>(), V4,
                           M, s));
diff --git a/wenet_amd/csrc/cabi_ctc.hip b/wenet_amd/csrc/cabi_ctc.hip
--- a/wenet_amd/csrc/cabi_ctc.hip
+++ b/wenet_amd/csrc/cabi_ctc.hip
@@ -223,9 +223,13 @@
   m->ctc_rows = M; m->ctc_k = k;
   int ldv = V;
   if (M > 0) {
-    const int V4 = (V + 31) / 32 * 32;
+    const int V4 = ctc_logits_pitch(V);
     ldv = V4;
     WN_TRY(m->logits.ensure((size_t)M * V4 * sizeof(float)));
+    if (m->dbg_logits_fill)
+      WN_HIP(hipMemsetD32Async((hipDeviceptr_t)m->logits.p,
+                               m->dbg_logits_fill == 1 ? 0x7fc00000 : 0x7f800000,
+                               (size_t)M * V4, s));
     WN_TRY(m->topk_val.ensure((size_t)M * k * sizeof(float)));
     WN_TRY(m->topk_idx.ensure((size_t)M * k * sizeof(int)));
     WN_TRY(vocab_linear(m, W.ctc, m->enc.as<float>(), c.d_model, m->logits.as<float>(), V4, M,
@@ -248,6 +252,27 @@
     }
   }
   m->ctc_valid = true;
+  return 0;
+}
+
+int wn_ctc_topk_host(wn_model* m, float* val_host, int32_t* idx_host, int64_t capacity,
+                     int32_t* rows_out, int32_t* k_out, void* stream) {
+  WN_CHECK(m && val_host && idx_host && rows_out && k_out, "wn_ctc_topk_host: null argument");
+  WN_ENTER(m);
+  WN_CHECK(m->ctc_valid, "wn_ctc_topk_host: no CTC posteriors (call wn_ctc_logprobs)");
+  hipStream_t s = (hipStream_t)stream;
+  WN_HIP(hipSetDevice(m->device));
+  const int64_t n = (int64_t)m->ctc_rows * m->ctc_k;
+  WN_CHECK(capacity >= n, "wn_ctc_topk_host: the arrays hold " + std::to_string(capacity) +
+                              " pairs, the batch has " + std::to_string(n));
+  *rows_out = m->ctc_rows; *k_out = m->ctc_k;
+  if (n > 0) {
+    WN_HIP(hipMemcpyAsync(val_host, m->topk_val.p, (size_t)n * sizeof(float),
+                          hipMemcpyDeviceToHost, s));
+    WN_HIP(hipMemcpyAsync(idx_host, m->topk_idx.p, (size_t)n * sizeof(int),
+                          hipMemcpyDeviceToHost, s));
+  }
+  WN_HIP(stream_wait(s));
   return 0;
 }
 
@@ -598,7 +623,7 @@
   WN_HIP(hipSetDevice(m->device));
   const wn_config& c = m->cfg;
   const int M = n * chunk, V = c.vocab, k = set->beam;
-  const int V4 = (V + 31) / 32 * 32;
+  const int V4 = ctc_logits_pitch(V);
   WN_TRY(set->logits.ensure((size_t)M * V4 * sizeof(float)));
   WN_TRY(set->topk_val.ensure((size_t)M * k * sizeof(float)));
   WN_TRY(set->topk_idx.ensure((size_t)M * k * sizeof(int)));
diff --git a/wenet_amd/csrc/cabi_firered.hip b/wenet_amd/csrc/cabi_firered.hip
--- a/wenet_amd/csrc/cabi_firered.hip
+++ b/wenet_amd/csrc/cabi_firered.hip
@@ -69,6 +69,7 @@
                std::to_string(Tp) + " encoder frames, more than the " +
                std::to_string(m->fr.c.max_frames) + " the position rows of this handle cover");
   m->ln0_done = false;
+  m->ln0_img = false;
   m->front_route = 0;
   std::vector<int> off2(B), len2(B), off1(B), len1(B), flen(B);
   int M = 0, M1 = 0, max_t2 = 0;
diff --git a/wenet_amd/csrc/cabi_model.hip b/wenet_amd/csrc/cabi_model.hip
--- a/wenet_amd/csrc/cabi_model.hip
+++ b/wenet_amd/csrc/cabi_model.hip
@@ -924,6 +924,7 @@
   const std::string k(key);
   if (k == "n_layers") m->dbg_layers = value;
   else if (k == "skip_after_norm") m->dbg_skip_after_norm = value;
+  else if (k == "logits_fill") m->dbg_logits_fill = value;
   else { set_error("wn_debug_set: unknown key " + k); return -1; }
   return 0;
 }
diff --git a/wenet_amd/csrc/conformer.hip b/wenet_amd/csrc/conformer.hip
--- a/wenet_amd/csrc/conformer.hip
+++ b/wenet_amd/csrc/conformer.hip
@@ -116,6 +116,21 @@
   if (r == 0 || (r == 2 && tune().x6_af32 != 0)) return nullptr;
   if (m->t1_img.ensure(x6_bytes(m->rows, m->cfg.d_model)) != 0) return nullptr;
   return m->t1_img.p;
+}
+
+void* layer0_ffn_image(wn_model* m) {
+  const ModelData& W = *m->data;
+  if (W.layers.empty() || m->dbg_layers == 0) return nullptr;
+  return t1_image_for(m, W.layers[0].ffm1, W.layers[0].ffm2, ACT_SILU);
+}
+
+static void* enc_image_for(wn_model* m) {
+  const ModelData& W = *m->data;
+  if (tune().enc_tail_img == 0 || m->dbg_skip_after_norm || !W.ctc.w) return nullptr;
+  const float* bias = nullptr;
+  if (!vocab_x6_image(m, W.ctc, m->cfg.d_model, m->rows, &bias)) return nullptr;
+  if (m->enc_img.ensure(x6_bytes(m->rows, m->cfg.d_model)) != 0) return nullptr;
+  return m->enc_img.p;
 }
 
 static int ffn_x6_try(wn_model* m, const Linear& w1, const Linear& w2, int act, hipStream_t s) {
@@ -428,7 +443,8 @@
   return linear(L.pw2, t1, d, x, d, M, s, ACT_NONE, x, d);
 }
 
-int final_ffn(const LayerCtx& c, const EncLayer& L, const EncLayer* Ln, bool ln_ff_done) {
+int final_ffn(const LayerCtx& c, const EncLayer& L, const EncLayer* Ln, bool ln_ff_done,
+              bool* enc_done = nullptr) {
   wn_model* m = c.m;
   const int d = c.d, M = c.M;
   hipStream_t s = c.s;
@@ -440,9 +456,17 @@
   }
   if (fS > 0) {
     const float* P = m->ffn_part.as<float>();
-    if (!Ln)
-      return ffn_reduce_ln(c.x, P, fS, L.ff2.b, 0.5f, L.norm_final.w, L.norm_final.b, nullptr,
-                           nullptr, nullptr, M, d, c.eps, 2, s);
+    if (!Ln) {
+      void* enc_img = enc_done ? enc_image_for(m) : nullptr;
+      if (!enc_img || m->enc.ensure((size_t)M * d * sizeof(float)) != 0)
+        return ffn_reduce_ln(c.x, P, fS, L.ff2.b, 0.5f, L.norm_final.w, L.norm_final.b, nullptr,
+                             nullptr, nullptr, M, d, c.eps, 2, s);
+      const Norm& an = m->data->after_norm;
+      WN_TRY(ffn_reduce_ln_img(c.x, P, fS, L.ff2.b, 0.5f, L.norm_final.w, L.norm_final.b, an.w,
+                               an.b, enc_img, M, d, c.eps, s, 1, m->enc.as<float>()));
+      *enc_done = true;
+      return 0;
+    }
     void* mac_img = t1_image_for(m, Ln->ffm1, Ln->ffm2, ACT_SILU);
     if (!mac_img)
       return ffn_reduce_ln(c.x, P, fS, L.ff2.b, 0.5f, L.norm_final.w, L.norm_final.b,
@@ -466,7 +490,9 @@
   const wn_config& cfg = m->cfg;
   const LayerCtx c(m, chunk, left, s);
   const int n_run = m->dbg_layers >= 0 ? std::min(m->dbg_layers, cfg.n_layers) : cfg.n_layers;
-  m->t1_img_ok = false;
+  m->t1_img_ok = m->ln0_done && m->ln0_img;
+  m->ln0_img = false;
+  bool enc_done = false;
   for (int li = 0; li < n_run; ++li) {
     const EncLayer& L = W.layers[li];
     const void* qkv_w6 = x6r_image(c, L.qkv, 3 * c.d, 0);
@@ -475,7 +501,13 @@
     WN_TRY(macaron_ffn(c, L, li, qkv_w6 != nullptr, &pro_S));
     WN_TRY(self_attention(c, L, qkv_w6, pro_S));
     WN_TRY(conv_module(c, L, &ln_ff_done));
-    WN_TRY(final_ffn(c, L, li + 1 < n_run ? &W.layers[li + 1] : nullptr, ln_ff_done));
+    const bool last = li + 1 == n_run;
+    WN_TRY(final_ffn(c, L, last ? nullptr : &W.layers[li + 1], ln_ff_done,
+                     last ? &enc_done : nullptr));
+  }
+  if (enc_done) {
+    m->enc_img_ok = true;
+    return 0;
   }
   return after_norm_out(m, s);
 }
diff --git a/wenet_amd/csrc/ffn_fused.hip b/wenet_amd/csrc/ffn_fused.hip
--- a/wenet_amd/csrc/ffn_fused.hip
+++ b/wenet_amd/csrc/ffn_fused.hip
@@ -253,7 +253,8 @@
     }
     for (; s < S; ++s)
       acc += *reinterpret_cast<const f32x4*>(P + ((int64_t)s * M + row) * D + c);
-    const f32x4 xo = *reinterpret_cast<const f32x4*>(x + (int64_t)row * D + c);
+    f32x4 xo = {0.f, 0.f, 0.f, 0.f};
+    if (MODE != 3) xo = *reinterpret_cast<const f32x4*>(x + (int64_t)row * D + c);
 #pragma unroll
     for (int e = 0; e < 4; ++e) v[4 * j + e] = xo[e] + alpha * acc[e];
   }
@@ -283,7 +284,7 @@
       for (int e = 0; e < 4; ++e) v[4 * j + e] = (v[4 * j + e] - mean) * rstd * ww[e] + bv[e];
     }
   };
-  if (MODE == 0) {
+  if (MODE == 0 || MODE == 3) {
     store(x);
     norm(w, b);
     store(y);
@@ -299,11 +300,40 @@
 }
 
 template <int E>
+__device__ __forceinline__ void ln_rows_pinned(float (&v)[E], const float* gw, const float* gb,
+                                               int lane, float eps) {
+#pragma clang fp contract(off)
+  constexpr int D = E * 64;
+  float s = 0.f;
+#pragma unroll
+  for (int e = 0; e < E; ++e) s += v[e];
+  const float mean = wave_sum(s) * (1.0f / D);
+  float q = 0.f;
+#pragma unroll
+  for (int e = 0; e < E; ++e) {
+    const float d = v[e] - mean;
+    const float d2 = d * d;
+    q += d2;
+  }
+  const float rstd = 1.0f / sqrtf(__builtin_fmaf(wave_sum(q), 1.0f / D, eps));
+#pragma unroll
+  for (int j = 0; j < E / 4; ++j) {
+    const f32x4 ww = *reinterpret_cast<const f32x4*>(gw + j * 256 + lane * 4);
+    const f32x4 bv = *reinterpret_cast<const f32x4*>(gb + j * 256 + lane * 4);
+#pragma unroll
+    for (int e = 0; e < 4; ++e) {
+      const float t = (v[4 * j + e] - mean) * rstd;
+      v[4 * j + e] = __builtin_fmaf(t, ww[e], bv[e]);
+    }
+  }
+}
+
+template <int E, int FORM>
 __global__ __launch_bounds__(256) void ffn_reduce_ln_img_kernel(
     float* __restrict__ x, const float* __restrict__ P, int S, const float* __restrict__ b2,
     float alpha, const float* __restrict__ w, const float* __restrict__ b,
-    const float* __restrict__ w2, const float* __restrict__ bb2, char* __restrict__ y3,
-    int M, float eps) {
+    const float* __restrict__ w2, const float* __restrict__ bb2, float* __restrict__ y,
+    char* __restrict__ y3, int M, float eps) {
   static_assert(E % 4 == 0, "4 columns per lane and chunk");
   constexpr int D = E * 64;
   constexpr int NP = D / 8;
@@ -331,10 +361,17 @@
       }
       for (; s < S; ++s)
         acc += *reinterpret_cast<const f32x4*>(P + ((int64_t)s * M + row) * D + c);
-      const f32x4 xo = *reinterpret_cast<const f32x4*>(x + (int64_t)row * D + c);
+      f32x4 xo = {0.f, 0.f, 0.f, 0.f};
+      if (FORM != 2) xo = *reinterpret_cast<const f32x4*>(x + (int64_t)row * D + c);
 #pragma unroll
       for (int e = 0; e < 4; ++e) v[4 * j + e] = xo[e] + alpha * acc[e];
     }
+    auto store = [&](float* dst) {
+#pragma unroll
+      for (int j = 0; j < E / 4; ++j)
+        *reinterpret_cast<f32x4*>(dst + (int64_t)row * D + j * 256 + lane * 4) =
+            f32x4{v[4 * j], v[4 * j + 1], v[4 * j + 2], v[4 * j + 3]};
+    };
     auto norm = [&](const float* gw, const float* gb) {
       float sm = 0.f;
 #pragma unroll
@@ -355,12 +392,19 @@
         for (int e = 0; e < 4; ++e) v[4 * j + e] = (v[4 * j + e] - mean) * rstd * ww[e] + bv[e];
       }
     };
-    norm(w, b);
-#pragma unroll
-    for (int j = 0; j < E / 4; ++j)
-      *reinterpret_cast<f32x4*>(x + (int64_t)row * D + j * 256 + lane * 4) =
-          f32x4{v[4 * j], v[4 * j + 1], v[4 * j + 2], v[4 * j + 3]};
-    norm(w2, bb2);
+    if (FORM == 2) {
+      store(x);
+      norm(w, b);
+    } else {
+      norm(w, b);
+      store(x);
+      if (FORM == 1) {
+        ln_rows_pinned<E>(v, w2, bb2, lane, eps);
+        store(y);
+      } else {
+        norm(w2, bb2);
+      }
+    }
 #pragma unroll
     for (int j = 0; j < E / 4; ++j) {
       bf16x4 h0, h1, h2;
@@ -446,15 +490,17 @@
 int ffn_reduce_ln(float* x, const float* P, int S, const float* b2, float alpha,
                   const float* w, const float* b, const float* w2, const float* bb2, float* y,
                   int M, int D, float eps, int mode, hipStream_t s) {
-  WN_CHECK(M > 0 && (D == 256 || D == 512) && mode >= 0 && mode <= 2, "ffn_reduce_ln: shape");
+  WN_CHECK(M > 0 && (D == 256 || D == 512) && mode >= 0 && mode <= 3, "ffn_reduce_ln: shape");
   dim3 g(cdiv(M, 4)), t(256);
 #define WN_RL(E, MODE)                                                                 \
   hipLaunchKernelGGL((ffn_reduce_ln_kernel<E, MODE>), g, t, 0, s, x, P, S, b2, alpha, w, b, \
                      w2, bb2, y, M, eps)
   if (D == 256) {
-    if (mode == 0) WN_RL(4, 0); else if (mode == 1) WN_RL(4, 1); else WN_RL(4, 2);
+    if (mode == 0) WN_RL(4, 0); else if (mode == 1) WN_RL(4, 1); else if (mode == 2) WN_RL(4, 2);
+    else WN_RL(4, 3);
   } else {
-    if (mode == 0) WN_RL(8, 0); else if (mode == 1) WN_RL(8, 1); else WN_RL(8, 2);
+    if (mode == 0) WN_RL(8, 0); else if (mode == 1) WN_RL(8, 1); else if (mode == 2) WN_RL(8, 2);
+    else WN_RL(8, 3);
   }
 #undef WN_RL
   WN_HIP(hipGetLastError());
@@ -463,14 +509,20 @@
 
 int ffn_reduce_ln_img(float* x, const float* P, int S, const float* b2, float alpha,
                       const float* w, const float* b, const float* w2, const float* bb2,
-                      void* y3, int M, int D, float eps, hipStream_t s) {
-  WN_CHECK(M > 0 && (D == 256 || D == 512) && y3 && w2 && bb2, "ffn_reduce_ln_img: shape");
-  if (D == 256)
-    hipLaunchKernelGGL(ffn_reduce_ln_img_kernel<4>, dim3(cdiv(M, 8)), dim3(256), 0, s, x, P, S,
-                       b2, alpha, w, b, w2, bb2, reinterpret_cast<char*>(y3), M, eps);
-  else
-    hipLaunchKernelGGL(ffn_reduce_ln_img_kernel<8>, dim3(cdiv(M, 8)), dim3(256), 0, s, x, P, S,
-                       b2, alpha, w, b, w2, bb2, reinterpret_cast<char*>(y3), M, eps);
+                      void* y3, int M, int D, float eps, hipStream_t s, int form, float* y) {
+  WN_CHECK(M > 0 && (D == 256 || D == 512) && y3 && form >= 0 && form <= 2,
+           "ffn_reduce_ln_img: shape");
+  WN_CHECK(form == 2 || (w2 && bb2), "ffn_reduce_ln_img: forms 0 and 1 take a second LayerNorm");
+  WN_CHECK(form != 1 || y, "ffn_reduce_ln_img: form 1 writes the fp32 rows too");
+#define WN_RLI(E, FORM)                                                                        \
+  hipLaunchKernelGGL((ffn_reduce_ln_img_kernel<E, FORM>), dim3(cdiv(M, 8)), dim3(256), 0, s, x, P, \
+                     S, b2, alpha, w, b, w2, bb2, y, reinterpret_cast<char*>(y3), M, eps)
+  if (D == 256) {
+    if (form == 0) WN_RLI(4, 0); else if (form == 1) WN_RLI(4, 1); else WN_RLI(4, 2);
+  } else {
+    if (form == 0) WN_RLI(8, 0); else if (form == 1) WN_RLI(8, 1); else WN_RLI(8, 2);
+  }
+#undef WN_RLI
   WN_HIP(hipGetLastError());
   return 0;
 }
diff --git a/wenet_amd/csrc/kernels.h b/wenet_amd/csrc/kernels.h
--- a/wenet_amd/csrc/kernels.h
+++ b/wenet_amd/csrc/kernels.h
@@ -164,7 +164,8 @@
                   int M, int D, float eps, int mode, hipStream_t s);
 int ffn_reduce_ln_img(float* x, const float* P, int S, const float* b2, float alpha,
                       const float* w, const float* b, const float* w2, const float* bb2,
-                      void* y3, int M, int D, float eps, hipStream_t s);
+                      void* y3, int M, int D, float eps, hipStream_t s, int form = 0,
+                      float* y = nullptr);
 
 struct X6Args {
   const void* A3 = nullptr;
diff --git a/wenet_amd/csrc/model.hip b/wenet_amd/csrc/model.hip
--- a/wenet_amd/csrc/model.hip
+++ b/wenet_amd/csrc/model.hip
@@ -115,6 +115,7 @@
 
 int after_norm_out(wn_model* m, hipStream_t s) {
   const int d = m->cfg.d_model, M = m->rows;
+  m->enc_img_ok = false;
   WN_TRY(m->enc.ensure((size_t)std::max(M, 1) * d * sizeof(float)));
   if (m->dbg_skip_after_norm) {
     WN_HIP(hipMemcpyAsync(m->enc.p, m->x.p, (size_t)M * d * sizeof(float),
@@ -225,29 +226,42 @@
   return 0;
 }
 
-int vocab_linear(wn_model* m, const Linear& l, const float* A, int lda, float* C, int ldc,
-                 int M, hipStream_t s) {
+const void* vocab_x6_image(const wn_model* m, const Linear& l, int lda, int M,
+                           const float** bias) {
   const ModelData& W = *m->data;
   const int V = l.out, V4 = (V + 3) / 4 * 4;
-  WN_CHECK(ldc >= V4 && ldc % 4 == 0, "vocab_linear: pitch");
   const void* w6 = nullptr;
-  const float* bias = l.b;
+  *bias = l.b;
   if (t_gemm_prec == PREC_F32 && tune().gemm_x6 != 0 && tune().x6_linear != 0 &&
       l.in % 16 == 0 && lda % 4 == 0 && M >= 512) {
     auto it = W.x6_at.find(l.w);
     if (it != W.x6_at.end()) w6 = it->second;
     if (w6 && V != V4 && l.b) {
-      bias = nullptr;
+      *bias = nullptr;
       auto ib = W.bias4.find(l.w);
-      if (ib != W.bias4.end()) bias = ib->second;
-      if (!bias) w6 = nullptr;
-    }
-  }
+      if (ib != W.bias4.end()) *bias = ib->second;
+      if (!*bias) w6 = nullptr;
+    }
+  }
+  return w6;
+}
+
+int vocab_linear(wn_model* m, const Linear& l, const float* A, int lda, float* C, int ldc,
+                 int M, hipStream_t s) {
+  const int V = l.out, V4 = (V + 3) / 4 * 4;
+  WN_CHECK(ldc >= V4 && ldc % 4 == 0, "vocab_linear: pitch");
+  const float* bias = nullptr;
+  const void* w6 = vocab_x6_image(m, l, lda, M, &bias);
   if (!w6) return linear(l, A, lda, C, ldc, M, s);
-  WN_TRY(m->x6_lin.ensure(x6_bytes(M, l.in)));
-  WN_TRY(x6_split(A, M, l.in, lda, m->x6_lin.as<char>(), s));
+  const bool have_img = A == m->enc.as<float>() && m->enc_img_ok && M == m->rows &&
+                        l.in == m->cfg.d_model && lda == l.in && m->enc_img.p;
+  if (!have_img) {
+    WN_TRY(m->x6_lin.ensure(x6_bytes(M, l.in)));
+    WN_TRY(x6_split(A, M, l.in, lda, m->x6_lin.as<char>(), s));
+  }
   X6Args x;
-  x.A3 = m->x6_lin.as<char>(); x.B3 = w6; x.M = M; x.N = V4; x.K = l.in;
+  x.A3 = have_img ? m->enc_img.as<char>() : m->x6_lin.as<char>();
+  x.B3 = w6; x.M = M; x.N = V4; x.K = l.in;
   x.epi = 0; x.bias = bias; x.C = C; x.ldc = ldc;
   return gemm_x6(x, s);
 }
@@ -334,6 +348,7 @@
                const std::vector<int>& len, int rows, hipStream_t s) {
   m->B = B; m->Tp = Tp; m->off = off; m->len = len; m->rows = rows;
   m->mem_cache_valid = false;
+  m->enc_img_ok = false;
   if (m->kv_ready) {
     (void)hipStreamWaitEvent(s, m->side.e1, 0);
     m->kv_ready = false;
@@ -393,11 +408,25 @@
   g.B3 = it->second; g.M = M; g.N = d; g.K = K; g.epi = 1; g.ksplit = S; g.bm = bm;
   g.C = m->ffn_part.as<float>();
   WN_TRY(gemm_x6(g, s));
-  WN_HIP(hipMemsetAsync(m->x.p, 0, (size_t)M * d * sizeof(float), s));
   const EncLayer& L0 = W.layers[0];
-  WN_TRY(ffn_reduce_ln(m->x.as<float>(), m->ffn_part.as<float>(), S, W.sub_out.b, sqrtf((float)d),
-                       L0.norm_ff_mac.w, L0.norm_ff_mac.b, nullptr, nullptr, m->t1.as<float>(), M,
-                       d, c.norm_eps, 0, s));
+  if (tune().sub_out_img == 0) {
+    WN_HIP(hipMemsetAsync(m->x.p, 0, (size_t)M * d * sizeof(float), s));
+    WN_TRY(ffn_reduce_ln(m->x.as<float>(), m->ffn_part.as<float>(), S, W.sub_out.b,
+                         sqrtf((float)d), L0.norm_ff_mac.w, L0.norm_ff_mac.b, nullptr, nullptr,
+                         m->t1.as<float>(), M, d, c.norm_eps, 0, s));
+    m->ln0_done = true;
+    return 1;
+  }
+  if (void* img = layer0_ffn_image(m)) {
+    WN_TRY(ffn_reduce_ln_img(m->x.as<float>(), m->ffn_part.as<float>(), S, W.sub_out.b,
+                             sqrtf((float)d), L0.norm_ff_mac.w, L0.norm_ff_mac.b, nullptr,
+                             nullptr, img, M, d, c.norm_eps, s, 2));
+    m->ln0_img = true;
+  } else {
+    WN_TRY(ffn_reduce_ln(m->x.as<float>(), m->ffn_part.as<float>(), S, W.sub_out.b,
+                         sqrtf((float)d), L0.norm_ff_mac.w, L0.norm_ff_mac.b, nullptr, nullptr,
+                         m->t1.as<float>(), M, d, c.norm_eps, 3, s));
+  }
   m->ln0_done = true;
   return 1;
 }
@@ -435,6 +464,7 @@
   const int d = c.d_model, F1 = m->F1(), F2 = m->F2();
   const int Tp = ((T - 1) / 2 - 1) / 2;
   m->ln0_done = false;
+  m->ln0_img = false;
   m->front_route = 0;
   WN_CHECK(pos0 + Tp <= c.max_pos, "utterance longer than the positional table");
   std::vector<int> off2(B), len2(B), off1(B), len1(B);
@@ -637,6 +667,7 @@
   m->B = B; m->Tp = Tp; m->off = off2; m->len = len2; m->rows = M;
   m->ctc_valid = false;
   m->mem_cache_valid = false;
+  m->enc_img_ok = false;
   if (m->kv_ready) {
     (void)hipStreamWaitEvent(s, m->side.e1, 0);
     m->kv_ready = false;
diff --git a/wenet_amd/csrc/model_state.h b/wenet_amd/csrc/model_state.h
--- a/wenet_amd/csrc/model_state.h
+++ b/wenet_amd/csrc/model_state.h
@@ -285,6 +285,10 @@
   int ctc_rows = 0, ctc_k = 0;
   bool ctc_valid = false;
   bool ln0_done = false;
+  bool ln0_img = false;
+  DevBuf enc_img;
+  bool enc_img_ok = false;
+  int dbg_logits_fill = 0;
   int front_route = 0;
   DevBuf logits, topk_val, topk_idx;
   DevBuf pb_dbg;
@@ -441,6 +445,11 @@
 int build_x6_images(const wn_config& cfg, ModelData& W, bool skip_encoder = false);
 int vocab_linear(wn_model* m, const Linear& l, const float* A, int lda, float* C, int ldc, int M,
                  hipStream_t s);
+const void* vocab_x6_image(const wn_model* m, const Linear& l, int lda, int M, const float** bias);
+inline int ctc_logits_pitch(int V) {
+  return tune().ctc_pitch32 != 0 ? (V + 31) / 32 * 32 : (V + 3) / 4 * 4;
+}
+void* layer0_ffn_image(wn_model* m);
 int scatter_padded(const float* src, int lds, const int* off, const int* len, int B, int Tp, int D,
                    float* dst, hipStream_t s);
 int set_layout(wn_model* m, int B, int Tp, const std::vector<int>& off,
diff --git a/wenet_amd/csrc/tune.h b/wenet_amd/csrc/tune.h
--- a/wenet_amd/csrc/tune.h
+++ b/wenet_amd/csrc/tune.h
@@ -88,6 +88,12 @@
   X(sync_spin, 1)                                                                               \
                          \
   X(ctc_wave, 1)                                                                                \
+              \
+  X(ctc_pitch32, 1)                                                                             \
+                                                                     \
+  X(enc_tail_img, 1)                                                                            \
+                                     \
+  X(sub_out_img, 1)                                                                             \
         \
   X(dec_skinny, 0)                                                                              \
                                             \
```

After: 72270 (median of 4 runs). Within noise of the previous version (+0.9%).
